# dylkot/cNMF

Measured on NVIDIA H100. Metric: NMF restarts/sec on NxG counts, K-sweep x100 seeds, 1/2/4/8 H100 vs sklearn CPU, higher is better.
Workload: dtype f32 (2-pass split-fp16 tensor-core products of group-normalised factors x exact integer counts, fp32 accumulate)

## Files before the change

### cnmf_b200/_lib.py

```python
import ctypes
import os

import numpy as np

_HERE = os.path.dirname(os.path.abspath(__file__))
LIB_PATH = os.path.join(_HERE, "libcnmf_b200.so")

SOLVER_MU, SOLVER_CD = 0, 1
PRECISION_FP32, PRECISION_TF32X3, PRECISION_TF32X3_GENERAL, PRECISION_F16X2, PRECISION_FP64 = 0, 1, 2, 3, 4
LOSS_FROBENIUS, LOSS_KULLBACK_LEIBLER, LOSS_ITAKURA_SAITO = 0, 1, 2
INIT_RANDOM, INIT_NNDSVD, INIT_NNDSVDA, INIT_NNDSVDAR = 0, 1, 2, 3
INIT_CODES = {"random": INIT_RANDOM, "nndsvd": INIT_NNDSVD, "nndsvda": INIT_NNDSVDA, "nndsvdar": INIT_NNDSVDAR}
MAX_COMPONENTS = 32


class CnmfError(RuntimeError):
    pass


class NmfParams(ctypes.Structure):
    _fields_ = [("solver", ctypes.c_int32), ("precision", ctypes.c_int32), ("max_iter", ctypes.c_int32),
                ("reserved", ctypes.c_int32), ("tol", ctypes.c_double),
                ("l1_reg_W", ctypes.c_double), ("l2_reg_W", ctypes.c_double),
                ("l1_reg_H", ctypes.c_double), ("l2_reg_H", ctypes.c_double),
                ("beta_loss", ctypes.c_int32), ("reserved2", ctypes.c_int32)]


UNIT_SOLVER_NONE = -1
UNIT_PIECES_NONE, UNIT_PIECES_TF32, UNIT_PIECES_F16 = 0, 1, 2
UNIT_GRAM_NONE, UNIT_GRAM_FUSED, UNIT_GRAM_STANDALONE = 0, 1, 2


class UpdateStepArgs(ctypes.Structure):
    _fields_ = [("n_slots", ctypes.c_int32), ("n_rids", ctypes.c_int32),
                ("ks", ctypes.c_void_p), ("rids", ctypes.c_void_p), ("done", ctypes.c_void_p),
                ("n", ctypes.c_int32), ("cpb_tiles", ctypes.c_int32), ("solver", ctypes.c_int32),
                ("pieces", ctypes.c_int32), ("gram", ctypes.c_int32), ("want_scalar", ctypes.c_int32),
                ("nsplit", ctypes.c_int32), ("l1", ctypes.c_float), ("l2", ctypes.c_float),
                ("F", ctypes.c_void_p), ("num", ctypes.c_void_p), ("gram_in", ctypes.c_void_p),
                ("piece_scale", ctypes.c_void_p), ("pieces_hi", ctypes.c_void_p), ("pieces_lo", ctypes.c_void_p),
                ("tile_scale", ctypes.c_void_p), ("gram_out", ctypes.c_void_p), ("scal_out", ctypes.c_void_p)]


UNIT_BETA_UPDATE, UNIT_BETA_DIVERGENCE = 0, 1
UNIT_SIDE_W, UNIT_SIDE_H = 0, 1


class BetaStepArgs(ctypes.Structure):
    _fields_ = [("n_slots", ctypes.c_int32), ("n_rids", ctypes.c_int32),
                ("ks", ctypes.c_void_p), ("rids", ctypes.c_void_p), ("done", ctypes.c_void_p),
                ("op", ctypes.c_int32), ("side", ctypes.c_int32), ("loss", ctypes.c_int32),
                ("n_items", ctypes.c_int32), ("n_contract", ctypes.c_int32), ("l1", ctypes.c_float), ("l2", ctypes.c_float),
                ("D", ctypes.c_void_p), ("F_own", ctypes.c_void_p), ("F_other", ctypes.c_void_p),
                ("oth_sum", ctypes.c_void_p), ("last", ctypes.c_void_p), ("totals", ctypes.c_void_p)]


UNIT_F64_UPDATE, UNIT_F64_GRAM, UNIT_F64_CROSS = 0, 1, 2


class UpdateStepF64Args(ctypes.Structure):
    _fields_ = [("n_slots", ctypes.c_int32), ("n_rids", ctypes.c_int32),
                ("ks", ctypes.c_void_p), ("rids", ctypes.c_void_p), ("done", ctypes.c_void_p),
                ("n", ctypes.c_int32), ("op", ctypes.c_int32), ("solver", ctypes.c_int32),
                ("want_scalar", ctypes.c_int32), ("l1", ctypes.c_double), ("l2", ctypes.c_double),
                ("F", ctypes.c_void_p), ("num", ctypes.c_void_p), ("gram_in", ctypes.c_void_p),
                ("gram_out", ctypes.c_void_p), ("scal_out", ctypes.c_void_p)]


FORM_FP32, FORM_TF32, FORM_TF32_EXACT, FORM_F16_EXACT, FORM_FP64 = 0, 1, 2, 3, 4
FORM_NAMES = {FORM_FP32: "fp32", FORM_TF32: "tf32", FORM_TF32_EXACT: "tf32_exact", FORM_F16_EXACT: "f16_exact",
              FORM_FP64: "fp64"}
OPERANDS = {"X": 0, "Xt": 1, "X_hi": 2, "X_lo": 3, "Xt_hi": 4, "Xt_lo": 5, "X_h16": 6, "Xt_h16": 7, "row_scale": 8,
            "col_scale": 9, "csc_col_ptr": 10, "csc_row_idx": 11, "csc_values": 12}


class ConvCheckArgs(ctypes.Structure):
    _fields_ = [("n_slots", ctypes.c_int32), ("n_rids", ctypes.c_int32),
                ("ks", ctypes.c_void_p), ("rids", ctypes.c_void_p),
                ("solver", ctypes.c_int32), ("it", ctypes.c_int32), ("max_iter", ctypes.c_int32),
                ("tol", ctypes.c_double), ("normX2", ctypes.c_double),
                ("cross", ctypes.c_void_p), ("gramA", ctypes.c_void_p), ("gramB", ctypes.c_void_p),
                ("violA", ctypes.c_void_p), ("violB", ctypes.c_void_p),
                ("done", ctypes.c_void_p), ("n_iter", ctypes.c_void_p),
                ("err0", ctypes.c_void_p), ("prev", ctypes.c_void_p), ("last", ctypes.c_void_p)]


_c = ctypes
_vp, _i, _ll, _d = _c.c_void_p, _c.c_int, _c.c_longlong, _c.c_double
_pp = _c.POINTER

SIGNATURES = {
    "cnmf_abi_version": (_i, []),
    "cnmf_last_error": (_c.c_char_p, []),
    "cnmf_create": (_i, [_pp(_vp), _i]),
    "cnmf_destroy": (_i, [_vp]),
    "cnmf_launch_count": (_ll, [_vp]),
    "cnmf_mem_info": (_i, [_vp, _pp(_ll), _pp(_ll), _pp(_ll)]),
    "cnmf_solve_bytes_per_row": (_ll, [_vp]),
    "cnmf_profile_enable": (_i, [_vp, _i]),
    "cnmf_profile_get": (_i, [_vp, _pp(_d), _pp(_ll), _pp(_d)]),
    "cnmf_profile_get_class": (_i, [_vp, _i, _pp(_d), _pp(_ll), _pp(_d)]),
    "cnmf_last_timing": (_i, [_vp, _pp(_d), _pp(_d), _pp(_d), _pp(_d)]),
    "cnmf_dataset_create": (_i, [_vp, _vp, _i, _i, _ll, _i, _i, _vp, _pp(_vp)]),
    "cnmf_dataset_create_csc": (_i, [_vp, _i, _i, _ll, _vp, _vp, _vp, _i, _vp, _pp(_vp)]),
    "cnmf_dataset_create_csr": (_i, [_vp, _i, _i, _ll, _vp, _vp, _vp, _i, _vp, _pp(_vp)]),
    "cnmf_dataset_create_from_csr": (_i, [_vp, _i, _i, _ll, _vp, _vp, _vp, _i, _vp, _pp(_vp)]),
    "cnmf_dataset_create_from_csr_f64": (_i, [_vp, _i, _i, _ll, _vp, _vp, _vp, _vp, _pp(_vp)]),
    "cnmf_dataset_dense_bytes": (_i, [_i, _i, _i, _pp(_ll)]),
    "cnmf_dataset_from_columns": (_i, [_vp, _vp, _vp, _i, _vp, _pp(_vp)]),
    "cnmf_dataset_destroy": (_i, [_vp]),
    "cnmf_dataset_shape": (_i, [_vp, _pp(_i), _pp(_i)]),
    "cnmf_dataset_ld": (_i, [_vp, _pp(_i), _pp(_i)]),
    "cnmf_dataset_is_exact": (_i, [_vp]),
    "cnmf_dataset_sums": (_i, [_vp, _pp(_d), _pp(_d)]),
    "cnmf_dataset_min": (_i, [_vp, _pp(_c.c_float), _vp]),
    "cnmf_dataset_col_stats": (_i, [_vp, _vp, _vp, _vp]),
    "cnmf_dataset_row_sums": (_i, [_vp, _vp, _vp]),
    "cnmf_dataset_scaled_col_stats": (_i, [_vp, _vp, _vp, _vp, _vp]),
    "cnmf_dataset_scale_rows": (_i, [_vp, _vp, _vp, _pp(_vp)]),
    "cnmf_dataset_tpm_stats": (_i, [_vp, _d, _vp, _vp, _vp, _vp]),
    "cnmf_random_init_host": (_i, [_c.c_uint32, _d, _i, _i, _i, _vp, _ll, _vp, _ll]),
    "cnmf_random_init_dev": (_i, [_vp, _i, _vp, _vp, _vp, _vp, _vp]),
    "cnmf_nndsvd_init_dev": (_i, [_vp, _i, _vp, _vp, _i, _vp, _vp, _vp]),
    "cnmf_nndsvd_chunk_limit": (_i, [_vp, _i]),
    "cnmf_nndsvd_gemm_host": (_i, [_vp, _i, _i, _vp, _vp, _vp]),
    "cnmf_dataset_create_f64": (_i, [_vp, _vp, _i, _i, _ll, _i, _vp, _pp(_vp)]),
    "cnmf_dataset_from_columns_f64": (_i, [_vp, _vp, _vp, _i, _vp, _pp(_vp)]),
    "cnmf_factorize_f64": (_i, [_vp, _i, _vp, _vp, _pp(NmfParams), _vp, _vp, _vp, _vp, _vp]),
    "cnmf_factorize_init_f64": (_i, [_vp, _i, _vp, _vp, _vp, _pp(NmfParams), _vp, _vp, _vp, _vp, _vp]),
    "cnmf_refit_f64": (_i, [_vp, _i, _i, _vp, _pp(NmfParams), _vp, _pp(_c.c_int32), _pp(_d), _vp]),
    "cnmf_project_rows_f64": (_i, [_vp, _i, _vp, _vp, _vp]),
    "cnmf_factorize": (_i, [_vp, _i, _vp, _vp, _pp(NmfParams), _vp, _vp, _vp, _vp, _vp]),
    "cnmf_factorize_seeds_dev": (_i, [_vp, _i, _vp, _vp, _pp(NmfParams), _vp, _ll, _vp, _vp, _vp]),
    "cnmf_allgather_spectra": (_i, [_vp, _vp, _ll, _ll, _vp, _vp]),
    "cnmf_comm_unique_id": (_i, [_vp]),
    "cnmf_comm_create": (_i, [_vp, _vp, _i, _i, _pp(_vp)]),
    "cnmf_comm_destroy": (_i, [_vp]),
    "cnmf_factorize_init": (_i, [_vp, _i, _vp, _vp, _vp, _pp(NmfParams), _vp, _vp, _vp, _vp, _vp]),
    "cnmf_factorize_dev": (_i, [_vp, _i, _vp, _vp, _vp, _pp(NmfParams), _vp, _vp, _vp, _vp]),
    "cnmf_refit": (_i, [_vp, _i, _i, _vp, _pp(NmfParams), _vp, _pp(_c.c_int32), _pp(_d), _vp]),
    "cnmf_project_rows": (_i, [_vp, _i, _vp, _vp, _vp]),
    "cnmf_gemm_abt_host": (_i, [_vp, _i, _vp, _vp, _i, _i, _i, _i, _i, _vp, _vp, _i, _vp, _i, _pp(_c.c_float), _vp]),
    "cnmf_update_step_host": (_i, [_vp, _pp(UpdateStepArgs), _vp]),
    "cnmf_beta_step_host": (_i, [_vp, _pp(BetaStepArgs), _vp]),
    "cnmf_update_step_f64_host": (_i, [_vp, _pp(UpdateStepF64Args), _vp]),
    "cnmf_conv_check_host": (_i, [_vp, _pp(ConvCheckArgs), _vp]),
    "cnmf_dataset_form": (_i, [_vp]),
    "cnmf_dataset_operand_host": (_i, [_vp, _i, _vp, _ll]),
    "cnmf_dataset_gemm_host": (_i, [_vp, _i, _i, _i, _vp, _vp, _pp(_i)]),
    "cnmf_l2_normalize_rows": (_i, [_vp, _vp, _i, _i, _i, _vp]),
    "cnmf_local_density": (_i, [_vp, _vp, _i, _i, _i, _i, _vp, _vp, _vp]),
    "cnmf_col_stats_dev": (_i, [_vp, _vp, _i, _i, _i, _vp, _vp, _vp]),
    "cnmf_gather_rows": (_i, [_vp, _vp, _i, _vp, _i, _i, _vp, _i, _vp]),
    "cnmf_sq_dists_to_rows": (_i, [_vp, _vp, _i, _i, _i, _vp, _i, _vp, _vp]),
    "cnmf_kmeans_step": (_i, [_vp, _vp, _i, _i, _i, _i, _vp, _vp, _vp, _vp, _vp, _vp, _vp, _vp, _pp(_c.c_int32), _pp(_c.c_int32), _pp(_d), _vp]),
    "cnmf_kmeans_fit": (_i, [_vp, _vp, _i, _i, _i, _i, _i, _i, _d, _vp, _vp, _i, _vp, _vp, _vp, _pp(_c.c_int32), _vp]),
    "cnmf_kmeans_assign": (_i, [_vp, _vp, _i, _i, _i, _vp, _i, _vp, _vp, _vp, _vp, _vp, _vp, _vp]),
    "cnmf_cluster_dist_sums": (_i, [_vp, _vp, _i, _i, _i, _vp, _i, _vp, _vp]),
    "cnmf_cluster_median": (_i, [_vp, _vp, _i, _i, _i, _vp, _i, _vp, _i, _vp]),
    "cnmf_l2_normalize_rows_f64": (_i, [_vp, _vp, _i, _i, _i, _vp]),
    "cnmf_local_density_f64": (_i, [_vp, _vp, _i, _i, _i, _i, _vp, _vp, _vp]),
    "cnmf_col_stats_dev_f64": (_i, [_vp, _vp, _i, _i, _i, _vp, _vp, _vp]),
    "cnmf_gather_rows_f64": (_i, [_vp, _vp, _i, _vp, _i, _i, _vp, _i, _vp]),
    "cnmf_sq_dists_to_rows_f64": (_i, [_vp, _vp, _i, _i, _i, _vp, _i, _vp, _vp]),
    "cnmf_kmeans_step_f64": (_i, [_vp, _vp, _i, _i, _i, _i, _vp, _vp, _vp, _vp, _vp, _vp, _pp(_c.c_int32), _pp(_c.c_int32), _pp(_d), _vp]),
    "cnmf_kmeans_fit_f64": (_i, [_vp, _vp, _i, _i, _i, _i, _i, _i, _d, _vp, _vp, _i, _vp, _vp, _vp, _pp(_c.c_int32), _vp]),
    "cnmf_kmeans_assign_f64": (_i, [_vp, _vp, _i, _i, _i, _vp, _i, _vp, _vp, _vp, _vp, _vp, _vp, _vp]),
    "cnmf_cluster_dist_sums_f64": (_i, [_vp, _vp, _i, _i, _i, _vp, _i, _vp, _vp]),
    "cnmf_cluster_median_f64": (_i, [_vp, _vp, _i, _i, _i, _vp, _i, _vp, _i, _vp]),
    "cnmf_moe_grams": (_i, [_vp, _vp, _vp, _vp, _i, _i, _i, _vp, _vp]),
    "cnmf_moe_correct": (_i, [_vp, _vp, _i, _i, _i, _ll, _i, _vp, _vp, _vp, _i, _i, _i, _vp, _ll, _i, _vp, _vp, _vp]),
    "cnmf_scale_quantile_ceiling": (_i, [_vp, _vp, _i, _i, _i, _ll, _i, _vp, _vp, _ll, _d, _i, _ll, _ll, _d, _vp, _ll,
                                         _i, _pp(_d), _vp]),
}

_lib = None


ABI_VERSION = 19


def load():
    global _lib
    if _lib is not None:
        return _lib
    if not os.path.exists(LIB_PATH):
        raise CnmfError(
            "libcnmf_b200.so not found at %s -- build it with `python -m cnmf_b200.build` "
            "(cnmf_b200 has no CPU / PyTorch fallback)" % LIB_PATH)
    lib = ctypes.CDLL(LIB_PATH)
    for name, (res, args) in SIGNATURES.items():
        fn = getattr(lib, name)
        fn.restype = res
        fn.argtypes = args
    if lib.cnmf_abi_version() != ABI_VERSION:
        raise CnmfError("libcnmf_b200.so ABI version mismatch")
    _lib = lib
    return lib


def check(rc):
    if rc != 0:
        msg = load().cnmf_last_error()
        raise CnmfError("cnmf_b200 error %d: %s" % (rc, msg.decode() if msg else "?"))


def ptr(a):
    if a is None:
        return None
    assert a.flags["C_CONTIGUOUS"]
    return a.ctypes.data_as(ctypes.c_void_p)


def f32c(a):
    return np.ascontiguousarray(a, dtype=np.float32)


def f64c(a):
    return np.ascontiguousarray(a, dtype=np.float64)
```

### cnmf_b200/csrc/capi_refit.cu

```cuda
#include <algorithm>
#include <chrono>
#include <cmath>
#include <cstring>
#include <vector>

#include "engine.h"
#include "gemm.h"
#include "nmf_kernels.cuh"

using namespace cnmf;

namespace {

__global__ void fill_kernel(float* p, float v, int rows, int n, int ld) {
  const long long total = (long long)rows * n;
  for (long long i = blockIdx.x * (long long)blockDim.x + threadIdx.x; i < total; i += (long long)gridDim.x * blockDim.x)
    p[(i / n) * ld + (i % n)] = v;
}

template <typename T>
__global__ void col_stats_kernel(const T* __restrict__ X, int rows, int cols, int ld,
                                 const double* __restrict__ row_scale, double* __restrict__ part) {
  const int c = blockIdx.x * blockDim.x + threadIdx.x;
  if (c >= cols) return;
// ... 342 lines not shown
  if (!A) return -2;
  CNMF_CUDA_CHECK(cudaMemsetAsync(A, 0, nr * 4, s));
  CNMF_CUDA_CHECK(cudaMemcpy2DAsync(A, (size_t)d->ld_r * 4, Ut_host, (size_t)d->n_rows * 4, (size_t)d->n_rows * 4, k,
                                    cudaMemcpyHostToDevice, s));
  if (v.form != Form::FP32) {
    A_hi = static_cast<float*>(h->dev_buf("proj.A_hi", nr * 4));
    A_lo = static_cast<float*>(h->dev_buf("proj.A_lo", nr * 4));
    if (!A_hi || !A_lo) return -2;
    if (v.form == Form::F16_EXACT) {
      A_rs = static_cast<float*>(h->dev_buf("proj.A_rs", sizeof(float) * (size_t)k * ((d->ld_r + 511) / 512)));
      if (!A_rs) return -2;
    }
    CNMF_TRY(make_pieces(v.form, A, k, d->n_rows, d->ld_r, v.scale_r, A_hi, A_lo, A_rs, s));
    h->launches += 1;
  }
  GemmArgs g{};
  g.M = k; g.N = d->n_cols; g.Kd = d->n_rows;
  g.lda = d->ld_r; g.ldb = d->ld_r; g.ldc = d->ld_c;
  int splits = 1;
  {
    const int tiles = ((k + 127) / 128) * ((d->n_cols + 255) / 256);
    if (tiles < 2 * h->sm_count) splits = (2 * h->sm_count + tiles - 1) / tiles;
    splits = std::min(splits, std::max(1, ((d->n_rows + 31) / 32) / 8));
    splits = std::min(splits, 32);
    splits = gemm_effective_splits(d->n_rows, splits, v.form == Form::F16_EXACT ? 1 : 0);
  }
  g.splits = g.splits_effective = splits;
  g.c_split_stride = (long long)k * d->ld_c;
  float* C = static_cast<float*>(h->dev_buf("proj.C", (size_t)splits * k * d->ld_c * 4));
  if (!C) return -2;
  g.C = C;
  CNMF_TRY(form_gemm(v.form, g, A, A_hi, A_lo, A_rs, v.B_cols, v.scale_c, s));
  h->launches += 1;
  std::vector<float> tmp((size_t)splits * k * d->ld_c);
  CNMF_CUDA_CHECK(cudaMemcpyAsync(tmp.data(), C, tmp.size() * 4, cudaMemcpyDeviceToHost, s));
  CNMF_CUDA_CHECK(cudaStreamSynchronize(s));
  for (int c = 0; c < k; ++c)
    for (int j = 0; j < d->n_cols; ++j) {
      double a = 0.0;
      for (int z = 0; z < splits; ++z) a += tmp[(size_t)z * k * d->ld_c + (size_t)c * d->ld_c + j];
      out_host[(size_t)c * d->n_cols + j] = (float)a;
    }
  return 0;
}

int cnmf_dataset_from_columns_f64(cnmf_dataset_t src, const int32_t* cols_host, const double* divisor_host, int n_cols,
                                  void* stream, cnmf_dataset_t* out) {
  CNMF_REQUIRE(src && cols_host && divisor_host && out && n_cols > 0, "dataset_from_columns_f64: bad arguments");
  CNMF_TRY(require_f64(src, "dataset_from_columns"));
  for (int c = 0; c < n_cols; ++c)
    CNMF_REQUIRE(cols_host[c] >= 0 && cols_host[c] < src->n_cols, "dataset_from_columns_f64: column index out of range");
  cnmf_handle_s* h = src->h;
  cudaStream_t s = as_stream(stream);
  CNMF_CUDA_CHECK(cudaSetDevice(h->device));
  int* d_cols = static_cast<int*>(h->dev_buf("fromcols.idx", sizeof(int) * n_cols));
  double* d_div = static_cast<double*>(h->dev_buf("fromcols.div64", sizeof(double) * n_cols));
  if (!d_cols || !d_div) return -2;
  CNMF_CUDA_CHECK(cudaMemcpyAsync(d_cols, cols_host, sizeof(int) * n_cols, cudaMemcpyHostToDevice, s));
  CNMF_CUDA_CHECK(cudaMemcpyAsync(d_div, divisor_host, sizeof(double) * n_cols, cudaMemcpyHostToDevice, s));
  auto* d = new cnmf_dataset_s(h, src->n_rows, n_cols, CNMF_PRECISION_FP64);
  d->form = Form::FP64;
  const size_t nx = (size_t)d->n_rows * d->ld_c;
  float* buf = nullptr;
  int rc = dataset_alloc(d, &buf, 2 * nx);
  if (rc == 0) {
    d->X64 = reinterpret_cast<double*>(buf);
    if (cudaMemsetAsync(d->X64, 0, nx * sizeof(double), s) != cudaSuccess) rc = -2;
  }
  if (rc == 0) {
    dim3 grid((n_cols + 127) / 128, std::min(d->n_rows, 16384));
    gather_cols_div_kernel<<<grid, 128, 0, s>>>(src->X64, d->n_rows, src->ld_c, d_cols, d_div, n_cols, d->X64, d->ld_c);
    h->launches += 1;
    if (cudaGetLastError() != cudaSuccess) rc = -2;
  }
  double sums[2] = {0.0, 0.0};
  if (rc == 0) rc = matrix_sums_f64(h, d->X64, d->n_rows, d->n_cols, d->ld_c, sums, s);
  if (rc != 0) {
    cnmf_dataset_destroy(d);
    return rc;
  }
  d->sum = sums[0];
  d->sum_sq = sums[1];
  *out = d;
  return 0;
}

int cnmf_refit_f64(cnmf_dataset_t d, int transposed, int k, const double* fixed_host, const cnmf_nmf_params* p,
                   double* out_host, int32_t* n_iter_host, double* err_host, void* stream) {
  CNMF_REQUIRE(d && fixed_host && p && out_host, "refit_f64: NULL argument");
  CNMF_TRY(require_f64(d, "refit"));
  CNMF_TRY(check_params_precision(d, p));
  CNMF_REQUIRE(k >= 1 && k <= KMAX, "refit_f64: n_components must be in [1, 32] on the CUDA path");
  if (p->beta_loss != CNMF_LOSS_FROBENIUS) {
    set_last_error("cnmf_refit_f64: float64 datasets support beta_loss = frobenius only");
    return -3;
  }
  cnmf_handle_s* h = d->h;
  cudaStream_t s = as_stream(stream);
  CNMF_CUDA_CHECK(cudaSetDevice(h->device));
  const DataView v = make_view(d, transposed != 0);
  const size_t nr = (size_t)k * v.ld_r, nc = (size_t)k * v.ld_c;
  double* Fr = static_cast<double*>(h->dev_buf("refit.Fr64", nr * 8));
  double* Fc = static_cast<double*>(h->dev_buf("refit.Fc64", nc * 8));
  double* T = static_cast<double*>(h->dev_buf("refit.T64", (size_t)v.n_r * k * 8));
  if (!Fr || !Fc || !T) return -2;
  CNMF_CUDA_CHECK(cudaMemsetAsync(Fr, 0, nr * 8, s));
  CNMF_CUDA_CHECK(cudaMemsetAsync(Fc, 0, nc * 8, s));
  CNMF_CUDA_CHECK(cudaMemcpy2DAsync(Fc, (size_t)v.ld_c * 8, fixed_host, (size_t)v.n_c * 8, (size_t)v.n_c * 8, k,
                                    cudaMemcpyHostToDevice, s));
  if (p->solver == CNMF_SOLVER_MU) {
    const double mean = v.sum / ((double)v.n_r * (double)v.n_c);
    CNMF_TRY(fill_f64(Fr, std::sqrt(mean / k), k, v.n_r, v.ld_r, s));
    h->launches += 1;
  }
  SolveIO io;
  io.R = 1;
  io.ks = {k};
  io.Fr64 = Fr;
  io.Fc64 = Fc;
  io.update_cols = false;
  CNMF_TRY(solve_batched(h, v, io, *p, s));
  transpose64_kernel<<<NUM_SMS * 4, 256, 0, s>>>(Fr, k, v.n_r, v.ld_r, T);
  CNMF_CUDA_CHECK(cudaGetLastError());
  h->launches += 1;
  CNMF_CUDA_CHECK(cudaMemcpyAsync(out_host, T, (size_t)v.n_r * k * 8, cudaMemcpyDeviceToHost, s));
  CNMF_CUDA_CHECK(cudaStreamSynchronize(s));
  if (n_iter_host) *n_iter_host = io.n_iter[0];
  if (err_host) *err_host = io.err[0];
  return 0;
}

int cnmf_project_rows_f64(cnmf_dataset_t d, int k, const double* Ut_host, double* out_host, void* stream) {
  CNMF_REQUIRE(d && Ut_host && out_host && k >= 1, "project_rows_f64: bad arguments");
  CNMF_TRY(require_f64(d, "project_rows"));
  cnmf_handle_s* h = d->h;
  cudaStream_t s = as_stream(stream);
  CNMF_CUDA_CHECK(cudaSetDevice(h->device));
  const size_t na = (size_t)k * d->ld_r, nc = (size_t)k * d->ld_c;
  double* A = static_cast<double*>(h->dev_buf("proj.A64", na * 8));
  double* C = static_cast<double*>(h->dev_buf("proj.C64", nc * 8));
  if (!A || !C) return -2;
  CNMF_CUDA_CHECK(cudaMemsetAsync(A, 0, na * 8, s));
  CNMF_CUDA_CHECK(cudaMemcpy2DAsync(A, (size_t)d->ld_r * 8, Ut_host, (size_t)d->n_rows * 8, (size_t)d->n_rows * 8, k,
                                    cudaMemcpyHostToDevice, s));
  h->launches += 1;
  CNMF_TRY(launch_gemm_f64(A, d->ld_r, k, d->X64, d->n_rows, d->n_cols, d->ld_c, true, C, d->ld_c, s));
  CNMF_CUDA_CHECK(cudaMemcpy2DAsync(out_host, (size_t)d->n_cols * 8, C, (size_t)d->ld_c * 8, (size_t)d->n_cols * 8, k,
                                    cudaMemcpyDeviceToHost, s));
  CNMF_CUDA_CHECK(cudaStreamSynchronize(s));
  return 0;
}

int cnmf_gemm_abt_host(cnmf_handle_t h, int precision, const float* A, const float* B, int M, int N, int Kd, int splits,
                       int b_exact, const float* k_scale, const float* out_col_scale, int tile_n, float* C, int reps,
                       float* ms_out, void* stream) {
  CNMF_REQUIRE(h && A && B && C && M > 0 && N > 0 && Kd > 0, "gemm_abt_host: bad arguments");
  const bool f16 = precision == CNMF_PRECISION_F16X2;
  CNMF_REQUIRE(!b_exact || f16 || precision == CNMF_PRECISION_TF32X3, "gemm_abt_host: b_exact needs tf32x3 or f16x2");
  const bool exact = f16 || b_exact;
  CNMF_REQUIRE(exact || (!k_scale && !out_col_scale), "gemm_abt_host: k_scale / out_col_scale need an exact form");
  const Form form = f16 ? Form::F16_EXACT
                  : precision != CNMF_PRECISION_TF32X3 ? Form::FP32
                  : b_exact ? Form::TF32_EXACT : Form::TF32;
  cudaStream_t s = as_stream(stream);
  CNMF_CUDA_CHECK(cudaSetDevice(h->device));
  const int lda = pad_ld(Kd), ldc = pad_ld(N);
  const size_t na = (size_t)M * lda, nb = (size_t)N * lda;
  float* dA = static_cast<float*>(h->dev_buf("gemmtest.A", na * 4));
  float* dB = static_cast<float*>(h->dev_buf("gemmtest.B", nb * 4));
  float* dAh = static_cast<float*>(h->dev_buf("gemmtest.Ah", na * 4));
  float* dAl = static_cast<float*>(h->dev_buf("gemmtest.Al", na * 4));
  float* dBh = static_cast<float*>(h->dev_buf("gemmtest.Bh", nb * 4));
  float* dBl = static_cast<float*>(h->dev_buf("gemmtest.Bl", nb * 4));
  const int se = gemm_effective_splits(Kd, splits, f16 ? 1 : 0);
  float* dC = static_cast<float*>(h->dev_buf("gemmtest.C", (size_t)se * M * ldc * 4));
  float* dRs = static_cast<float*>(h->dev_buf("gemmtest.rs", sizeof(float) * (size_t)M * ((lda + 511) / 512)));
  if (!dA || !dB || !dAh || !dAl || !dBh || !dBl || !dC || !dRs) return -2;
  CNMF_CUDA_CHECK(cudaMemsetAsync(dA, 0, na * 4, s));
  CNMF_CUDA_CHECK(cudaMemsetAsync(dB, 0, nb * 4, s));
  CNMF_CUDA_CHECK(cudaMemcpy2DAsync(dA, (size_t)lda * 4, A, (size_t)Kd * 4, (size_t)Kd * 4, M, cudaMemcpyHostToDevice, s));
  CNMF_CUDA_CHECK(cudaMemcpy2DAsync(dB, (size_t)lda * 4, B, (size_t)Kd * 4, (size_t)Kd * 4, N, cudaMemcpyHostToDevice, s));
  float* dKs = nullptr;
  float* dCs = nullptr;
  if (k_scale) {
    dKs = static_cast<float*>(h->dev_buf("gemmtest.kscale", (size_t)lda * 4));
    if (!dKs) return -2;
    CNMF_CUDA_CHECK(cudaMemsetAsync(dKs, 0, (size_t)lda * 4, s));
    CNMF_CUDA_CHECK(cudaMemcpyAsync(dKs, k_scale, (size_t)Kd * 4, cudaMemcpyHostToDevice, s));
  }
  if (out_col_scale) {
    dCs = static_cast<float*>(h->dev_buf("gemmtest.cscale", (size_t)ldc * 4));
    if (!dCs) return -2;
    CNMF_CUDA_CHECK(cudaMemsetAsync(dCs, 0, (size_t)ldc * 4, s));
    CNMF_CUDA_CHECK(cudaMemcpyAsync(dCs, out_col_scale, (size_t)N * 4, cudaMemcpyHostToDevice, s));
  }
  if (f16) CNMF_TRY(launch_to_half(dB, dBh, (long long)nb, s));
  else if (form != Form::FP32) CNMF_TRY(launch_split_tf32(dB, dBh, dBl, (long long)nb, s));
  CNMF_TRY(make_pieces(form, dA, M, Kd, lda, dKs, dAh, dAl, dRs, s));
  CNMF_CUDA_CHECK(cudaMemsetAsync(dC, 0xff, (size_t)se * M * ldc * 4, s));
  GemmArgs g{};
  g.M = M; g.N = N; g.Kd = Kd; g.lda = lda; g.ldb = lda; g.ldc = ldc;
  g.C = dC; g.c_split_stride = (long long)M * ldc; g.splits = splits; g.splits_effective = se;
  g.tile_n = tile_n;
  const Operand Bop{dB, dBh, dBl, N, Kd, lda};
  cudaEvent_t e0, e1;
  CNMF_CUDA_CHECK(cudaEventCreate(&e0));
  CNMF_CUDA_CHECK(cudaEventCreate(&e1));
  if (reps < 1) reps = 1;
  int rc = form_gemm(form, g, dA, dAh, dAl, dRs, Bop, dCs, s);
  if (rc == 0 && reps > 1) {
    cudaEventRecord(e0, s);
    for (int i = 0; i < reps && rc == 0; ++i) rc = form_gemm(form, g, dA, dAh, dAl, dRs, Bop, dCs, s);
    cudaEventRecord(e1, s);
  }
  h->launches += reps;
  if (rc != 0) return rc;
  std::vector<float> tmp((size_t)se * M * ldc);
  CNMF_CUDA_CHECK(cudaMemcpyAsync(tmp.data(), dC, tmp.size() * 4, cudaMemcpyDeviceToHost, s));
  CNMF_CUDA_CHECK(cudaStreamSynchronize(s));
  if (ms_out) {
    float ms = 0.f;
    if (reps > 1) cudaEventElapsedTime(&ms, e0, e1);
    *ms_out = reps > 1 ? ms / reps : 0.f;
  }
  cudaEventDestroy(e0);
  cudaEventDestroy(e1);
  for (int m = 0; m < M; ++m)
    for (int n = 0; n < N; ++n) {
      double a = 0.0;
      for (int z = 0; z < se; ++z) a += tmp[(size_t)z * M * ldc + (size_t)m * ldc + n];
      C[(size_t)m * N + n] = (float)a;
    }
  return 0;
}

}
```

### cnmf_b200/csrc/capi_units.cu

```cuda
#include <algorithm>
#include <vector>

#include "engine.h"
#include "nmf_beta.h"
#include "nmf_f64.h"
#include "nmf_kernels.cuh"

using namespace cnmf;

extern "C" int cnmf_update_step_host(cnmf_handle_t h, const cnmf_update_step_args* a, void* stream) {
  CNMF_REQUIRE(h && a && a->ks && a->rids && a->done && a->F && a->gram_in, "update_step: NULL argument");
  CNMF_REQUIRE(a->n_slots >= 1 && a->n_rids >= 1 && a->n >= 1 && a->nsplit >= 1, "update_step: bad sizes");
  CNMF_REQUIRE(a->cpb_tiles == 1 || a->cpb_tiles == 2 || a->cpb_tiles == 4, "update_step: cpb_tiles must be 1, 2 or 4");
  CNMF_REQUIRE(a->solver == CNMF_SOLVER_MU || a->solver == CNMF_SOLVER_CD || a->solver == CNMF_UNIT_SOLVER_NONE,
               "update_step: unknown solver");
  CNMF_REQUIRE(a->pieces >= CNMF_UNIT_PIECES_NONE && a->pieces <= CNMF_UNIT_PIECES_F16, "update_step: unknown pieces mode");
  CNMF_REQUIRE(a->gram >= CNMF_UNIT_GRAM_NONE && a->gram <= CNMF_UNIT_GRAM_STANDALONE, "update_step: unknown Gram mode");
  CNMF_REQUIRE(a->pieces == CNMF_UNIT_PIECES_NONE || (a->pieces_hi && a->pieces_lo), "update_step: pieces buffers missing");
  CNMF_REQUIRE(a->pieces != CNMF_UNIT_PIECES_F16 || a->tile_scale, "update_step: tile_scale missing");
  CNMF_REQUIRE(a->gram == CNMF_UNIT_GRAM_NONE || a->gram_out, "update_step: gram_out missing");
  CNMF_REQUIRE(!a->want_scalar || a->scal_out, "update_step: scal_out missing");
  const bool none = a->solver == CNMF_UNIT_SOLVER_NONE;
  CNMF_REQUIRE(!none || a->gram != CNMF_UNIT_GRAM_FUSED, "update_step: no update launch to fuse the Gram into");
  CNMF_REQUIRE(a->num || (none && !a->want_scalar), "update_step: num missing");
// ... 248 lines not shown
  CNMF_REQUIRE(a->op != CNMF_UNIT_F64_CROSS || (a->num && a->scal_out), "update_step_f64: num / scal_out missing");
  CNMF_REQUIRE(a->op != CNMF_UNIT_F64_GRAM || a->gram_out, "update_step_f64: gram_out missing");
  CNMF_REQUIRE(!(upd && a->want_scalar) || a->scal_out, "update_step_f64: scal_out missing");
  const int R = a->n_slots, NR = a->n_rids;
  std::vector<int> meta;
  int SK = 0, kmax = 0;
  CNMF_TRY(unit_slots(a->ks, a->rids, a->done, R, NR, "update_step_f64", meta, &SK, &kmax));
  const int kp = round_up(kmax, 4);

  cudaStream_t s = as_stream(stream);
  CNMF_CUDA_CHECK(cudaSetDevice(h->device));
  const int n = a->n, ld = pad_ld(n);
  const size_t nf = (size_t)SK * ld, gsz = (size_t)NR * KMAX * KMAX;
  const int chunks = f64_chunks(n), gchunks = f64_gram_chunks(n);
  int* d_meta = static_cast<int*>(h->dev_buf("unit.meta", sizeof(int) * meta.size()));
  double* d_F = static_cast<double*>(h->dev_buf("unit.F64", nf * 8));
  double* d_num = static_cast<double*>(h->dev_buf("unit.num64", nf * 8));
  double* d_gin = static_cast<double*>(h->dev_buf("unit.gram_in", sizeof(double) * gsz));
  double* d_gout = static_cast<double*>(h->dev_buf("unit.gram_out", sizeof(double) * gsz));
  double* d_scal = static_cast<double*>(h->dev_buf("unit.scal", sizeof(double) * NR));
  double* d_gpart = static_cast<double*>(h->dev_buf("unit.gram_part", sizeof(double) * (size_t)NR * gchunks * kp * kp));
  double* d_spart = static_cast<double*>(h->dev_buf("unit.scal_part", sizeof(double) * (size_t)NR * chunks));
  if (!d_meta || !d_F || !d_num || !d_gin || !d_gout || !d_scal || !d_gpart || !d_spart) return -2;
  CNMF_CUDA_CHECK(cudaMemcpyAsync(d_meta, meta.data(), sizeof(int) * meta.size(), cudaMemcpyHostToDevice, s));
  CNMF_CUDA_CHECK(cudaMemcpyAsync(d_F, a->F, nf * 8, cudaMemcpyHostToDevice, s));
  if (a->num) CNMF_CUDA_CHECK(cudaMemcpyAsync(d_num, a->num, nf * 8, cudaMemcpyHostToDevice, s));
  if (a->gram_in) CNMF_CUDA_CHECK(cudaMemcpyAsync(d_gin, a->gram_in, sizeof(double) * gsz, cudaMemcpyHostToDevice, s));
  if (a->gram_out) CNMF_CUDA_CHECK(cudaMemcpyAsync(d_gout, a->gram_out, sizeof(double) * gsz, cudaMemcpyHostToDevice, s));
  if (a->scal_out) CNMF_CUDA_CHECK(cudaMemcpyAsync(d_scal, a->scal_out, sizeof(double) * NR, cudaMemcpyHostToDevice, s));

  const BatchMeta b{d_meta, d_meta + R, d_meta + 2 * R, d_meta + 3 * R, R, kp};
  const F64Launch L{h, s, SK};
  const F64View f{d_F, n, ld};
  if (upd)
    CNMF_TRY(f64_update(L, a->solver == CNMF_SOLVER_CD, f, d_num, d_gin, b, a->l1, a->l2, d_spart,
                        a->want_scalar ? d_scal : nullptr));
  else if (a->op == CNMF_UNIT_F64_GRAM)
    CNMF_TRY(f64_gram(L, f, b, d_gpart, d_gout));
  else
    CNMF_TRY(f64_cross(L, f, d_num, b, d_spart, d_scal));

  CNMF_CUDA_CHECK(cudaMemcpyAsync(a->F, d_F, nf * 8, cudaMemcpyDeviceToHost, s));
  if (a->gram_out) CNMF_CUDA_CHECK(cudaMemcpyAsync(a->gram_out, d_gout, sizeof(double) * gsz, cudaMemcpyDeviceToHost, s));
  if (a->scal_out) CNMF_CUDA_CHECK(cudaMemcpyAsync(a->scal_out, d_scal, sizeof(double) * NR, cudaMemcpyDeviceToHost, s));
  CNMF_CUDA_CHECK(cudaStreamSynchronize(s));
  return 0;
}

extern "C" int cnmf_conv_check_host(cnmf_handle_t h, const cnmf_conv_check_args* a, void* stream) {
  CNMF_REQUIRE(h && a && a->ks && a->rids && a->done && a->n_iter && a->err0 && a->prev && a->last,
               "conv_check: NULL argument");
  CNMF_REQUIRE(a->n_slots >= 1 && a->n_rids >= 1, "conv_check: bad sizes");
  CNMF_REQUIRE(a->solver == CNMF_SOLVER_MU || a->solver == CNMF_SOLVER_CD, "conv_check: unknown solver");
  const bool mu = a->solver == CNMF_SOLVER_MU;
  CNMF_REQUIRE(!mu || (a->cross && a->gramA && a->gramB), "conv_check: cross / gramA / gramB missing");
  CNMF_REQUIRE(mu || a->violA, "conv_check: violA missing");
  const int R = a->n_slots, NR = a->n_rids;
  std::vector<int> meta;
  int SK = 0, kmax = 0;
  CNMF_TRY(unit_slots(a->ks, a->rids, nullptr, R, NR, "conv_check", meta, &SK, &kmax));
  meta.resize(3 * R + 2 * NR);
  for (int r = 0; r < NR; ++r) {
    meta[3 * R + r] = a->done[r];
    meta[3 * R + NR + r] = a->n_iter[r];
  }

  cudaStream_t s = as_stream(stream);
  CNMF_CUDA_CHECK(cudaSetDevice(h->device));
  const size_t gsz = (size_t)NR * KMAX * KMAX;
  int* d_meta = static_cast<int*>(h->dev_buf("unit.meta", sizeof(int) * meta.size()));
  double* d_state = static_cast<double*>(h->dev_buf("unit.conv_state", sizeof(double) * 6 * NR));
  double* d_gram = static_cast<double*>(h->dev_buf("unit.conv_gram", sizeof(double) * 2 * gsz));
  if (!d_meta || !d_state || !d_gram) return -2;
  double *d_err0 = d_state, *d_prev = d_state + NR, *d_last = d_state + 2 * NR;
  double *d_x = d_state + 3 * NR, *d_vb = d_state + 4 * NR;
  CNMF_CUDA_CHECK(cudaMemcpyAsync(d_meta, meta.data(), sizeof(int) * meta.size(), cudaMemcpyHostToDevice, s));
  CNMF_CUDA_CHECK(cudaMemcpyAsync(d_err0, a->err0, sizeof(double) * NR, cudaMemcpyHostToDevice, s));
  CNMF_CUDA_CHECK(cudaMemcpyAsync(d_prev, a->prev, sizeof(double) * NR, cudaMemcpyHostToDevice, s));
  CNMF_CUDA_CHECK(cudaMemcpyAsync(d_last, a->last, sizeof(double) * NR, cudaMemcpyHostToDevice, s));
  CNMF_CUDA_CHECK(cudaMemcpyAsync(d_x, mu ? a->cross : a->violA, sizeof(double) * NR, cudaMemcpyHostToDevice, s));
  if (mu) {
    CNMF_CUDA_CHECK(cudaMemcpyAsync(d_gram, a->gramA, sizeof(double) * gsz, cudaMemcpyHostToDevice, s));
    CNMF_CUDA_CHECK(cudaMemcpyAsync(d_gram + gsz, a->gramB, sizeof(double) * gsz, cudaMemcpyHostToDevice, s));
  } else if (a->violB) {
    CNMF_CUDA_CHECK(cudaMemcpyAsync(d_vb, a->violB, sizeof(double) * NR, cudaMemcpyHostToDevice, s));
  }

  int* d_done = d_meta + 3 * R;
  const BatchMeta b{d_meta, d_meta + R, d_meta + 2 * R, d_done, R, round_up(kmax, 4)};
  const ConvState st{d_err0, d_prev, d_last, d_done, d_done + NR};
  h->launches += 1;
  if (mu) CNMF_TRY(launch_mu_check(st, d_x, d_gram, d_gram + gsz, a->normX2, b, a->it, a->tol, a->max_iter, s));
  else CNMF_TRY(launch_cd_check(st, d_x, a->violB ? d_vb : nullptr, b, a->it, a->tol, a->max_iter, s));

  CNMF_CUDA_CHECK(cudaMemcpyAsync(meta.data(), d_meta, sizeof(int) * meta.size(), cudaMemcpyDeviceToHost, s));
  CNMF_CUDA_CHECK(cudaMemcpyAsync(a->err0, d_err0, sizeof(double) * NR, cudaMemcpyDeviceToHost, s));
  CNMF_CUDA_CHECK(cudaMemcpyAsync(a->prev, d_prev, sizeof(double) * NR, cudaMemcpyDeviceToHost, s));
  CNMF_CUDA_CHECK(cudaMemcpyAsync(a->last, d_last, sizeof(double) * NR, cudaMemcpyDeviceToHost, s));
  CNMF_CUDA_CHECK(cudaStreamSynchronize(s));
  for (int r = 0; r < NR; ++r) {
    a->done[r] = meta[3 * R + r];
    a->n_iter[r] = meta[3 * R + NR + r];
  }
  return 0;
}

static_assert((int)Form::FP32 == CNMF_FORM_FP32 && (int)Form::TF32 == CNMF_FORM_TF32 &&
                  (int)Form::TF32_EXACT == CNMF_FORM_TF32_EXACT && (int)Form::F16_EXACT == CNMF_FORM_F16_EXACT &&
                  (int)Form::FP64 == CNMF_FORM_FP64,
              "CNMF_FORM_* mirror cnmf::Form");

extern "C" int cnmf_dataset_form(cnmf_dataset_t d) {
  CNMF_REQUIRE(d, "dataset_form: NULL dataset");
  return (int)d->form;
}

extern "C" int cnmf_dataset_operand_host(cnmf_dataset_t d, int which, void* out_host, long long bytes) {
  CNMF_REQUIRE(d && out_host, "dataset_operand: NULL argument");
  const long long nx = (long long)d->n_rows * d->ld_c, nxt = (long long)d->n_cols * d->ld_r;
  const void* src = nullptr;
  long long size = 0;
  switch (which) {
    case CNMF_OPERAND_X: src = d->X; size = 4 * nx; break;
    case CNMF_OPERAND_XT: src = d->Xt; size = 4 * nxt; break;
    case CNMF_OPERAND_X_HI: src = d->X_hi; size = 4 * nx; break;
    case CNMF_OPERAND_X_LO: src = d->X_lo; size = 4 * nx; break;
    case CNMF_OPERAND_XT_HI: src = d->Xt_hi; size = 4 * nxt; break;
    case CNMF_OPERAND_XT_LO: src = d->Xt_lo; size = 4 * nxt; break;
    case CNMF_OPERAND_X_H16: src = d->X_h16; size = 2 * nx; break;
    case CNMF_OPERAND_XT_H16: src = d->Xt_h16; size = 2 * nxt; break;
    case CNMF_OPERAND_ROW_SCALE: src = d->row_scale; size = 4LL * d->ld_r; break;
    case CNMF_OPERAND_COL_SCALE: src = d->col_scale; size = 4LL * d->ld_c; break;
    case CNMF_OPERAND_CSC_COL_PTR: src = d->col_ptr; size = 8LL * (d->n_cols + 1); break;
    case CNMF_OPERAND_CSC_ROW_IDX: src = d->row_idx; size = 4LL * d->nnz; break;
    case CNMF_OPERAND_CSC_VALUES: src = d->vals; size = 4LL * d->nnz; break;
    default: CNMF_REQUIRE(false, "dataset_operand: unknown array");
  }
  if (!src) {
    set_last_error("dataset_operand: this dataset does not hold that array");
    return -3;
  }
  CNMF_REQUIRE(bytes == size, "dataset_operand: bytes must be the array's size");
  CNMF_CUDA_CHECK(cudaSetDevice(d->h->device));
  CNMF_CUDA_CHECK(cudaMemcpy(out_host, src, (size_t)size, cudaMemcpyDeviceToHost));
  return 0;
}

extern "C" int cnmf_dataset_gemm_host(cnmf_dataset_t d, int transposed, int side, int SK, const float* F_host,
                                      float* out_host, int* splits_out) {
  CNMF_REQUIRE(d && splits_out && (side == 0 || side == 1) && SK >= 1, "dataset_gemm: bad arguments");
  CNMF_TRY(require_dense(d, "dataset_gemm"));
  cnmf_handle_s* h = d->h;
  const DataView v = make_view(d, transposed != 0);
  const GemmPlan plan = view_gemm_plan(v, side, SK);
  *splits_out = plan.splits;
  if (!out_host) return 0;
  CNMF_REQUIRE(F_host, "dataset_gemm: NULL factor");
  const int n_in = side == 0 ? v.n_c : v.n_r, ld_in = side == 0 ? v.ld_c : v.ld_r;
  const int n_out = side == 0 ? v.n_r : v.n_c, ld_out = side == 0 ? v.ld_r : v.ld_c;
  const float* piece_scale = side == 0 ? v.scale_c : v.scale_r;
  cudaStream_t s = nullptr;
  CNMF_CUDA_CHECK(cudaSetDevice(h->device));
  const size_t nf = (size_t)SK * ld_in, nc = (size_t)plan.splits * SK * ld_out;
  const int ktiles = (ld_in + 511) / 512;
  float* F = static_cast<float*>(h->dev_buf("unit.gemm_F", nf * 4));
  float* F_hi = static_cast<float*>(h->dev_buf("unit.gemm_F_hi", nf * 4));
  float* F_lo = static_cast<float*>(h->dev_buf("unit.gemm_F_lo", nf * 4));
  float* ts = static_cast<float*>(h->dev_buf("unit.gemm_tile_scale", sizeof(float) * (size_t)SK * ktiles));
  float* C = static_cast<float*>(h->dev_buf("unit.gemm_C", nc * 4));
  if (!F || !F_hi || !F_lo || !ts || !C) return -2;
  CNMF_CUDA_CHECK(cudaMemsetAsync(F, 0, nf * 4, s));
  CNMF_CUDA_CHECK(cudaMemcpy2DAsync(F, (size_t)ld_in * 4, F_host, (size_t)n_in * 4, (size_t)n_in * 4, SK,
                                    cudaMemcpyHostToDevice, s));
  CNMF_TRY(make_pieces(v.form, F, SK, n_in, ld_in, piece_scale, F_hi, F_lo, ts, s));
  h->launches += v.form == Form::FP32 ? 0 : 1;
  CNMF_TRY(view_gemm(h, v, side, F, F_hi, F_lo, ts, SK, C, plan, s));
  CNMF_CUDA_CHECK(cudaMemcpy2DAsync(out_host, (size_t)n_out * 4, C, (size_t)ld_out * 4, (size_t)n_out * 4,
                                    (size_t)plan.splits * SK, cudaMemcpyDeviceToHost, s));
  CNMF_CUDA_CHECK(cudaStreamSynchronize(s));
  return 0;
}
```

### cnmf_b200/csrc/engine.h

```cpp
#pragma once
#include <cuda_runtime.h>

#include <map>
#include <string>
#include <vector>

#include "../../include/cnmf_b200.h"
#include "common.cuh"
#include "gemm.h"

namespace cnmf {

enum class Form { FP32, TF32, TF32_EXACT, F16_EXACT, FP64 };
inline bool form_exact(Form f) { return f == Form::TF32_EXACT || f == Form::F16_EXACT; }

}

struct cnmf_handle_s {
  int device = 0;
  int sm_count = cnmf::NUM_SMS;
  long long launches = 0;
  bool profile = false;
  std::vector<cudaEvent_t> ev_pool;
  struct Pending { int begin; int end; int cls; double work; };
  int prof_last_end = -1;
  long long prof_last_launches = -1;
  cudaStream_t prof_last_stream = nullptr;
  std::vector<Pending> ev_pending;
  size_t ev_used = 0;
  static constexpr int PROF_CLASSES = 6;
  double prof_ms[PROF_CLASSES] = {}, prof_work[PROF_CLASSES] = {};
  long long prof_launches[PROF_CLASSES] = {};
  int nndsvd_chunk_restarts = 0;
  double t_rng_ms = 0, t_h2d_ms = 0, t_solve_ms = 0, t_d2h_ms = 0;
  int prof_begin(cudaStream_t s, double work, int cls = 0);
  void prof_end(cudaStream_t s, int slot);
  void prof_collect();
  std::map<std::string, std::pair<void*, size_t>> ws;
  std::map<std::string, std::pair<void*, size_t>> pinned;

  std::multimap<size_t, void*> pool;
  size_t pool_bytes = 0;
  void* pool_take(size_t bytes);
  void pool_give(void* p, size_t bytes);
  void* dev_buf(const std::string& name, size_t bytes);
  void* host_buf(const std::string& name, size_t bytes);
  void release_all();
};

struct cnmf_dataset_s {
  cnmf_handle_s* h = nullptr;
  int n_rows = 0, n_cols = 0;
  int ld_c = 0;
  int ld_r = 0;
  int precision = 0;
  cnmf::Form form = cnmf::Form::FP32;
  float *X = nullptr, *Xt = nullptr;
  float *X_hi = nullptr, *X_lo = nullptr, *Xt_hi = nullptr, *Xt_lo = nullptr;
  void *X_h16 = nullptr, *Xt_h16 = nullptr;
  float *row_scale = nullptr, *col_scale = nullptr;
  double sum = 0.0, sum_sq = 0.0;
  bool sparse = false;
  long long nnz = 0;
  long long* col_ptr = nullptr;
  int* row_idx = nullptr;
  float* vals = nullptr;
  double* col_sums = nullptr;
  int* item_ptr = nullptr;
  int n_items = 0;
  double* X64 = nullptr;
  std::vector<std::pair<void*, size_t>> owned;

  cnmf_dataset_s(cnmf_handle_s* h_, int rows, int cols, int precision_)
      : h(h_), n_rows(rows), n_cols(cols), ld_c(cnmf::pad_ld(cols)), ld_r(cnmf::pad_ld(rows)), precision(precision_) {}
};

namespace cnmf {

inline cudaStream_t as_stream(void* s) { return reinterpret_cast<cudaStream_t>(s); }

struct Operand {
  const float* full;
  const float* hi;
  const float* lo;
  int rows, cols, ld;
};

struct DataView {
  Operand B_rows;
  Operand B_cols;
  int n_r, n_c, ld_r, ld_c;
  double sum, sum_sq;
  Form form;
  const float* scale_r;
  const float* scale_c;
  const double* X64;
  bool transposed;
};

DataView make_view(const cnmf_dataset_s* d, bool transposed);

int form_gemm(Form form, GemmArgs g, const float* A, const float* A_hi, const float* A_lo, const float* a_tile_scale,
              const Operand& B, const float* out_scale, cudaStream_t s);
struct GemmPlan {
  int splits;
  long long split_stride;
};
GemmPlan view_gemm_plan(const DataView& v, int side, int SK);
int view_gemm(cnmf_handle_s* h, const DataView& v, int side, const float* F, const float* F_hi, const float* F_lo,
              const float* tile_scale, int SK, float* C, const GemmPlan& plan, cudaStream_t s);
int make_pieces(Form form, const float* F, int rows, int n, int ld, const float* scale, float* hi, float* lo,
                float* tile_scale, cudaStream_t s);

int dataset_alloc(cnmf_dataset_s* d, float** p, size_t elems);
int dataset_finish(cnmf_dataset_s* d, cudaStream_t s, bool exact = false);
int dataset_resolve_form(cnmf_dataset_s* d, bool exact, cudaStream_t s);
int check_params_precision(const cnmf_dataset_s* d, const cnmf_nmf_params* p);
int require_f32(const cnmf_dataset_s* d, const char* what);
int require_f64(const cnmf_dataset_s* d, const char* what);

struct SolveIO {
  int R = 0;
  std::vector<int> ks;
  float *Fr = nullptr, *Fc = nullptr;
  bool update_cols = true;
  const float* num_rows = nullptr;
  double *Fr64 = nullptr, *Fc64 = nullptr;
  std::vector<int> n_iter;
  std::vector<double> last;
  std::vector<double> err;
};

int solve_batched(cnmf_handle_s* h, const DataView& v, SolveIO& io, const cnmf_nmf_params& p, cudaStream_t s);
int solve_batched_beta(cnmf_handle_s* h, const DataView& v, SolveIO& io, const cnmf_nmf_params& p, cudaStream_t s);
int solve_batched_f64(cnmf_handle_s* h, const DataView& v, SolveIO& io, const cnmf_nmf_params& p, cudaStream_t s);
int matrix_sums_f64(cnmf_handle_s* h, const double* X, int rows, int cols, int ld, double* out_host, cudaStream_t s);
int fill_f64(double* p, double v, int rows, int n, int ld, cudaStream_t s);
int matrix_min(cnmf_handle_s* h, const float* X, int rows, int cols, int ld, float* out_host, cudaStream_t s);
int dataset_ensure_full_transpose(cnmf_dataset_s* d, cudaStream_t s);

constexpr int CSC_CHUNK = 4096;
int require_dense(const cnmf_dataset_s* d, const char* what);
int csc_project(const cnmf_dataset_s* d, const float* U, int k, int kp, float* out, int ld, cudaStream_t s);
int stage_rows(cnmf_handle_s* h, const float* F, int k, int n, int ld, int kp, float* U, cudaStream_t s);
int csc_col_stats(cnmf_dataset_s* d, cudaStream_t s);
int csc_detect_exact(cnmf_dataset_s* d, cudaStream_t s, bool* exact);
int csc_gather_cols(const cnmf_dataset_s* d, const int* cols, const float* scale, int n_cols, float* dst, int ld_dst,
                    cudaStream_t s);
int csc_tpm_sums(const cnmf_dataset_s* d, double target_sum, double* totals, double* col_sums, cudaStream_t s);
struct DeviceTemp {
  void* p = nullptr;
  DeviceTemp() = default;
  DeviceTemp(const DeviceTemp&) = delete;
  DeviceTemp& operator=(const DeviceTemp&) = delete;
  ~DeviceTemp() {
    if (p) cudaFree(p);
  }
  int alloc(size_t bytes, const std::string& what) {
    const cudaError_t e = cudaMalloc(&p, bytes < 256 ? 256 : bytes);
    if (e != cudaSuccess) {
      p = nullptr;
      set_last_error(what + ": cudaMalloc(" + std::to_string(bytes) + " bytes) failed: " + cudaGetErrorString(e));
      return -2;
    }
    return 0;
  }
  template <class T>
  T* as() const { return static_cast<T*>(p); }
};
int check_csr(const char* what, int n_rows, int n_cols, long long nnz, const int64_t* row_ptr, const int32_t* col_idx);
constexpr int CSR_ROW_BLOCK = 256;
constexpr long long CSR_COUNT_BUDGET = 1LL << 25;
int csr_to_csc(cnmf_dataset_s* d, const long long* row_ptr, const int* col_idx, const float* vals, cudaStream_t s);
int csr_scatter_rows(const long long* row_ptr, long long base, const int* col_idx, const float* vals, int r0, int r1,
                     float* X, int ld, cudaStream_t s);
int csr_scatter_rows(const long long* row_ptr, long long base, const int* col_idx, const double* vals, int r0, int r1,
                     double* X, int ld, cudaStream_t s);

int launch_gemm_f64(const double* A, int lda, int M, const float* X, int n_rows, int n_cols, int ldx, bool to_genes,
                    double* C, int ldc, cudaStream_t s);
int launch_gemm_f64(const double* A, int lda, int M, const double* X, int n_rows, int n_cols, int ldx, bool to_genes,
                    double* C, int ldc, cudaStream_t s);
int launch_gemm_f64_split(const double* A, int lda, int M, const float* X, int n_rows, int n_cols, int ldx,
                          bool to_genes, int k_chunk, double* C, int ldc, long long c_split_stride, cudaStream_t s);
int launch_gemm_f64_split(const double* A, int lda, int M, const double* X, int n_rows, int n_cols, int ldx,
                          bool to_genes, int k_chunk, double* C, int ldc, long long c_split_stride, cudaStream_t s);
int nndsvd_starts_dev(cnmf_dataset_s* d, int R, const int* ks, const uint32_t* seeds, int init, float* Wt, float* H,
                      cudaStream_t s);
int nndsvd_starts_dev(cnmf_dataset_s* d, int R, const int* ks, const uint32_t* seeds, int init, double* Wt, double* H,
                      cudaStream_t s);

}
```

### cnmf_b200/csrc/gemm.h

```cpp
#pragma once
#include <cuda_runtime.h>

namespace cnmf {

struct GemmArgs {
  const float* A_hi;
  const float* A_lo;
  const float* B_hi;
  const float* B_lo;
  float* C;
  int M, N, Kd;
  int lda, ldb, ldc;
  long long c_split_stride;
  int splits;
  int splits_effective;
  int b_exact;
  const float* out_col_scale;
  int f16;
  const float* a_tile_scale;
  int a_tiles;
  int tile_n;
};

int gemm_effective_splits(int Kd, int splits, int f16 = 0);

int gemm_fixed_splits(int Kd, int f16 = 0);

int gemm_tf32x3(const GemmArgs& g, cudaStream_t stream);

int gemm_fp32_simt(const GemmArgs& g, cudaStream_t stream);

}
```

### cnmf_b200/csrc/gemm_simt.cu

```cuda
#include <cuda_runtime.h>

#include "common.cuh"
#include "gemm.h"

namespace cnmf {

namespace {

constexpr int TM = 128, TN = 128, TK = 16;

__global__ void __launch_bounds__(256)
gemm_fp32_simt_kernel(const float* __restrict__ A, const float* __restrict__ B, float* __restrict__ C, int M, int N,
                      int Kd, int lda, int ldb, int ldc, long long c_split_stride, int k_per_split) {
  __shared__ float As[TK][TM + 4];
  __shared__ float Bs[TK][TN + 4];

  const int m0 = blockIdx.y * TM;
  const int n0 = blockIdx.x * TN;
  const int z = blockIdx.z;
  const int k_begin = z * k_per_split;
  const int k_end = min(Kd, k_begin + k_per_split);

  const int tid = threadIdx.x;
  const int tx = tid & 15;
  const int ty = tid >> 4;
  const int lrow = tid >> 2;
  const int lk = (tid & 3) * 4;

  float acc[8][8];
#pragma unroll
  for (int i = 0; i < 8; ++i)
#pragma unroll
    for (int j = 0; j < 8; ++j) acc[i][j] = 0.f;

  for (int k0 = k_begin; k0 < k_end; k0 += TK) {
#pragma unroll
    for (int h = 0; h < 2; ++h) {
      const int r = lrow + h * 64;
      float4 va = make_float4(0.f, 0.f, 0.f, 0.f), vb = va;
      const int gk = k0 + lk;
      if (m0 + r < M) {
        const float* p = A + static_cast<long long>(m0 + r) * lda + gk;
        if (gk + 3 < k_end) va = *reinterpret_cast<const float4*>(p);
        else {
          if (gk < k_end) va.x = p[0];
          if (gk + 1 < k_end) va.y = p[1];
          if (gk + 2 < k_end) va.z = p[2];
        }
      }
      if (n0 + r < N) {
        const float* p = B + static_cast<long long>(n0 + r) * ldb + gk;
        if (gk + 3 < k_end) vb = *reinterpret_cast<const float4*>(p);
        else {
          if (gk < k_end) vb.x = p[0];
          if (gk + 1 < k_end) vb.y = p[1];
          if (gk + 2 < k_end) vb.z = p[2];
        }
      }
      As[lk + 0][r] = va.x; As[lk + 1][r] = va.y; As[lk + 2][r] = va.z; As[lk + 3][r] = va.w;
      Bs[lk + 0][r] = vb.x; Bs[lk + 1][r] = vb.y; Bs[lk + 2][r] = vb.z; Bs[lk + 3][r] = vb.w;
    }
    __syncthreads();
#pragma unroll
    for (int k = 0; k < TK; ++k) {
      float a[8], b[8];
      const float4 a0 = *reinterpret_cast<const float4*>(&As[k][ty * 4]);
      const float4 a1 = *reinterpret_cast<const float4*>(&As[k][ty * 4 + 64]);
      const float4 b0 = *reinterpret_cast<const float4*>(&Bs[k][tx * 4]);
      const float4 b1 = *reinterpret_cast<const float4*>(&Bs[k][tx * 4 + 64]);
      a[0] = a0.x; a[1] = a0.y; a[2] = a0.z; a[3] = a0.w; a[4] = a1.x; a[5] = a1.y; a[6] = a1.z; a[7] = a1.w;
      b[0] = b0.x; b[1] = b0.y; b[2] = b0.z; b[3] = b0.w; b[4] = b1.x; b[5] = b1.y; b[6] = b1.z; b[7] = b1.w;
#pragma unroll
      for (int i = 0; i < 8; ++i)
#pragma unroll
        for (int j = 0; j < 8; ++j) acc[i][j] = fmaf(a[i], b[j], acc[i][j]);
    }
    __syncthreads();
  }

  float* Cz = C + static_cast<long long>(z) * c_split_stride;
#pragma unroll
  for (int i = 0; i < 8; ++i) {
    const int m = m0 + ty * 4 + (i & 3) + (i >> 2) * 64;
    if (m >= M) continue;
#pragma unroll
    for (int jh = 0; jh < 2; ++jh) {
      const int n = n0 + tx * 4 + jh * 64;
      if (n + 3 < ldc && n < round_up(N, 4)) {
        *reinterpret_cast<float4*>(Cz + static_cast<long long>(m) * ldc + n) =
            make_float4(acc[i][jh * 4], acc[i][jh * 4 + 1], acc[i][jh * 4 + 2], acc[i][jh * 4 + 3]);
      }
    }
  }
}

}

int gemm_fp32_simt(const GemmArgs& g, cudaStream_t stream) {
  CNMF_REQUIRE(g.M > 0 && g.N > 0 && g.Kd > 0, "gemm: empty problem");
  CNMF_REQUIRE(g.lda % 4 == 0 && g.ldb % 4 == 0 && g.ldc % 4 == 0, "gemm: leading dimensions must be multiples of 4 floats");
  const int splits = gemm_effective_splits(g.Kd, g.splits);
  CNMF_REQUIRE(splits == g.splits_effective, "gemm: splits_effective mismatch");
  const int total_kb = (g.Kd + 31) / 32;
  const int kb_per_split = (total_kb + splits - 1) / splits;
  dim3 grid((g.N + TN - 1) / TN, (g.M + TM - 1) / TM, splits);
  gemm_fp32_simt_kernel<<<grid, 256, 0, stream>>>(g.A_hi, g.B_hi, g.C, g.M, g.N, g.Kd, g.lda, g.ldb, g.ldc,
                                                   g.c_split_stride, kb_per_split * 32);
  CNMF_CUDA_CHECK(cudaGetLastError());
  return 0;
}

}
```

### cnmf_b200/csrc/gemm_tf32x3.cu

```cuda
#include <cuda.h>
#include <cuda_runtime.h>
#include <cstdint>
#include <cstdio>
#include <algorithm>
#include <map>
#include <mutex>
#include <tuple>

#include "common.cuh"
#include "gemm.h"

namespace cnmf {

namespace {

constexpr int BM = 128;
constexpr int NUM_THREADS = 128 * (1 + BM / 64);
constexpr int BK = 32;
constexpr long long WAIT_TIMEOUT_CYCLES = 4000000000LL;

template <int BN, int STAGES, bool BEXACT>
struct SmemLayout {
  static constexpr int A_BYTES = BM * BK * 4;
  static constexpr int B_BYTES = BN * BK * 4;
  static constexpr int STAGE_BYTES = 2 * A_BYTES + (BEXACT ? 1 : 2) * B_BYTES;
  static constexpr int BAR_OFFSET = STAGES * STAGE_BYTES;
  static constexpr int TOTAL = BAR_OFFSET + 3 * STAGES * 8;
  static constexpr int DYN_BYTES = TOTAL + 1024;
  static_assert(DYN_BYTES <= 227 * 1024, "pipeline stages do not fit the shared memory of an SM");
};

__device__ __forceinline__ void mbar_init(uint32_t bar, uint32_t count) {
  asm volatile("mbarrier.init.shared::cta.b64 [%0], %1;" ::"r"(bar), "r"(count) : "memory");
}
__device__ __forceinline__ void mbar_arrive_expect_tx(uint32_t bar, uint32_t bytes) {
  asm volatile("mbarrier.arrive.expect_tx.shared::cta.b64 _, [%0], %1;" ::"r"(bar), "r"(bytes) : "memory");
}
__device__ __forceinline__ void mbar_arrive(uint32_t bar) {
  asm volatile("mbarrier.arrive.shared::cta.b64 _, [%0];" ::"r"(bar) : "memory");
}
__device__ __forceinline__ bool mbar_try_wait(uint32_t bar, uint32_t parity) {
  uint32_t ok;
  asm volatile(
      "{\n\t.reg .pred p;\n\t"
      "mbarrier.try_wait.parity.shared::cta.b64 p, [%1], %2;\n\t"
      "selp.u32 %0, 1, 0, p;\n\t}"
      : "=r"(ok)
      : "r"(bar), "r"(parity)
      : "memory");
  return ok != 0;
}
template <bool TRAP>
__device__ __forceinline__ void mbar_wait(uint32_t bar, uint32_t parity) {
  if (mbar_try_wait(bar, parity)) return;
  const long long t0 = clock64();
  while (!mbar_try_wait(bar, parity)) {
    if (TRAP && clock64() - t0 > WAIT_TIMEOUT_CYCLES) __trap();
  }
}
__device__ __forceinline__ void tma_load_2d(uint32_t dst, const CUtensorMap* map, uint32_t bar, int c0, int c1) {
  asm volatile(
      "cp.async.bulk.tensor.2d.shared::cluster.global.mbarrier::complete_tx::bytes [%0], [%1, {%3, %4}], [%2];"
      ::"r"(dst), "l"(reinterpret_cast<uint64_t>(map)), "r"(bar), "r"(c0), "r"(c1)
      : "memory");
}
__device__ __forceinline__ void tma_load_2d_multicast(uint32_t dst, const CUtensorMap* map, uint32_t bar, int c0, int c1,
                                                      uint16_t mask) {
  asm volatile(
      "cp.async.bulk.tensor.2d.shared::cluster.global.mbarrier::complete_tx::bytes.multicast::cluster"
      " [%0], [%1, {%3, %4}], [%2], %5;"
      ::"r"(dst), "l"(reinterpret_cast<uint64_t>(map)), "r"(bar), "r"(c0), "r"(c1), "h"(mask)
      : "memory");
}

__device__ __forceinline__ void mbar_arrive_remote(uint32_t bar, uint32_t rank) {
  asm volatile(
      "{\n\t.reg .b32 remote;\n\t"
      "mapa.shared::cluster.u32 remote, %0, %1;\n\t"
      "mbarrier.arrive.shared::cluster.b64 _, [remote];\n\t}"
      ::"r"(bar), "r"(rank)
      : "memory");
}
__device__ __forceinline__ void cluster_sync() {
  asm volatile("barrier.cluster.arrive.release;\n\tbarrier.cluster.wait.acquire;" ::: "memory");
}

__device__ __forceinline__ uint64_t make_smem_desc(uint32_t smem_addr) {
  uint64_t d = 0;
  d |= static_cast<uint64_t>((smem_addr & 0x3FFFFu) >> 4);
  d |= static_cast<uint64_t>(1) << 16;
  d |= static_cast<uint64_t>(1024 >> 4) << 32;
  d |= static_cast<uint64_t>(1) << 62;
  return d;
}

__device__ __forceinline__ void named_bar_sync(uint32_t id, uint32_t count) {
  asm volatile("bar.sync %0, %1;" ::"r"(id), "r"(count) : "memory");
}
__device__ __forceinline__ void named_bar_arrive(uint32_t id, uint32_t count) {
  asm volatile("bar.arrive %0, %1;" ::"r"(id), "r"(count) : "memory");
}

template <int N>
__device__ __forceinline__ void setmaxnreg_dec() { asm volatile("setmaxnreg.dec.sync.aligned.u32 %0;" ::"n"(N)); }
template <int N>
__device__ __forceinline__ void setmaxnreg_inc() { asm volatile("setmaxnreg.inc.sync.aligned.u32 %0;" ::"n"(N)); }

__device__ __forceinline__ void wgmma_fence() { asm volatile("wgmma.fence.sync.aligned;" ::: "memory"); }
__device__ __forceinline__ void wgmma_commit() { asm volatile("wgmma.commit_group.sync.aligned;" ::: "memory"); }
template <int N>
__device__ __forceinline__ void wgmma_wait() { asm volatile("wgmma.wait_group.sync.aligned %0;" ::"n"(N) : "memory"); }

#define CNMF_R64                                                                      \
  "%0, %1, %2, %3, %4, %5, %6, %7, %8, %9, %10, %11, %12, %13, %14, %15, "            \
  "%16, %17, %18, %19, %20, %21, %22, %23, %24, %25, %26, %27, %28, %29, %30, %31, "  \
  "%32, %33, %34, %35, %36, %37, %38, %39, %40, %41, %42, %43, %44, %45, %46, %47, "  \
  "%48, %49, %50, %51, %52, %53, %54, %55, %56, %57, %58, %59, %60, %61, %62, %63"
#define CNMF_R84 CNMF_R64 ", %64, %65, %66, %67, %68, %69, %70, %71, %72, %73, %74, %75, %76, %77, %78, %79, " \
  "%80, %81, %82, %83"
#define CNMF_R96 CNMF_R84 ", %84, %85, %86, %87, %88, %89, %90, %91, %92, %93, %94, %95"
#define CNMF_D4(i) "+f"(d[i]), "+f"(d[i + 1]), "+f"(d[i + 2]), "+f"(d[i + 3])
#define CNMF_D8(i) CNMF_D4(i), CNMF_D4(i + 4)
#define CNMF_D64 CNMF_D8(0), CNMF_D8(8), CNMF_D8(16), CNMF_D8(24), CNMF_D8(32), CNMF_D8(40), CNMF_D8(48), CNMF_D8(56)
#define CNMF_D84 CNMF_D64, CNMF_D8(64), CNMF_D8(72), CNMF_D4(80)
#define CNMF_D96 CNMF_D64, CNMF_D8(64), CNMF_D8(72), CNMF_D8(80), CNMF_D8(88)
#define CNMF_WGMMA(N, REGS, IA, IB, IACC, ...)                                                                        \
  template <bool F16>                                                                                                 \
  __device__ __forceinline__ void wgmma_m64n##N(float (&d)[N / 2], uint64_t adesc, uint64_t bdesc, uint32_t acc) {    \
    if constexpr (F16)                                                                                                \
      asm volatile("{\n\t.reg .pred p;\n\tsetp.ne.b32 p, %" IACC ", 0;\n\t"                                          \
                   "wgmma.mma_async.sync.aligned.m64n" #N "k16.f32.f16.f16 {" REGS "}, %" IA ", %" IB                 \
                   ", p, 1, 1, 0, 0;\n\t}"                                                                            \
                   : __VA_ARGS__ : "l"(adesc), "l"(bdesc), "r"(acc));                                                 \
    else                                                                                                              \
      asm volatile("{\n\t.reg .pred p;\n\tsetp.ne.b32 p, %" IACC ", 0;\n\t"                                          \
                   "wgmma.mma_async.sync.aligned.m64n" #N "k8.f32.tf32.tf32 {" REGS "}, %" IA ", %" IB ", p, 1, 1;\n\t}" \
                   : __VA_ARGS__ : "l"(adesc), "l"(bdesc), "r"(acc));                                                 \
  }
CNMF_WGMMA(128, CNMF_R64, "64", "65", "66", CNMF_D64)
CNMF_WGMMA(168, CNMF_R84, "84", "85", "86", CNMF_D84)
CNMF_WGMMA(192, CNMF_R96, "96", "97", "98", CNMF_D96)

template <int BN, bool F16>
__device__ __forceinline__ void wgmma_tile(float (&d)[BN / 2], uint64_t adesc, uint64_t bdesc, uint32_t acc) {
  if constexpr (BN == 128) wgmma_m64n128<F16>(d, adesc, bdesc, acc);
  else if constexpr (BN == 168) wgmma_m64n168<F16>(d, adesc, bdesc, acc);
  else wgmma_m64n192<F16>(d, adesc, bdesc, acc);
}

struct TileOrder {
  int m_tiles, n_pairs, group, group_n;
};

__host__ __device__ __forceinline__ void decode_item(int w, const TileOrder& o, int& mt, int& np, int& z) {
  const int per_slice = o.m_tiles * o.n_pairs;
  z = w / per_slice;
  int r = w - z * per_slice;
  const int q_tiles = o.group_n ? o.n_pairs : o.m_tiles;
  const int p_tiles = o.group_n ? o.m_tiles : o.n_pairs;
  const int g0 = r / (o.group * p_tiles) * o.group;
  r -= g0 * p_tiles;
  const int gq = q_tiles - g0 < o.group ? q_tiles - g0 : o.group;
  const int p = r / gq, q = g0 + r % gq;
  mt = o.group_n ? p : q;
  np = o.group_n ? q : p;
}

template <int BN, int STAGES, bool BEXACT, bool F16>
__device__ __forceinline__ void
gemm_body(const CUtensorMap& tmA_hi, const CUtensorMap& tmA_lo, const CUtensorMap& tmB_hi, const CUtensorMap& tmB_lo,
          float* __restrict__ C, int M, int ldc, long long c_split_stride,
          const TileOrder& ord, int n_tiles, int splits, int total_kb, int kb_per_split, int chain_kb,
          const float* __restrict__ out_scale, const float* __restrict__ a_tile_scale, int a_tiles, int a_gshift) {
  static_assert(!F16 || BEXACT, "the fp16 path exists for exact integer B operands only");
  static_assert(BN == 128 || (BEXACT && (BN == 168 || BN == 192)), "wide n-tiles in the exact-B forms only");
  constexpr int NC = BM / 64;
  constexpr int BKE = F16 ? 2 * BK : BK;
  constexpr int KSTEP_BYTES = 32;
  using L = SmemLayout<BN, STAGES, BEXACT>;
  extern __shared__ uint8_t smem_raw[];
  const uint32_t smem_base = (smem_u32(smem_raw) + 1023u) & ~1023u;

  const uint32_t bar_base = smem_base + L::BAR_OFFSET;
  auto full_bar = [&](int s) { return bar_base + 8u * s; };
  auto empty_bar = [&](int s) { return bar_base + 8u * (STAGES + s); };
  auto peer_free_bar = [&](int s) { return bar_base + 8u * (2 * STAGES + s); };

  const int wg = __shfl_sync(0xffffffffu, static_cast<int>(threadIdx.x >> 7), 0);
  const int warp = (threadIdx.x >> 5) & 3;
  const int lane = threadIdx.x & 31;
  const int rank = blockIdx.x & 1, cluster = blockIdx.x >> 1, clusters = gridDim.x >> 1;

  if (threadIdx.x == 0) {
    for (int s = 0; s < STAGES; ++s) {
      mbar_init(full_bar(s), 1);
      mbar_init(empty_bar(s), 4 * NC);
      mbar_init(peer_free_bar(s), 1);
    }
    asm volatile("fence.mbarrier_init.release.cluster;" ::: "memory");
  }
  cluster_sync();

  const int items = ord.m_tiles * ord.n_pairs * splits;

  constexpr bool REBALANCE = BN > 128;
  if (wg == 0) {
    if constexpr (REBALANCE) setmaxnreg_dec<40>();
    if (threadIdx.x == 0) {
      int stage = 0;
      uint32_t phase = 0;
      constexpr uint32_t stage_tx = static_cast<uint32_t>(L::STAGE_BYTES);
      constexpr uint32_t HALF_A = L::A_BYTES / 2;
      for (int w = cluster; w < items; w += clusters) {
        int mt, np, z;
        decode_item(w, ord, mt, np, z);
        const int nt = 2 * np + rank;
        const int kb0 = z * kb_per_split;
        const int kb1 = min(total_kb, kb0 + kb_per_split);
        for (int kb = kb0; kb < kb1; ++kb) {
          mbar_wait<true>(empty_bar(stage), phase ^ 1u);
          mbar_arrive_remote(peer_free_bar(stage), rank ^ 1);
          mbar_wait<true>(peer_free_bar(stage), phase);
          const uint32_t st = smem_base + stage * L::STAGE_BYTES;
          mbar_arrive_expect_tx(full_bar(stage), stage_tx);
          tma_load_2d_multicast(st + rank * HALF_A, &tmA_hi, full_bar(stage), kb * BKE, mt * BM + rank * (BM / 2), 0x3);
          tma_load_2d_multicast(st + L::A_BYTES + rank * HALF_A, &tmA_lo, full_bar(stage), kb * BKE,
                                mt * BM + rank * (BM / 2), 0x3);
          tma_load_2d(st + 2 * L::A_BYTES, &tmB_hi, full_bar(stage), kb * BKE, nt * BN);
          if constexpr (!BEXACT) tma_load_2d(st + 2 * L::A_BYTES + L::B_BYTES, &tmB_lo, full_bar(stage), kb * BKE, nt * BN);
          if (++stage == STAGES) { stage = 0; phase ^= 1u; }
        }
      }
      for (int s = 0; s < STAGES; ++s) {
        mbar_wait<true>(empty_bar(stage), phase ^ 1u);
        if (++stage == STAGES) { stage = 0; phase ^= 1u; }
      }
    }
  } else {
    if constexpr (REBALANCE) setmaxnreg_inc<232>();
    constexpr uint32_t TURN_BAR = 1, TURN_THREADS = 256;
    const int cw = wg - 1;
    const uint32_t a_off = static_cast<uint32_t>(cw * 64 * 128);
    const uint32_t next_bar = TURN_BAR + (cw + 1 == NC ? 0 : cw + 1);
    if (cw == NC - 1) named_bar_arrive(TURN_BAR, TURN_THREADS);
    int stage = 0;
    uint32_t phase = 0;
    for (int w = cluster; w < items; w += clusters) {
      int mt, np, z;
      decode_item(w, ord, mt, np, z);
      const int nt = 2 * np + rank;
      const int kb0 = z * kb_per_split;
      const int kb1 = min(total_kb, kb0 + kb_per_split);
      const int row0 = mt * BM + cw * 64 + warp * 16 + (lane >> 2);
      float acc[BN / 2];
#pragma unroll
      for (int i = 0; i < BN / 2; ++i) acc[i] = 0.f;
      const float* sc_row0 = (F16 && a_tile_scale && row0 < M) ? a_tile_scale + static_cast<long long>(row0) * a_tiles : nullptr;
      const float* sc_row1 = (F16 && a_tile_scale && row0 + 8 < M) ? a_tile_scale + static_cast<long long>(row0 + 8) * a_tiles : nullptr;
      for (int c0 = kb0; c0 < kb1; c0 += chain_kb) {
        const int c1 = min(kb1, c0 + chain_kb);
        float d[BN / 2];
        int prev = -1;
        for (int kb = c0; kb < c1; ++kb) {
          mbar_wait<false>(full_bar(stage), phase);
          named_bar_sync(TURN_BAR + cw, TURN_THREADS);
          const uint32_t st = smem_base + stage * L::STAGE_BYTES;
          const uint64_t a_hi = make_smem_desc(st + a_off);
          const uint64_t a_lo = make_smem_desc(st + L::A_BYTES + a_off);
          const uint64_t b_hi = make_smem_desc(st + 2 * L::A_BYTES);
          const uint64_t b_lo = make_smem_desc(st + 2 * L::A_BYTES + L::B_BYTES);
          wgmma_fence();
#pragma unroll
          for (int k = 0; k < BK * 4 / KSTEP_BYTES; ++k) {
            const uint64_t koff = static_cast<uint64_t>((k * KSTEP_BYTES) >> 4);
            const uint32_t acc0 = (kb > c0 || k > 0) ? 1u : 0u;
            wgmma_tile<BN, F16>(d, a_lo + koff, b_hi + koff, acc0);
            if constexpr (!BEXACT) wgmma_tile<BN, F16>(d, a_hi + koff, b_lo + koff, 1u);
            wgmma_tile<BN, F16>(d, a_hi + koff, b_hi + koff, 1u);
          }
          wgmma_commit();
          named_bar_arrive(next_bar, TURN_THREADS);
          if (prev >= 0) {
            wgmma_wait<1>();
            if (lane == 0) mbar_arrive(empty_bar(prev));
          }
          prev = stage;
          if (++stage == STAGES) { stage = 0; phase ^= 1u; }
        }
        wgmma_wait<0>();
        if (lane == 0) mbar_arrive(empty_bar(prev));
        if constexpr (F16) {
          const float s0 = sc_row0 ? sc_row0[c0 >> a_gshift] : 1.f;
          const float s1 = sc_row1 ? sc_row1[c0 >> a_gshift] : 1.f;
#pragma unroll
          for (int i = 0; i < BN / 2; i += 4) {
            acc[i] = fmaf(d[i], s0, acc[i]);
            acc[i + 1] = fmaf(d[i + 1], s0, acc[i + 1]);
            acc[i + 2] = fmaf(d[i + 2], s1, acc[i + 2]);
            acc[i + 3] = fmaf(d[i + 3], s1, acc[i + 3]);
          }
        } else {
#pragma unroll
          for (int i = 0; i < BN / 2; ++i) acc[i] += d[i];
        }
      }
      if (nt >= n_tiles) continue;
      constexpr int EPI_J = (BN / 8) % 8 == 0 ? 8 : 7;
      static_assert((BN / 8) % EPI_J == 0, "column groups in whole batches");
      float* cbase = C + static_cast<long long>(z) * c_split_stride;
      const int colq = nt * BN + 2 * (lane & 3);
#pragma unroll
      for (int j0 = 0; j0 < BN / 8; j0 += EPI_J) {
        float2 sc[EPI_J];
#pragma unroll
        for (int j = 0; j < EPI_J; ++j) {
          const int col = colq + 8 * (j0 + j);
          sc[j] = out_scale && col < ldc ? *reinterpret_cast<const float2*>(out_scale + col) : make_float2(1.f, 1.f);
        }
#pragma unroll
        for (int j = 0; j < EPI_J; ++j) {
          const int col = colq + 8 * (j0 + j);
          if (col >= ldc) continue;
          const float* a = acc + 4 * (j0 + j);
          if (row0 < M)
            *reinterpret_cast<float2*>(cbase + static_cast<long long>(row0) * ldc + col) =
                make_float2(a[0] * sc[j].x, a[1] * sc[j].y);
          if (row0 + 8 < M)
            *reinterpret_cast<float2*>(cbase + static_cast<long long>(row0 + 8) * ldc + col) =
                make_float2(a[2] * sc[j].x, a[3] * sc[j].y);
        }
      }
    }
    if (cw == 0) named_bar_sync(TURN_BAR, TURN_THREADS);
  }
  cluster_sync();
}

template <int BN, int STAGES, bool BEXACT, bool F16>
__global__ void __cluster_dims__(2, 1, 1) __launch_bounds__(NUM_THREADS, 1)
gemm_tf32x3_kernel(const __grid_constant__ CUtensorMap tmA_hi, const __grid_constant__ CUtensorMap tmA_lo,
                   const __grid_constant__ CUtensorMap tmB_hi, const __grid_constant__ CUtensorMap tmB_lo,
                   float* __restrict__ C, int M, int ldc, long long c_split_stride,
                   const TileOrder ord, int n_tiles, int splits, int total_kb, int kb_per_split, int chain_kb,
                   const float* __restrict__ out_scale, const float* __restrict__ a_tile_scale, int a_tiles, int a_gshift) {
  gemm_body<BN, STAGES, BEXACT, F16>(tmA_hi, tmA_lo, tmB_hi, tmB_lo, C, M, ldc, c_split_stride, ord, n_tiles, splits,
                                     total_kb, kb_per_split, chain_kb, out_scale, a_tile_scale, a_tiles, a_gshift);
}

typedef CUresult (*PFN_encodeTiled)(CUtensorMap*, CUtensorMapDataType, cuuint32_t, void*, const cuuint64_t*,
                                    const cuuint64_t*, const cuuint32_t*, const cuuint32_t*, CUtensorMapInterleave,
                                    CUtensorMapSwizzle, CUtensorMapL2promotion, CUtensorMapFloatOOBfill);

PFN_encodeTiled get_encode_fn() {
  static PFN_encodeTiled fn = nullptr;
  static std::once_flag once;
  std::call_once(once, [] {
    void* p = nullptr;
    cudaDriverEntryPointQueryResult qres;
    if (cudaGetDriverEntryPoint("cuTensorMapEncodeTiled", &p, cudaEnableDefault, &qres) == cudaSuccess &&
        qres == cudaDriverEntryPointSuccess)
      fn = reinterpret_cast<PFN_encodeTiled>(p);
  });
  return fn;
}

struct MapKey {
  const void* ptr; int rows, cols, ld, box_rows, f16;
  bool operator<(const MapKey& o) const {
    return std::tie(ptr, rows, cols, ld, box_rows, f16) < std::tie(o.ptr, o.rows, o.cols, o.ld, o.box_rows, o.f16);
  }
};

int make_map(CUtensorMap* map, const float* ptr, int rows, int cols, int ld, int box_rows, bool f16 = false) {
  static std::mutex mu;
  static std::map<MapKey, CUtensorMap> cache;
  const MapKey key{ptr, rows, cols, ld, box_rows, f16 ? 1 : 0};
  {
    std::lock_guard<std::mutex> lock(mu);
    auto it = cache.find(key);
    if (it != cache.end()) { *map = it->second; return 0; }
  }
  PFN_encodeTiled enc = get_encode_fn();
  if (!enc) { set_last_error("cuTensorMapEncodeTiled entry point not available"); return -2; }
  const int esize = f16 ? 2 : 4;
  cuuint64_t dims[2] = {static_cast<cuuint64_t>(cols), static_cast<cuuint64_t>(rows)};
  cuuint64_t strides[1] = {static_cast<cuuint64_t>(ld) * esize};
  cuuint32_t box[2] = {static_cast<cuuint32_t>(128 / esize), static_cast<cuuint32_t>(box_rows)};
  cuuint32_t estr[2] = {1, 1};
  CUresult r = enc(map, f16 ? CU_TENSOR_MAP_DATA_TYPE_FLOAT16 : CU_TENSOR_MAP_DATA_TYPE_FLOAT32, 2, const_cast<float*>(ptr), dims, strides, box, estr,
                   CU_TENSOR_MAP_INTERLEAVE_NONE, CU_TENSOR_MAP_SWIZZLE_128B, CU_TENSOR_MAP_L2_PROMOTION_L2_256B,
                   CU_TENSOR_MAP_FLOAT_OOB_FILL_NONE);
  if (r != CUDA_SUCCESS) {
    set_last_error("cuTensorMapEncodeTiled failed with CUresult " + std::to_string(static_cast<int>(r)));
    return -2;
  }
  std::lock_guard<std::mutex> lock(mu);
  if (cache.size() >= 512) cache.clear();
  cache.emplace(key, *map);
  return 0;
}

static double order_bytes(int q_tiles, int p_tiles, double q_panel, double p_panel, int group, int grid, double budget) {
  const long long waves = (static_cast<long long>(group) * p_tiles + grid - 1) / grid;
  const double q_reads = group * q_panel <= budget ? 1.0 : static_cast<double>(std::min<long long>(p_tiles, waves));
  return q_tiles * q_panel * q_reads + static_cast<double>((q_tiles + group - 1) / group) * p_tiles * p_panel;
}

static TileOrder pick_tile_order(int m_tiles, int n_pairs, double a_panel, double b_panel, int grid, long long l2_bytes) {
  const double budget = 0.5 * static_cast<double>(l2_bytes);
  TileOrder best{m_tiles, n_pairs, m_tiles, 0};
  double best_bytes = order_bytes(m_tiles, n_pairs, a_panel, b_panel, m_tiles, grid, budget);
  for (int gn = 0; gn < 2; ++gn) {
    const int q = gn ? n_pairs : m_tiles, p = gn ? m_tiles : n_pairs;
    const double qb = gn ? b_panel : a_panel, pb = gn ? a_panel : b_panel;
    int prev = 0;
    for (int ng = 1; ng <= q; ++ng) {
      const int g = (q + ng - 1) / ng;
      if (g == prev) continue;
      prev = g;
      const double b = order_bytes(q, p, qb, pb, g, grid, budget);
      if (b < best_bytes) { best_bytes = b; best = TileOrder{m_tiles, n_pairs, g, gn}; }
    }
  }
  return best;
}

template <int BN, int STAGES, bool BEXACT, bool F16>
int launch(const GemmArgs& g, cudaStream_t stream) {
  using L = SmemLayout<BN, STAGES, BEXACT>;
  constexpr int BKE = F16 ? 2 * BK : BK;
  CUtensorMap mAh, mAl, mBh, mBl;
  int rc;
  if ((rc = make_map(&mAh, g.A_hi, g.M, g.Kd, g.lda, BM / 2, F16))) return rc;
  if ((rc = make_map(&mAl, g.A_lo, g.M, g.Kd, g.lda, BM / 2, F16))) return rc;
  if ((rc = make_map(&mBh, g.B_hi, g.N, g.Kd, g.ldb, BN, F16))) return rc;
  if ((rc = make_map(&mBl, BEXACT ? g.B_hi : g.B_lo, g.N, g.Kd, g.ldb, BN, F16))) return rc;
  int dev = 0, l2 = 0;
  CNMF_CUDA_CHECK(cudaGetDevice(&dev));
  CNMF_CUDA_CHECK(cudaDeviceGetAttribute(&l2, cudaDevAttrL2CacheSize, dev));
  const int m_tiles = (g.M + BM - 1) / BM;
  const int n_tiles = (std::min(g.ldc, (g.N + 31) / 32 * 32) + BN - 1) / BN;
  const int n_pairs = (n_tiles + 1) / 2;
  const int total_kb = (g.Kd + BKE - 1) / BKE;
  int splits = g.splits < 1 ? 1 : g.splits;
  if (splits > total_kb) splits = total_kb;
  int kb_per_split = (total_kb + splits - 1) / splits;
  if (F16 && (kb_per_split & 1)) ++kb_per_split;
  splits = (total_kb + kb_per_split - 1) / kb_per_split;
  if (splits != g.splits_effective) { set_last_error("gemm: splits_effective mismatch (use gemm_effective_splits)"); return -1; }

  auto kern = gemm_tf32x3_kernel<BN, STAGES, BEXACT, F16>;
  static int max_clusters[64] = {};
  int clusters_cap = dev >= 0 && dev < 64 ? max_clusters[dev] : 0;
  if (clusters_cap == 0) {
    CNMF_CUDA_CHECK(cudaFuncSetAttribute(kern, cudaFuncAttributeMaxDynamicSharedMemorySize, L::DYN_BYTES));
    cudaLaunchConfig_t cfg = {};
    cfg.gridDim = dim3(2, 1, 1);
    cfg.blockDim = dim3(NUM_THREADS, 1, 1);
    cfg.dynamicSmemBytes = L::DYN_BYTES;
    CNMF_CUDA_CHECK(cudaOccupancyMaxActiveClusters(&clusters_cap, kern, &cfg));
    if (clusters_cap < 1) { set_last_error("gemm: no 2-CTA cluster of this kernel fits the device"); return -1; }
    if (dev >= 0 && dev < 64) max_clusters[dev] = clusters_cap;
  }
  const int items = m_tiles * n_pairs * splits;
  const int clusters = items < clusters_cap ? items : clusters_cap;
  const double kslice_row = static_cast<double>(kb_per_split) * BK * 4;
  const TileOrder ord = pick_tile_order(m_tiles, n_pairs, BM * kslice_row * 2, 2 * BN * kslice_row * (BEXACT ? 1 : 2),
                                        clusters, l2);
  kern<<<2 * clusters, NUM_THREADS, L::DYN_BYTES, stream>>>(mAh, mAl, mBh, mBl, g.C, g.M, g.ldc, g.c_split_stride,
                                                            ord, n_tiles, splits, total_kb, kb_per_split, BEXACT ? 2 : 1,
                                                    g.out_col_scale, g.a_tile_scale, g.a_tiles, 3);
  CNMF_CUDA_CHECK(cudaGetLastError());
  return 0;
}

}

int gemm_fixed_splits(int Kd, int f16) {
  const int bke = f16 ? 2 * BK : BK;
  const int total_kb = (Kd + bke - 1) / bke;
  const int s = std::max(1, std::min(16, (total_kb + 63) / 64));
  return gemm_effective_splits(Kd, s, f16);
}

int gemm_effective_splits(int Kd, int splits, int f16) {
  const int bke = f16 ? 2 * BK : BK;
  const int total_kb = (Kd + bke - 1) / bke;
  if (splits < 1) splits = 1;
  if (splits > total_kb) splits = total_kb;
  int kb_per_split = (total_kb + splits - 1) / splits;
  if (f16 && (kb_per_split & 1)) ++kb_per_split;
  return (total_kb + kb_per_split - 1) / kb_per_split;
}

static int pick_tile_n(const GemmArgs& g) {
  if (!g.b_exact) return 128;
  int dev = 0, sms = 0;
  CNMF_CUDA_CHECK(cudaGetDevice(&dev));
  CNMF_CUDA_CHECK(cudaDeviceGetAttribute(&sms, cudaDevAttrMultiProcessorCount, dev));
  const long long pairs = std::max(1, sms / 2);
  const long long m_items = static_cast<long long>((g.M + BM - 1) / BM) * g.splits_effective;
  const int cols = std::min(g.ldc, (g.N + 31) / 32 * 32);
  auto cost = [&](int bn, int per_item) {
    const long long items = m_items * (((cols + bn - 1) / bn + 1) / 2);
    return (items + pairs - 1) / pairs * per_item;
  };
  const long long narrow = cost(128, 100);
  int best = 128;
  long long best_cost = narrow * 98 / 100;
  for (const auto& [bn, per_item] : {std::pair<int, int>{168, 125}, std::pair<int, int>{192, 142}}) {
    const long long c = cost(bn, per_item);
    if (c <= best_cost) { best_cost = c; best = bn; }
  }
  return best;
}

int gemm_tf32x3(const GemmArgs& g, cudaStream_t stream) {
  CNMF_REQUIRE(g.M > 0 && g.N > 0 && g.Kd > 0, "gemm: empty problem");
  CNMF_REQUIRE(g.lda % 4 == 0 && g.ldb % 4 == 0 && g.ldc % 4 == 0, "gemm: leading dimensions must be multiples of 4 floats");
  CNMF_REQUIRE((reinterpret_cast<uintptr_t>(g.A_hi) | reinterpret_cast<uintptr_t>(g.A_lo) |
                reinterpret_cast<uintptr_t>(g.B_hi) | reinterpret_cast<uintptr_t>(g.B_lo) |
                reinterpret_cast<uintptr_t>(g.C) | reinterpret_cast<uintptr_t>(g.out_col_scale)) % 16 == 0,
               "gemm: pointers must be 16-byte aligned");
  CNMF_REQUIRE(g.tile_n == 0 || g.tile_n == 128 || (g.b_exact && (g.tile_n == 168 || g.tile_n == 192)),
               "gemm: tile_n must be 0 (the launcher's choice), 128, or 168 / 192 with an exact B");
  const int bn = g.tile_n ? g.tile_n : pick_tile_n(g);
  if (g.f16) {
    CNMF_REQUIRE(g.b_exact, "gemm: the fp16 path needs an exact B operand");
    CNMF_REQUIRE(g.lda % 8 == 0 && g.ldb % 8 == 0, "gemm: fp16 leading dimensions must be multiples of 8 halves");
    CNMF_REQUIRE(!g.a_tile_scale || g.a_tiles * 512 >= g.Kd, "gemm: a_tiles does not cover the reduction length");
    if (bn == 168) return launch<168, 4, true, true>(g, stream);
    if (bn == 192) return launch<192, 4, true, true>(g, stream);
    return launch<128, 4, true, true>(g, stream);
  }
  if (g.b_exact) {
    if (bn == 168) return launch<168, 4, true, false>(g, stream);
    if (bn == 192) return launch<192, 4, true, false>(g, stream);
    return launch<128, 4, true, false>(g, stream);
  }
  return launch<128, 3, false, false>(g, stream);
}

}
```

### cnmf_b200/csrc/nmf_engine.cu

```cuda
#include <algorithm>
#include <cmath>
#include <cstring>

#include "engine.h"
#include "gemm.h"
#include "nmf_kernels.cuh"

namespace cnmf {

DataView make_view(const cnmf_dataset_s* d, bool transposed) {
  const bool f16 = d->form == Form::F16_EXACT;
  Operand X{d->X, f16 ? static_cast<const float*>(d->X_h16) : d->X_hi, d->X_lo, d->n_rows, d->n_cols, d->ld_c};
  Operand Xt{d->Xt, f16 ? static_cast<const float*>(d->Xt_h16) : d->Xt_hi, d->Xt_lo, d->n_cols, d->n_rows, d->ld_r};
  DataView v;
  if (!transposed) {
    v.B_rows = X; v.B_cols = Xt;
    v.n_r = d->n_rows; v.n_c = d->n_cols; v.ld_r = d->ld_r; v.ld_c = d->ld_c;
  } else {
    v.B_rows = Xt; v.B_cols = X;
    v.n_r = d->n_cols; v.n_c = d->n_rows; v.ld_r = d->ld_c; v.ld_c = d->ld_r;
  }
  v.sum = d->sum;
  v.sum_sq = d->sum_sq;
  v.form = d->sparse ? Form::FP32 : d->form;
  v.scale_r = d->sparse ? nullptr : transposed ? d->col_scale : d->row_scale;
  v.scale_c = d->sparse ? nullptr : transposed ? d->row_scale : d->col_scale;
  v.X64 = d->X64;
  v.transposed = transposed;
  return v;
}

int form_gemm(Form form, GemmArgs g, const float* A, const float* A_hi, const float* A_lo, const float* a_tile_scale,
              const Operand& B, const float* out_scale, cudaStream_t s) {
  switch (form) {
    case Form::FP32:
      g.A_hi = A; g.B_hi = B.full;
      return gemm_fp32_simt(g, s);
    case Form::TF32:
      g.B_lo = B.lo;
      break;
    case Form::F16_EXACT:
      g.f16 = 1; g.a_tile_scale = a_tile_scale; g.a_tiles = (g.lda + 511) / 512;
      [[fallthrough]];
    case Form::TF32_EXACT:
      g.b_exact = 1; g.out_col_scale = out_scale;
      break;
    case Form::FP64:
      set_last_error("float64 datasets run their products through gemm_f64");
      return -3;
  }
  g.A_hi = A_hi; g.A_lo = A_lo; g.B_hi = B.hi;
  return gemm_tf32x3(g, s);
}

int make_pieces(Form form, const float* F, int rows, int n, int ld, const float* scale, float* hi, float* lo,
                float* tile_scale, cudaStream_t s) {
  switch (form) {
    case Form::FP32:
    case Form::FP64: return 0;
    case Form::F16_EXACT: return launch_emit_f16(F, rows, n, ld, scale, hi, lo, tile_scale, (ld + 511) / 512, s);
    default: return launch_split_scaled(F, hi, lo, rows, ld, scale, s);
  }
}

GemmPlan view_gemm_plan(const DataView& v, int side, int SK) {
  const int f16 = v.form == Form::F16_EXACT ? 1 : 0;
  return side == 0 ? GemmPlan{gemm_fixed_splits(v.n_c, f16), (long long)SK * v.ld_r}
                   : GemmPlan{gemm_fixed_splits(v.n_r, f16), (long long)SK * v.ld_c};
}

int view_gemm(cnmf_handle_s* h, const DataView& v, int side, const float* F, const float* F_hi, const float* F_lo,
              const float* tile_scale, int SK, float* C, const GemmPlan& plan, cudaStream_t s) {
  const Operand& B = side == 0 ? v.B_rows : v.B_cols;
  GemmArgs g{};
  g.M = SK; g.N = B.rows; g.Kd = B.cols;
  g.lda = side == 0 ? v.ld_c : v.ld_r;
  g.ldb = B.ld;
  g.ldc = side == 0 ? v.ld_r : v.ld_c;
  g.C = C;
  g.c_split_stride = plan.split_stride;
  g.splits = plan.splits;
  g.splits_effective = plan.splits;
  h->launches += 1;
  const int slot = h->prof_begin(s, 2.0 * (double)g.M * (double)g.N * (double)g.Kd);
  const int rc = form_gemm(v.form, g, F, F_hi, F_lo, tile_scale, B, side == 0 ? v.scale_r : v.scale_c, s);
  h->prof_end(s, slot);
  return rc;
}

int solve_batched(cnmf_handle_s* h, const DataView& v, SolveIO& io, const cnmf_nmf_params& p, cudaStream_t s) {
  const int R0 = io.R;
  if (v.form == Form::FP64) return solve_batched_f64(h, v, io, p, s);
  if (p.beta_loss != CNMF_LOSS_FROBENIUS) return solve_batched_beta(h, v, io, p, s);
  CNMF_REQUIRE(R0 > 0 && (int)io.ks.size() == R0, "solve: bad restart list");
  CNMF_REQUIRE(p.solver == CNMF_SOLVER_MU || p.solver == CNMF_SOLVER_CD, "solve: unknown solver");
  CNMF_REQUIRE(p.max_iter >= 1, "solve: max_iter must be >= 1");
  CNMF_REQUIRE(!io.num_rows || !io.update_cols, "solve: a caller-computed row product needs update_cols = false");
  const bool tf32 = v.form != Form::FP32;
  const bool f16 = v.form == Form::F16_EXACT;
  const bool mu = p.solver == CNMF_SOLVER_MU;

  std::vector<int> off0(R0), s_off(R0), s_k(io.ks), s_rid(R0);
  int SK0 = 0, kmax = 0;
  for (int r = 0; r < R0; ++r) {
    CNMF_REQUIRE(io.ks[r] >= 1 && io.ks[r] <= KMAX, "solve: n_components must be in [1, 32] on the CUDA path");
    off0[r] = s_off[r] = SK0;
    s_rid[r] = r;
    SK0 += io.ks[r];
    kmax = std::max(kmax, io.ks[r]);
  }
  int R = R0, SK = SK0;
  const int kp = kmax <= 16 ? 16 : 32;
  auto pack_offsets = [&](const std::vector<int>& kk, std::vector<int>& offs) -> int {
    int pos = 0;
    offs.clear();
    for (int k : kk) {
      offs.push_back(pos);
      pos += k;
    }
    return pos;
  };
  const int tile = upd_tile_cols(kp);
  int cpb_r = 0, cpb_c = 0, chunks_r = 0, chunks_c = 0;
  auto plan_blocks = [&](int r_live) {
    cpb_r = pick_cols_per_block(v.n_r, r_live, 4 * tile, tile, h->sm_count * 8);
    cpb_c = pick_cols_per_block(v.n_c, r_live, 4 * tile, tile, h->sm_count * 8);
    chunks_r = (v.n_r + cpb_r - 1) / cpb_r;
    chunks_c = (v.n_c + cpb_c - 1) / cpb_c;
  };
  const int gcpb_r = pick_cols_per_block(v.n_r, R0, 8192, 1024, h->sm_count * 2);
  const int gcpb_c = pick_cols_per_block(v.n_c, R0, 8192, 1024, h->sm_count * 2);
  const int chunks_cap = std::max((v.n_r + tile - 1) / tile, (v.n_c + tile - 1) / tile);
  const int gchunks_max = std::max((v.n_r + gcpb_r - 1) / gcpb_r, (v.n_c + gcpb_c - 1) / gcpb_c);
  size_t fused_part_slots = 0;
  for (int r = 1; r <= R0; ++r) {
    plan_blocks(r);
    fused_part_slots = std::max(fused_part_slots, (size_t)r * std::max(chunks_r, chunks_c));
  }
  plan_blocks(R0);
  const bool fuse = kp == 16;

  int* d_meta = static_cast<int*>(h->dev_buf("solve.meta", sizeof(int) * 8 * R0));
  double* d_state = static_cast<double*>(h->dev_buf("solve.state", sizeof(double) * 8 * R0));
  double* d_gram = static_cast<double*>(h->dev_buf("solve.gram", sizeof(double) * 2 * R0 * KMAX * KMAX));
  const size_t gpart_elems = std::max((size_t)R0 * std::max(gchunks_max, std::max((v.n_r + 1023) / 1024, (v.n_c + 1023) / 1024)),
                                     fused_part_slots) * kp * kp;
  double* d_gram_part = static_cast<double*>(h->dev_buf("solve.gram_part", sizeof(double) * 2 * gpart_elems));
  double* d_scal_part = static_cast<double*>(h->dev_buf("solve.scal_part", sizeof(double) * 2 * (size_t)R0 * chunks_cap));
  if (!d_meta || !d_state || !d_gram || !d_gram_part || !d_scal_part) return -2;

  GemmPlan plan_r, plan_c;
  float *NUMr = nullptr, *NUMc = nullptr;
  auto plan_gemms = [&]() -> int {
    plan_r = view_gemm_plan(v, 0, SK);
    if (io.num_rows) plan_r.splits = 1;
    plan_c = view_gemm_plan(v, 1, SK);
    return 0;
  };
  plan_gemms();
  {
    const size_t need_r = (size_t)plan_r.splits * (size_t)SK0 * v.ld_r;
    const size_t need_c = (size_t)plan_c.splits * (size_t)SK0 * v.ld_c;
    NUMr = io.num_rows ? const_cast<float*>(io.num_rows) : static_cast<float*>(h->dev_buf("solve.NUMr", sizeof(float) * need_r));
    NUMc = io.update_cols ? static_cast<float*>(h->dev_buf("solve.NUMc", sizeof(float) * need_c)) : nullptr;
    if (!NUMr || (io.update_cols && !NUMc)) return -2;
  }

  int* d_off = d_meta;
  int* d_k = d_meta + R0;
  int* d_rid = d_meta + 2 * R0;
  int* d_done = d_meta + 3 * R0;
  int* d_niter = d_meta + 4 * R0;
  int* d_ticket = d_meta + 5 * R0;
  auto upload_slots = [&]() -> int {
    std::vector<int> hm(3 * R0, 0);
    std::memcpy(hm.data(), s_off.data(), sizeof(int) * R);
    std::memcpy(hm.data() + R0, s_k.data(), sizeof(int) * R);
    std::memcpy(hm.data() + 2 * R0, s_rid.data(), sizeof(int) * R);
    CNMF_CUDA_CHECK(cudaMemcpyAsync(d_meta, hm.data(), sizeof(int) * 3 * R0, cudaMemcpyHostToDevice, s));
    CNMF_CUDA_CHECK(cudaStreamSynchronize(s));
    return 0;
  };
  CNMF_TRY(upload_slots());
  CNMF_CUDA_CHECK(cudaMemsetAsync(d_done, 0, sizeof(int) * 3 * R0, s));
  CNMF_CUDA_CHECK(cudaMemsetAsync(d_state, 0, sizeof(double) * 8 * R0, s));
  ConvState st{d_state, d_state + R0, d_state + 2 * R0, d_done, d_niter};
  double* d_crossA = d_state + 3 * R0;
  double* d_crossB = d_state + 4 * R0;
  double* d_gramR = d_gram;
  double* d_gramC = d_gram + (size_t)R0 * KMAX * KMAX;
  double* d_scalA = d_scal_part;
  double* d_scalB = d_scal_part + (size_t)R0 * chunks_cap;
  double* d_gpartR = d_gram_part;
  double* d_gpartC = d_gram_part + gpart_elems;

  float *wFr = io.Fr, *wFr_hi = nullptr, *wFr_lo = nullptr, *wFc = io.Fc, *wFc_hi = nullptr, *wFc_lo = nullptr;
  if (tf32) {
    const size_t nr = (size_t)SK0 * v.ld_r, nc = (size_t)SK0 * v.ld_c;
    wFr_hi = static_cast<float*>(h->dev_buf("solve.Fr_hi", nr * 4));
    wFr_lo = static_cast<float*>(h->dev_buf("solve.Fr_lo", nr * 4));
    wFc_hi = static_cast<float*>(h->dev_buf("solve.Fc_hi", nc * 4));
    wFc_lo = static_cast<float*>(h->dev_buf("solve.Fc_lo", nc * 4));
    if (!wFr_hi || !wFr_lo || !wFc_hi || !wFc_lo) return -2;
  }
  float *aFr = nullptr, *aFr_hi = nullptr, *aFr_lo = nullptr, *aFc = nullptr, *aFc_hi = nullptr, *aFc_lo = nullptr;
  float *resFr = nullptr, *resFc = nullptr;
  bool compacted = false;

  auto bm = [&]() { return BatchMeta{d_off, d_k, d_rid, d_done, R, kp}; };
  float* d_rs_r = nullptr;
  float* d_rs_c = nullptr;
  if (f16) {
    d_rs_r = static_cast<float*>(h->dev_buf("solve.rowscale_r", sizeof(float) * (size_t)SK0 * ((v.ld_r + 511) / 512)));
    d_rs_c = static_cast<float*>(h->dev_buf("solve.rowscale_c", sizeof(float) * (size_t)SK0 * ((v.ld_c + 511) / 512)));
    if (!d_rs_r || !d_rs_c) return -2;
  }
  const bool upd_pieces = tf32 && !f16;
  const int ktiles_r = (v.ld_r + 511) / 512, ktiles_c = (v.ld_c + 511) / 512;
  const bool emit_in_update = f16 && kp == 16 && io.update_cols;
  auto fr = [&]() {
    FactorView f{};
    f.F = wFr; f.F_hi = upd_pieces ? wFr_hi : nullptr; f.F_lo = upd_pieces ? wFr_lo : nullptr;
    f.n = v.n_r; f.ld = v.ld_r; f.piece_scale = v.scale_r;
    if (emit_in_update) { f.P_hi = wFr_hi; f.P_mid = wFr_lo; f.tile_scale = d_rs_r; f.n_ktiles = ktiles_r; }
    f.cpb = cpb_r; f.gcpb = gcpb_r;
    return f;
  };
  auto fc = [&]() {
    FactorView f{};
    f.F = wFc; f.F_hi = upd_pieces ? wFc_hi : nullptr; f.F_lo = upd_pieces ? wFc_lo : nullptr;
    f.n = v.n_c; f.ld = v.ld_c; f.piece_scale = v.scale_c;
    if (emit_in_update) { f.P_hi = wFc_hi; f.P_mid = wFc_lo; f.tile_scale = d_rs_c; f.n_ktiles = ktiles_c; }
    f.cpb = cpb_c; f.gcpb = gcpb_c;
    if (!io.update_cols) { f.F_hi = nullptr; f.F_lo = nullptr; }
    return f;
  };
  auto gram_full = [&](const FactorView& f, int side_is_c) -> int {
    h->launches += 2;
    double* part = side_is_c ? d_gpartC : d_gpartR;
    CNMF_TRY(launch_gram_partial(f, bm(), part, s));
    return launch_finalize(part, side_is_c ? d_gramC : d_gramR, nullptr, nullptr, gram_chunks(f), bm(), s);
  };
  auto gram_after = [&](const FactorView& f, int side_is_c) -> int {
    return fuse ? 0 : gram_full(f, side_is_c);
  };
  auto pieces = [&](int side_is_c) -> int {
    return side_is_c ? make_pieces(v.form, wFc, SK, v.n_c, v.ld_c, v.scale_c, wFc_hi, wFc_lo, d_rs_c, s)
                     : make_pieces(v.form, wFr, SK, v.n_r, v.ld_r, v.scale_r, wFr_hi, wFr_lo, d_rs_r, s);
  };
  auto emit_pieces = [&](int side_is_c) -> int {
    if (!f16) return 0;
    h->launches += 1;
    const int n = side_is_c ? v.n_c : v.n_r;
    const int slot = h->prof_begin(s, 8.0 * (double)SK * (double)n, 1);
    const int rc = pieces(side_is_c);
    h->prof_end(s, slot);
    return rc;
  };
  auto upd_bytes = [&](int n_items, int nsplit, int piece_floats) {
    return 4.0 * (double)SK * (double)n_items * (double)(2 + nsplit + piece_floats);
  };
  auto update = [&](bool cd, const FactorView& f, const float* NUM, const GemmPlan& pl, const double* gram_in, float l1,
                    float l2, const FusedOut& out) -> int {
    h->launches += 1;
    const int slot = h->prof_begin(s, upd_bytes(f.n, pl.splits, f.F_hi ? 2 : ((f.P_hi && out.gram_part) ? 1 : 0)), 1);
    const int rc = cd ? launch_cd_update(f, NUM, pl.splits, pl.split_stride, gram_in, bm(), l1, l2, out, s)
                      : launch_mu_update(f, NUM, pl.splits, pl.split_stride, gram_in, bm(), l1, l2, out, s);
    h->prof_end(s, slot);
    if (rc != 0 || !io.update_cols) return rc;
    if (f.P_hi && out.gram_part) return 0;
    return emit_pieces(f.F == wFc ? 1 : 0);
  };
  auto fused_out = [&](int side_is_c, bool want_gram, double* scal_part, double* scal) {
    FusedOut o{};
    if (want_gram && fuse) {
      o.gram_part = side_is_c ? d_gpartC : d_gpartR;
      o.gram = side_is_c ? d_gramC : d_gramR;
    }
    o.scal_part = scal_part;
    o.scal = scal;
    o.counter = d_ticket;
    return o;
  };
  auto finalize_scal = [&](const double* part, double* out, int chunks) -> int {
    h->launches += 1;
    return launch_finalize(nullptr, nullptr, part, out, chunks, bm(), s);
  };
  auto gemm_rows = [&]() -> int {
    if (io.num_rows) return 0;
    return view_gemm(h, v, 0, wFc, wFc_hi, wFc_lo, d_rs_c, SK, NUMr, plan_r, s);
  };
  auto gemm_cols = [&]() -> int {
    return view_gemm(h, v, 1, wFr, wFr_hi, wFr_lo, d_rs_r, SK, NUMc, plan_c, s);
  };

  constexpr int GATHER_SLOTS = 12;
  int* h_gidx = static_cast<int*>(h->host_buf("solve.gather_idx", sizeof(int) * 3 * (size_t)R0 * GATHER_SLOTS));
  int* d_gidx = static_cast<int*>(h->dev_buf("solve.gather_didx", sizeof(int) * 3 * (size_t)R0 * GATHER_SLOTS));
  if (!h_gidx || !d_gidx) return -2;
  int gslot = 0;
  auto gather = [&](const float* src, float* dst, const std::vector<int>& so, const std::vector<int>& dof,
                    const std::vector<int>& kk, int ld) -> int {
    const int cnt = (int)kk.size();
    if (cnt == 0 || !src || !dst) return 0;
    if (gslot == GATHER_SLOTS) {
      CNMF_CUDA_CHECK(cudaStreamSynchronize(s));
      gslot = 0;
    }
    int* hm = h_gidx + (size_t)gslot * 3 * R0;
    int* dm = d_gidx + (size_t)gslot * 3 * R0;
    ++gslot;
    std::memcpy(hm, so.data(), sizeof(int) * cnt);
    std::memcpy(hm + R0, dof.data(), sizeof(int) * cnt);
    std::memcpy(hm + 2 * R0, kk.data(), sizeof(int) * cnt);
    CNMF_CUDA_CHECK(cudaMemcpyAsync(dm, hm, sizeof(int) * 3 * R0, cudaMemcpyHostToDevice, s));
    h->launches += 1;
    return launch_gather_rows(src, dm, dst, dm + R0, dm + 2 * R0, cnt, ld, s);
  };

  const double normX2 = v.sum_sq;
  double* d_cd_err = d_state + 7 * R0;
  auto cd_final_error = [&]() -> int {
    int* d_zero = static_cast<int*>(h->dev_buf("solve.zero", sizeof(int) * 2 * R0));
    if (!d_zero) return -2;
    CNMF_CUDA_CHECK(cudaMemsetAsync(d_zero, 0, sizeof(int) * 2 * R0, s));
    BatchMeta bm0{d_off, d_k, d_rid, d_zero, R, kp};
    h->launches += 7;
    CNMF_TRY(launch_gram_partial(fr(), bm0, d_gpartR, s));
    CNMF_TRY(launch_gram_partial(fc(), bm0, d_gpartC, s));
    CNMF_TRY(launch_finalize(d_gpartR, d_gramR, nullptr, nullptr, gram_chunks(fr()), bm0, s));
    CNMF_TRY(launch_finalize(d_gpartC, d_gramC, nullptr, nullptr, gram_chunks(fc()), bm0, s));
    if (io.update_cols) {
      CNMF_TRY(launch_cross(fc(), NUMc, plan_c.splits, plan_c.split_stride, bm0, d_scalB, s));
      CNMF_TRY(launch_finalize(nullptr, nullptr, d_scalB, d_crossB, chunks_c, bm0, s));
    } else {
      CNMF_TRY(launch_cross(fr(), NUMr, plan_r.splits, plan_r.split_stride, bm0, d_scalA, s));
      CNMF_TRY(launch_finalize(nullptr, nullptr, d_scalA, d_crossB, chunks_r, bm0, s));
    }
    ConvState scratch{d_state + 5 * R0, d_state + 6 * R0, d_cd_err, d_zero, d_zero + R0};
    return launch_mu_check(scratch, d_crossB, d_gramR, d_gramC, normX2, bm0, 0, 0.0, p.max_iter, s);
  };

  std::vector<int> h_done(R0, 0);
  auto maybe_compact = [&]() -> int {
    if (!io.update_cols) return 0;
    int live_rows = 0;
    for (int sl = 0; sl < R; ++sl)
      if (!h_done[s_rid[sl]]) live_rows += s_k[sl];
    if (live_rows == SK || live_rows == 0) return 0;
    std::vector<int> lk, lo;
    for (int sl = 0; sl < R; ++sl)
      if (!h_done[s_rid[sl]]) lk.push_back(s_k[sl]);
    const int new_rows = pack_offsets(lk, lo);
    const bool saves_tile = (new_rows + 127) / 128 < (SK + 127) / 128;
    if (!saves_tile && new_rows > SK - SK / 8) return 0;
    if (!mu) CNMF_TRY(cd_final_error());
    if (!aFr) {
      const size_t nr = (size_t)SK0 * v.ld_r, nc = (size_t)SK0 * v.ld_c;
      aFr = static_cast<float*>(h->dev_buf("solve.alt.Fr", nr * 4));
      aFc = static_cast<float*>(h->dev_buf("solve.alt.Fc", nc * 4));
      resFr = static_cast<float*>(h->dev_buf("solve.res.Fr", nr * 4));
      resFc = static_cast<float*>(h->dev_buf("solve.res.Fc", nc * 4));
      if (!aFr || !aFc || !resFr || !resFc) return -2;
      if (tf32) {
        aFr_hi = static_cast<float*>(h->dev_buf("solve.alt.Fr_hi", nr * 4));
        aFr_lo = static_cast<float*>(h->dev_buf("solve.alt.Fr_lo", nr * 4));
        aFc_hi = static_cast<float*>(h->dev_buf("solve.alt.Fc_hi", nc * 4));
        aFc_lo = static_cast<float*>(h->dev_buf("solve.alt.Fc_lo", nc * 4));
        if (!aFr_hi || !aFr_lo || !aFc_hi || !aFc_lo) return -2;
      }
    }
    std::vector<int> f_src, f_dst, f_k, l_src, l_dst, l_k, n_off, n_k, n_rid;
    for (int sl = 0; sl < R; ++sl) {
      const int rid = s_rid[sl];
      if (h_done[rid]) {
        f_src.push_back(s_off[sl]); f_dst.push_back(off0[rid]); f_k.push_back(s_k[sl]);
      } else {
        l_src.push_back(s_off[sl]); l_k.push_back(s_k[sl]);
        n_k.push_back(s_k[sl]); n_rid.push_back(rid);
      }
    }
    const int pos = pack_offsets(l_k, l_dst);
    n_off = l_dst;
    CNMF_TRY(gather(wFr, resFr, f_src, f_dst, f_k, v.ld_r));
    CNMF_TRY(gather(wFc, resFc, f_src, f_dst, f_k, v.ld_c));
    CNMF_TRY(gather(wFr, aFr, l_src, l_dst, l_k, v.ld_r));
    CNMF_TRY(gather(wFc, aFc, l_src, l_dst, l_k, v.ld_c));
    if (upd_pieces) {
      CNMF_TRY(gather(wFr_hi, aFr_hi, l_src, l_dst, l_k, v.ld_r));
      CNMF_TRY(gather(wFr_lo, aFr_lo, l_src, l_dst, l_k, v.ld_r));
      CNMF_TRY(gather(wFc_hi, aFc_hi, l_src, l_dst, l_k, v.ld_c));
      CNMF_TRY(gather(wFc_lo, aFc_lo, l_src, l_dst, l_k, v.ld_c));
    }
    std::swap(wFr, aFr); std::swap(wFr_hi, aFr_hi); std::swap(wFr_lo, aFr_lo);
    std::swap(wFc, aFc); std::swap(wFc_hi, aFc_hi); std::swap(wFc_lo, aFc_lo);
    R = (int)n_k.size();
    SK = pos;
    std::copy(n_off.begin(), n_off.end(), s_off.begin());
    std::copy(n_k.begin(), n_k.end(), s_k.begin());
    std::copy(n_rid.begin(), n_rid.end(), s_rid.begin());
    CNMF_TRY(upload_slots());
    gslot = 0;
    plan_gemms();
    plan_blocks(R);
    CNMF_TRY(emit_pieces(0));
    CNMF_TRY(emit_pieces(1));
    compacted = true;
    return 0;
  };

  auto poll_all_done = [&]() -> int {
    CNMF_CUDA_CHECK(cudaMemcpyAsync(h_done.data(), d_done, sizeof(int) * R0, cudaMemcpyDeviceToHost, s));
    CNMF_CUDA_CHECK(cudaStreamSynchronize(s));
    for (int sl = 0; sl < R; ++sl)
      if (!h_done[s_rid[sl]]) return maybe_compact();
    return 1;
  };

  const float l1W = (float)p.l1_reg_W, l2W = (float)p.l2_reg_W, l1H = (float)p.l1_reg_H, l2H = (float)p.l2_reg_H;
  int it = 0;
  if (upd_pieces) {
    CNMF_TRY(pieces(0));
    CNMF_TRY(pieces(1));
    h->launches += 2;
  }
  CNMF_TRY(emit_pieces(0));
  CNMF_TRY(emit_pieces(1));

  if (mu) {
    CNMF_TRY(gram_full(fc(), 1));
    CNMF_TRY(gram_full(fr(), 0));
    if (io.update_cols) {
      CNMF_TRY(gemm_cols());
      h->launches += 1;
      CNMF_TRY(launch_cross(fc(), NUMc, plan_c.splits, plan_c.split_stride, bm(), d_scalB, s));
      CNMF_TRY(finalize_scal(d_scalB, d_crossB, chunks_c));
    } else {
      CNMF_TRY(gemm_rows());
      h->launches += 1;
      CNMF_TRY(launch_cross(fr(), NUMr, plan_r.splits, plan_r.split_stride, bm(), d_scalA, s));
      CNMF_TRY(finalize_scal(d_scalA, d_crossB, chunks_r));
    }
    h->launches += 1;
    CNMF_TRY(launch_mu_check(st, d_crossB, d_gramR, d_gramC, normX2, bm(), 0, p.tol, p.max_iter, s));

    for (it = 1; it <= p.max_iter; ++it) {
      const bool check = (p.tol > 0 && it % 10 == 0) || it == p.max_iter;
      if (io.update_cols) {
        CNMF_TRY(gemm_rows());
        CNMF_TRY(update(false, fr(), NUMr, plan_r, d_gramC, l1W, l2W, fused_out(0, true, nullptr, nullptr)));
        CNMF_TRY(gram_after(fr(), 0));
        CNMF_TRY(gemm_cols());
        CNMF_TRY(update(false, fc(), NUMc, plan_c, d_gramR, l1H, l2H, fused_out(1, true, check ? d_scalB : nullptr, d_crossB)));
        CNMF_TRY(gram_after(fc(), 1));
      } else {
        CNMF_TRY(update(false, fr(), NUMr, plan_r, d_gramC, l1W, l2W, fused_out(0, check, check ? d_scalA : nullptr, d_crossB)));
        if (check) CNMF_TRY(gram_after(fr(), 0));
      }
      if (check) {
        h->launches += 1;
        const double tol_eff = (p.tol > 0 && it % 10 == 0) ? p.tol : -1.0;
        CNMF_TRY(launch_mu_check(st, d_crossB, d_gramR, d_gramC, normX2, bm(), it, tol_eff, p.max_iter, s));
        const int all = poll_all_done();
        if (all < 0) return all;
        if (all) break;
      }
    }
  } else {
    const int poll_every = 4;
    for (it = 1; it <= p.max_iter; ++it) {
      if (it == 1) CNMF_TRY(gram_full(fc(), 1));
      if (io.update_cols || it == 1) CNMF_TRY(gemm_rows());
      CNMF_TRY(update(true, fr(), NUMr, plan_r, d_gramC, l1W, l2W, fused_out(0, io.update_cols, d_scalA, d_crossA)));
      if (io.update_cols) {
        CNMF_TRY(gram_after(fr(), 0));
        CNMF_TRY(gemm_cols());
        CNMF_TRY(update(true, fc(), NUMc, plan_c, d_gramR, l1H, l2H, fused_out(1, true, d_scalB, d_crossB)));
        CNMF_TRY(gram_after(fc(), 1));
      }
      h->launches += 1;
      CNMF_TRY(launch_cd_check(st, d_crossA, io.update_cols ? d_crossB : nullptr, bm(), it, p.tol, p.max_iter, s));
      if (it % poll_every == 0 || it == p.max_iter) {
        const int all = poll_all_done();
        if (all < 0) return all;
        if (all) break;
      }
    }
  }

  double* d_err = st.last;
  if (!mu) {
    CNMF_TRY(cd_final_error());
    d_err = d_cd_err;
  }

  if (compacted) {
    std::vector<int> so(s_off.begin(), s_off.begin() + R), ko(s_k.begin(), s_k.begin() + R), dof(R);
    for (int sl = 0; sl < R; ++sl) dof[sl] = off0[s_rid[sl]];
    CNMF_TRY(gather(wFr, resFr, so, dof, ko, v.ld_r));
    CNMF_TRY(gather(wFc, resFc, so, dof, ko, v.ld_c));
    CNMF_CUDA_CHECK(cudaMemcpyAsync(io.Fr, resFr, (size_t)SK0 * v.ld_r * 4, cudaMemcpyDeviceToDevice, s));
    CNMF_CUDA_CHECK(cudaMemcpyAsync(io.Fc, resFc, (size_t)SK0 * v.ld_c * 4, cudaMemcpyDeviceToDevice, s));
  }

  io.n_iter.assign(R0, 0);
  io.last.assign(R0, 0.0);
  io.err.assign(R0, 0.0);
  CNMF_CUDA_CHECK(cudaMemcpyAsync(io.n_iter.data(), d_niter, sizeof(int) * R0, cudaMemcpyDeviceToHost, s));
  CNMF_CUDA_CHECK(cudaMemcpyAsync(io.last.data(), st.last, sizeof(double) * R0, cudaMemcpyDeviceToHost, s));
  CNMF_CUDA_CHECK(cudaMemcpyAsync(io.err.data(), d_err, sizeof(double) * R0, cudaMemcpyDeviceToHost, s));
  CNMF_CUDA_CHECK(cudaStreamSynchronize(s));
  return 0;
}

}
```

### cnmf_b200/engine.py

```python
import ctypes

import numpy as np

from . import _lib
from ._lib import (LOSS_FROBENIUS, LOSS_ITAKURA_SAITO, LOSS_KULLBACK_LEIBLER, NmfParams, PRECISION_FP32,
                   PRECISION_F16X2, PRECISION_FP64, PRECISION_TF32X3, PRECISION_TF32X3_GENERAL, SOLVER_CD, SOLVER_MU,
                   check, f32c, f64c, ptr)

_DEFAULT_PRECISION = PRECISION_F16X2


def precision_code(p):
    if p in (PRECISION_FP32, PRECISION_TF32X3, PRECISION_TF32X3_GENERAL, PRECISION_F16X2, PRECISION_FP64):
        return p
    return {"fp32": PRECISION_FP32, "tf32x3": PRECISION_TF32X3, "tf32x3-general": PRECISION_TF32X3_GENERAL,
            "f16x2": PRECISION_F16X2, "fp64": PRECISION_FP64}[p]


def is_fp64(precision):
    return precision is not None and precision_code(precision) == PRECISION_FP64


def check_fp64_supported(precision, beta_loss="frobenius", rng="device"):
    if not is_fp64(precision):
# ... 5 lines not shown
        raise NotImplementedError("cnmf_b200: precision='fp64' draws its random starts on the device; rng='host' "
                                  "serves the float precisions only")


def _params_precision(p):
    return PRECISION_TF32X3 if p in (PRECISION_TF32X3_GENERAL, PRECISION_F16X2) else p


def check_supported(ks=None, init="random", beta_loss="frobenius"):
    from .nndsvd import INITS
    if ks is not None:
        bad = [int(k) for k in np.atleast_1d(ks) if int(k) < 1 or int(k) > _lib.MAX_COMPONENTS]
        if bad:
            raise ValueError("cnmf_b200: n_components must be in [1, %d] on the CUDA path (got %s); the batched "
                             "kernels keep a restart's K x K Gram matrix and its K factor values per item on chip"
                             % (_lib.MAX_COMPONENTS, bad))
    if init is not None and init not in INITS:
        raise ValueError("Invalid init parameter: got %r instead of one of %r" % (init, (None,) + INITS))
    loss_code(beta_loss)


def init_code(init, ks, n_samples, n_features):
    from .nndsvd import resolve_init
    which = {resolve_init(init, int(k), n_samples, n_features) for k in np.atleast_1d(ks)}
    if len(which) > 1:
        raise ValueError("init=%r resolves to %s for different n_components of one call; split the call by K"
                         % (init, sorted(which)))
    return _lib.INIT_CODES[which.pop()]


def nndsvd_starts(X, ks, seeds, init, dtype=np.float32):
    import concurrent.futures
    import os
    from .nndsvd import nndsvd_init, resolve_init
    ks = [int(k) for k in ks]
    n, g = X.shape
    offs = np.concatenate([[0], np.cumsum(ks)]).astype(np.int64)
    W0 = np.empty((int(offs[-1]), n), dtype)
    H0 = np.empty((int(offs[-1]), g), dtype)

    def one(r):
        which = resolve_init(init, ks[r], n, g)
        if which == "random":
            raise ValueError("init=None resolves to 'random' for n_components > min(shape): use the seeded device generator")
        W, H = nndsvd_init(X, ks[r], int(seeds[r]), which)
        W0[offs[r]:offs[r + 1]] = W.T
        H0[offs[r]:offs[r + 1]] = H

    workers = max(1, min(8, (os.cpu_count() or 1) // 4, len(ks)))
    if workers == 1:
        for r in range(len(ks)):
            one(r)
    else:
        with concurrent.futures.ThreadPoolExecutor(max_workers=workers) as ex:
            list(ex.map(one, range(len(ks))))
    return W0, H0


def make_params(nmf_kwargs, n_samples, n_features, precision, for_refit=False):
    solver = nmf_kwargs.get("solver", "mu")
    beta = nmf_kwargs.get("beta_loss", "frobenius")
    loss = loss_code(beta)
    if loss != LOSS_FROBENIUS and solver != "mu":
        raise ValueError("Invalid beta_loss parameter: solver %r does not handle beta_loss = %r" % (solver, beta))
    if not for_refit:
        check_supported(None, nmf_kwargs.get("init", "random"), beta)
    if solver not in ("mu", "cd"):
        raise ValueError("solver must be 'mu' or 'cd'")
    alpha_W = float(nmf_kwargs.get("alpha_W", 0.0))
    alpha_H = nmf_kwargs.get("alpha_H", 0.0)
    alpha_H = alpha_W if alpha_H == "same" else float(alpha_H)
    l1_ratio = float(nmf_kwargs.get("l1_ratio", 0.0))
    p = NmfParams()
    p.solver = SOLVER_MU if solver == "mu" else SOLVER_CD
    p.precision = _params_precision(precision_code(precision))
    rng = nmf_kwargs.get("rng", "device")
    if rng not in ("device", "host"):
        raise ValueError("rng must be 'device' or 'host'")
    check_fp64_supported(precision, beta, rng)
    p.reserved = 1 if rng == "host" else 0
    p.max_iter = int(nmf_kwargs.get("max_iter", 1000))
    p.tol = float(nmf_kwargs.get("tol", 1e-4))
    p.l1_reg_W = n_features * alpha_W * l1_ratio
    p.l1_reg_H = n_samples * alpha_H * l1_ratio
    p.l2_reg_W = n_features * alpha_W * (1.0 - l1_ratio)
    p.l2_reg_H = n_samples * alpha_H * (1.0 - l1_ratio)
    p.beta_loss = loss
    return p


def loss_code(beta):
    table = {"frobenius": LOSS_FROBENIUS, 2: LOSS_FROBENIUS, "kullback-leibler": LOSS_KULLBACK_LEIBLER,
             1: LOSS_KULLBACK_LEIBLER, "itakura-saito": LOSS_ITAKURA_SAITO, 0: LOSS_ITAKURA_SAITO}
    try:
        return table[beta]
    except (KeyError, TypeError):
        raise NotImplementedError("cnmf_b200: beta_loss must be 'frobenius' (2), 'kullback-leibler' (1) or "
                                  "'itakura-saito' (0) on the CUDA path (got %r)" % (beta,))


def _csr_arrays(C, dtype):
    if not C.has_canonical_format:
        C = C.copy()
        C.sum_duplicates()
    return (np.ascontiguousarray(C.indptr, dtype=np.int64), np.ascontiguousarray(C.indices, dtype=np.int32),
            np.ascontiguousarray(C.data, dtype=dtype))


class Engine:

    def __init__(self, device=0):
        self.lib = _lib.load()
        self._h = ctypes.c_void_p()
        check(self.lib.cnmf_create(ctypes.byref(self._h), int(device)))
        self.device = int(device)

    def close(self):
        if self._h:
            self.lib.cnmf_destroy(self._h)
            self._h = ctypes.c_void_p()

    def __del__(self):
        try:
            self.close()
        except Exception:
            pass

    @property
    def launch_count(self):
        return int(self.lib.cnmf_launch_count(self._h))

    def profile(self, on=True):
        check(self.lib.cnmf_profile_enable(self._h, 1 if on else 0))

    def profile_get(self, kernel_class=0):
        ms, n, fl = ctypes.c_double(), ctypes.c_longlong(), ctypes.c_double()
        check(self.lib.cnmf_profile_get_class(self._h, int(kernel_class), ctypes.byref(ms), ctypes.byref(n),
                                              ctypes.byref(fl)))
        return ms.value, int(n.value), fl.value

    def mem_info(self):
        v = [ctypes.c_longlong() for _ in range(3)]
        check(self.lib.cnmf_mem_info(self._h, *[ctypes.byref(x) for x in v]))
        return tuple(int(x.value) for x in v)

    def last_timing(self):
        v = [ctypes.c_double() for _ in range(4)]
        check(self.lib.cnmf_last_timing(self._h, *[ctypes.byref(x) for x in v]))
        return dict(zip(("rng_ms", "h2d_ms", "solve_ms", "d2h_ms"), [x.value for x in v]))

    def nndsvd_chunk_limit(self, max_restarts):
        check(self.lib.cnmf_nndsvd_chunk_limit(self._h, int(max_restarts)))

    def dataset(self, X, precision=_DEFAULT_PRECISION, stream=None):
        return Dataset(self, X, precision, stream)

    def sparse_dataset(self, X, precision=_DEFAULT_PRECISION, stream=None):
        if is_fp64(precision):
            raise NotImplementedError("cnmf_b200: precision='fp64' needs a dense dataset; sparse (CSC) datasets hold "
                                      "float32 values")
        import scipy.sparse as sp
        out = ctypes.c_void_p()
        if sp.issparse(X) and X.format == "csr":
            n, g = X.shape
            row_ptr, col_idx, vals = _csr_arrays(sp.csr_matrix(X, dtype=np.float32), np.float32)
            check(self.lib.cnmf_dataset_create_csr(self._h, n, g, int(row_ptr[-1]), ptr(row_ptr), ptr(col_idx),
                                                   ptr(vals), precision_code(precision), stream, ctypes.byref(out)))
            return Dataset(self, None, precision, _handle=out, sparse=True)
        C = sp.csc_matrix(X, dtype=np.float32)
        if not C.has_canonical_format:
            C = C.copy()
            C.sum_duplicates()
        n, g = C.shape
        col_ptr = np.ascontiguousarray(C.indptr, dtype=np.int64)
        row_idx = np.ascontiguousarray(C.indices, dtype=np.int32)
        vals = np.ascontiguousarray(C.data, dtype=np.float32)
        check(self.lib.cnmf_dataset_create_csc(self._h, n, g, int(col_ptr[-1]), ptr(col_ptr), ptr(row_idx), ptr(vals),
                                               precision_code(precision), stream, ctypes.byref(out)))
        return Dataset(self, None, precision, _handle=out, sparse=True)

    def dataset_from_device(self, X_ptr, n_rows, n_cols, ld, precision=_DEFAULT_PRECISION, stream=None):
        out = ctypes.c_void_p()
        check(self.lib.cnmf_dataset_create(self._h, ctypes.c_void_p(X_ptr), int(n_rows), int(n_cols), int(ld), 1,
                                           precision_code(precision), stream, ctypes.byref(out)))
        return Dataset(self, None, precision, _handle=out)

    def dense_dataset_bytes(self, n_rows, n_cols, precision=_DEFAULT_PRECISION):
        peak = ctypes.c_longlong()
        check(self.lib.cnmf_dataset_dense_bytes(int(n_rows), int(n_cols), precision_code(precision), ctypes.byref(peak)))
        return int(peak.value)

    def gemm_abt(self, A, B, precision=PRECISION_TF32X3, splits=1, reps=1, b_exact=False, k_scale=None,
                 out_col_scale=None, tile_n=0):
        A, B = f32c(A), f32c(B)
        M, Kd = A.shape
        N = B.shape[0]
        assert B.shape[1] == Kd
        ks = None if k_scale is None else f32c(k_scale)
        cs = None if out_col_scale is None else f32c(out_col_scale)
        assert ks is None or ks.shape == (Kd,)
        assert cs is None or cs.shape == (N,)
        C = np.empty((M, N), np.float32)
        ms = ctypes.c_float(0)
        pc = precision_code(precision)
        pc = PRECISION_TF32X3 if pc == PRECISION_TF32X3_GENERAL else pc
        check(self.lib.cnmf_gemm_abt_host(self._h, pc, ptr(A), ptr(B), M, N, Kd, splits, 1 if b_exact else 0,
                                          ptr(ks), ptr(cs), int(tile_n), ptr(C), reps, ctypes.byref(ms), None))
        return C, float(ms.value)

    def update_step(self, ks, rids, done, n, F, num, gram_in, solver="mu", pieces=None, gram=None, want_scalar=False,
                    cpb_tiles=1, l1=0.0, l2=0.0, piece_scale=None, pieces_hi=None, pieces_lo=None, tile_scale=None,
                    gram_out=None, scal_out=None):
        ks = np.ascontiguousarray(ks, np.int32)
        rids = np.ascontiguousarray(rids, np.int32)
        done = np.ascontiguousarray(done, np.int32)
        F = f32c(F).copy()
        SK, ld = F.shape
        assert SK == int(ks.sum()) and ld == -(-int(n) // 32) * 32
        num = f32c(num).reshape(-1, SK, ld) if num is not None else None
        gram_in = np.ascontiguousarray(gram_in, np.float64)
        n_rids = len(done)
        assert gram_in.shape == (n_rids, 32, 32)
        pmode = {None: _lib.UNIT_PIECES_NONE, "tf32": _lib.UNIT_PIECES_TF32, "f16": _lib.UNIT_PIECES_F16}[pieces]
        gmode = {None: _lib.UNIT_GRAM_NONE, "fused": _lib.UNIT_GRAM_FUSED, "standalone": _lib.UNIT_GRAM_STANDALONE}[gram]
        smode = {None: _lib.UNIT_SOLVER_NONE, "mu": SOLVER_MU, "cd": SOLVER_CD}[solver]
        pdt = np.float16 if pieces == "f16" else np.float32
        hi = lo = ts = None
        if pieces is not None:
            hi = np.zeros((SK, ld), pdt) if pieces_hi is None else np.ascontiguousarray(pieces_hi, pdt).copy()
            lo = np.zeros((SK, ld), pdt) if pieces_lo is None else np.ascontiguousarray(pieces_lo, pdt).copy()
        if pieces == "f16":
            nt = (ld + 511) // 512
            ts = np.zeros((SK, nt), np.float32) if tile_scale is None else f32c(tile_scale).copy()
        g_out = np.zeros((n_rids, 32, 32)) if gram_out is None else np.ascontiguousarray(gram_out, np.float64).copy()
        s_out = np.zeros(n_rids) if scal_out is None else np.ascontiguousarray(scal_out, np.float64).copy()
        ps = None if piece_scale is None else f32c(piece_scale)
        assert ps is None or ps.shape == (ld,)
        a = _lib.UpdateStepArgs()
        a.n_slots, a.n_rids, a.n, a.cpb_tiles = len(ks), n_rids, int(n), int(cpb_tiles)
        a.ks, a.rids, a.done = ptr(ks), ptr(rids), ptr(done)
        a.solver, a.pieces, a.gram, a.want_scalar = smode, pmode, gmode, 1 if want_scalar else 0
        a.nsplit = 1 if num is None else num.shape[0]
        a.l1, a.l2 = float(l1), float(l2)
        a.F, a.num, a.gram_in, a.piece_scale = ptr(F), ptr(num), ptr(gram_in), ptr(ps)
        a.pieces_hi, a.pieces_lo, a.tile_scale = ptr(hi), ptr(lo), ptr(ts)
        a.gram_out, a.scal_out = ptr(g_out), ptr(s_out)
        check(self.lib.cnmf_update_step_host(self._h, ctypes.byref(a), None))
        return dict(F=F, hi=hi, lo=lo, tile_scale=ts, gram=g_out, scal=s_out)

    def beta_step(self, ks, rids, done, side, loss, D, F_own, F_other, n_items, n_contract, op="update", l1=0.0, l2=0.0,
                  last=None, totals=None):
        ks = np.ascontiguousarray(ks, np.int32)
        rids = np.ascontiguousarray(rids, np.int32)
        done = np.ascontiguousarray(done, np.int32)
        SK, n_rids = int(ks.sum()), len(done)
        ld_i, ld_k = -(-int(n_items) // 32) * 32, -(-int(n_contract) // 32) * 32
        D = f32c(D)
        F = f32c(F_own).copy()
        Fo = f32c(F_other)
        assert D.shape == (n_contract, ld_i) and F.shape == (SK, ld_i) and Fo.shape == (SK, ld_k)
        lcode = {"kullback-leibler": LOSS_KULLBACK_LEIBLER, "itakura-saito": LOSS_ITAKURA_SAITO,
                 "frobenius": LOSS_FROBENIUS}[loss]
        oth = np.zeros(SK)
        lo = np.zeros(n_rids) if last is None else np.ascontiguousarray(last, np.float64).copy()
        tt = np.zeros((n_rids, 2)) if totals is None else np.ascontiguousarray(totals, np.float64).copy()
        assert lo.shape == (n_rids,) and tt.shape == (n_rids, 2)
        a = _lib.BetaStepArgs()
        a.n_slots, a.n_rids = len(ks), n_rids
        a.ks, a.rids, a.done = ptr(ks), ptr(rids), ptr(done)
        a.op = {"update": _lib.UNIT_BETA_UPDATE, "divergence": _lib.UNIT_BETA_DIVERGENCE}[op]
        a.side = {"W": _lib.UNIT_SIDE_W, "H": _lib.UNIT_SIDE_H}[side]
        a.loss, a.n_items, a.n_contract = lcode, int(n_items), int(n_contract)
        a.l1, a.l2 = float(l1), float(l2)
        a.D, a.F_own, a.F_other = ptr(D), ptr(F), ptr(Fo)
        a.oth_sum, a.last, a.totals = ptr(oth), ptr(lo), ptr(tt)
        check(self.lib.cnmf_beta_step_host(self._h, ctypes.byref(a), None))
        return dict(F=F, oth_sum=oth, last=lo, totals=tt)

    def update_step_f64(self, ks, rids, done, n, F, op="update", num=None, gram_in=None, solver="mu", want_scalar=False,
                        l1=0.0, l2=0.0, gram_out=None, scal_out=None):
        ks = np.ascontiguousarray(ks, np.int32)
        rids = np.ascontiguousarray(rids, np.int32)
        done = np.ascontiguousarray(done, np.int32)
        F = f64c(F).copy()
        SK, ld = F.shape
        assert SK == int(ks.sum()) and ld == -(-int(n) // 32) * 32
        num = None if num is None else f64c(num)
        assert num is None or num.shape == (SK, ld)
        n_rids = len(done)
        gin = None if gram_in is None else f64c(gram_in)
        assert gin is None or gin.shape == (n_rids, 32, 32)
        g_out = np.zeros((n_rids, 32, 32)) if gram_out is None else f64c(gram_out).copy()
        s_out = np.zeros(n_rids) if scal_out is None else f64c(scal_out).copy()
        a = _lib.UpdateStepF64Args()
        a.n_slots, a.n_rids, a.n = len(ks), n_rids, int(n)
        a.ks, a.rids, a.done = ptr(ks), ptr(rids), ptr(done)
        a.op = {"update": _lib.UNIT_F64_UPDATE, "gram": _lib.UNIT_F64_GRAM, "cross": _lib.UNIT_F64_CROSS}[op]
        a.solver = {"mu": SOLVER_MU, "cd": SOLVER_CD}[solver]
        a.want_scalar = 1 if want_scalar else 0
        a.l1, a.l2 = float(l1), float(l2)
        a.F, a.num, a.gram_in, a.gram_out, a.scal_out = ptr(F), ptr(num), ptr(gin), ptr(g_out), ptr(s_out)
        check(self.lib.cnmf_update_step_f64_host(self._h, ctypes.byref(a), None))
        return dict(F=F, gram=g_out, scal=s_out)

    def conv_check(self, ks, rids, solver, it, tol, max_iter, done, n_iter, err0, prev, last, normX2=0.0, cross=None,
                   gramA=None, gramB=None, violA=None, violB=None):
        ks = np.ascontiguousarray(ks, np.int32)
        rids = np.ascontiguousarray(rids, np.int32)
        st = dict(done=np.array(done, np.int32), n_iter=np.array(n_iter, np.int32), err0=np.array(err0, np.float64),
                  prev=np.array(prev, np.float64), last=np.array(last, np.float64))
        n_rids = len(st["done"])
        assert all(len(v) == n_rids for v in st.values())
        opt = {k: (None if v is None else f64c(v)) for k, v in
               dict(cross=cross, gramA=gramA, gramB=gramB, violA=violA, violB=violB).items()}
        a = _lib.ConvCheckArgs()
        a.n_slots, a.n_rids = len(ks), n_rids
        a.ks, a.rids = ptr(ks), ptr(rids)
        a.solver = {"mu": SOLVER_MU, "cd": SOLVER_CD}[solver]
        a.it, a.max_iter, a.tol, a.normX2 = int(it), int(max_iter), float(tol), float(normX2)
        for k, v in opt.items():
            setattr(a, k, ptr(v))
        for k, v in st.items():
            setattr(a, k, ptr(v))
        check(self.lib.cnmf_conv_check_host(self._h, ctypes.byref(a), None))
        return st


class Dataset:

    def __init__(self, engine, X, precision=_DEFAULT_PRECISION, stream=None, _handle=None, sparse=False):
        self.engine = engine
        self.lib = engine.lib
        self.precision = precision_code(precision)
        self.fp64 = self.precision == PRECISION_FP64
        self.sparse = sparse
        self._d = ctypes.c_void_p()
        if _handle is not None:
            self._d = _handle
        elif hasattr(X, "toarray"):
            import scipy.sparse as sp
            n, g = X.shape
            row_ptr, col_idx, vals = _csr_arrays(sp.csr_matrix(X), np.float64 if self.fp64 else np.float32)
            nnz = int(row_ptr[-1])
            if self.fp64:
                check(self.lib.cnmf_dataset_create_from_csr_f64(engine._h, n, g, nnz, ptr(row_ptr), ptr(col_idx),
                                                                ptr(vals), stream, ctypes.byref(self._d)))
            else:
                check(self.lib.cnmf_dataset_create_from_csr(engine._h, n, g, nnz, ptr(row_ptr), ptr(col_idx), ptr(vals),
                                                            self.precision, stream, ctypes.byref(self._d)))
        else:
            if self.fp64:
                X = f64c(X)
                n, g = X.shape
                check(self.lib.cnmf_dataset_create_f64(engine._h, ptr(X), n, g, g, 0, stream, ctypes.byref(self._d)))
            else:
                X = f32c(X)
                n, g = X.shape
                check(self.lib.cnmf_dataset_create(engine._h, ptr(X), n, g, g, 0, self.precision, stream,
                                                   ctypes.byref(self._d)))
        n, g = ctypes.c_int(), ctypes.c_int()
        check(self.lib.cnmf_dataset_shape(self._d, ctypes.byref(n), ctypes.byref(g)))
# ... 253 lines not shown
```

### include/cnmf_b200.h

```cpp
#ifndef CNMF_B200_H
#define CNMF_B200_H

#include <stdint.h>

#ifdef __cplusplus
extern "C" {
#endif

#define CNMF_B200_ABI_VERSION 19
#define CNMF_MAX_COMPONENTS 32

typedef struct cnmf_handle_s* cnmf_handle_t;
typedef struct cnmf_dataset_s* cnmf_dataset_t;

enum { CNMF_SOLVER_MU = 0, CNMF_SOLVER_CD = 1 };
enum { CNMF_PRECISION_FP32 = 0, CNMF_PRECISION_TF32X3 = 1, CNMF_PRECISION_TF32X3_GENERAL = 2,
       CNMF_PRECISION_F16X2 = 3,
       CNMF_PRECISION_FP64 = 4 };

enum { CNMF_LOSS_FROBENIUS = 0, CNMF_LOSS_KULLBACK_LEIBLER = 1, CNMF_LOSS_ITAKURA_SAITO = 2 };

enum { CNMF_INIT_RANDOM = 0, CNMF_INIT_NNDSVD = 1, CNMF_INIT_NNDSVDA = 2, CNMF_INIT_NNDSVDAR = 3 };

typedef struct cnmf_nmf_params {
  int32_t solver;
  int32_t precision;
  int32_t max_iter;
  int32_t reserved;
  double tol;
  double l1_reg_W, l2_reg_W, l1_reg_H, l2_reg_H;
  int32_t beta_loss;
  int32_t reserved2;
} cnmf_nmf_params;

int cnmf_abi_version(void);
const char* cnmf_last_error(void);
int cnmf_create(cnmf_handle_t* out, int device);
int cnmf_destroy(cnmf_handle_t h);
long long cnmf_launch_count(cnmf_handle_t h);
int cnmf_mem_info(cnmf_handle_t h, long long* free_bytes, long long* total_bytes, long long* cached_bytes);
long long cnmf_solve_bytes_per_row(cnmf_dataset_t d);

int cnmf_profile_enable(cnmf_handle_t h, int on);
int cnmf_profile_get(cnmf_handle_t h, double* gemm_ms, long long* gemm_launches, double* gemm_flops);
int cnmf_profile_get_class(cnmf_handle_t h, int kernel_class, double* ms, long long* launches, double* work);

int cnmf_last_timing(cnmf_handle_t h, double* rng_ms, double* h2d_ms, double* solve_ms, double* d2h_ms);

int cnmf_dataset_create(cnmf_handle_t h, const float* X, int n_rows, int n_cols, long long ld,
                        int src_is_device, int precision, void* stream, cnmf_dataset_t* out);
int cnmf_dataset_create_from_csr(cnmf_handle_t h, int n_rows, int n_cols, long long nnz, const int64_t* row_ptr,
                                 const int32_t* col_idx, const float* values, int precision, void* stream,
                                 cnmf_dataset_t* out);
int cnmf_dataset_create_csc(cnmf_handle_t h, int n_rows, int n_cols, long long nnz, const int64_t* col_ptr,
                            const int32_t* row_idx, const float* values, int precision, void* stream,
                            cnmf_dataset_t* out);
int cnmf_dataset_create_csr(cnmf_handle_t h, int n_rows, int n_cols, long long nnz, const int64_t* row_ptr,
                            const int32_t* col_idx, const float* values, int precision, void* stream,
                            cnmf_dataset_t* out);
int cnmf_dataset_dense_bytes(int n_rows, int n_cols, int precision, long long* peak);
int cnmf_dataset_from_columns(cnmf_dataset_t src, const int32_t* cols_host, const float* col_scale_host,
                              int n_cols, void* stream, cnmf_dataset_t* out);
int cnmf_dataset_destroy(cnmf_dataset_t d);
int cnmf_dataset_shape(cnmf_dataset_t d, int* n_rows, int* n_cols);
int cnmf_dataset_ld(cnmf_dataset_t d, int* ld_rows, int* ld_cols);
int cnmf_dataset_sums(cnmf_dataset_t d, double* sum, double* sum_sq);
int cnmf_dataset_min(cnmf_dataset_t d, float* min_host, void* stream);
int cnmf_dataset_is_exact(cnmf_dataset_t d);
int cnmf_dataset_col_stats(cnmf_dataset_t d, double* mean_host, double* var_host, void* stream);

int cnmf_dataset_row_sums(cnmf_dataset_t d, double* row_sums_host, void* stream);
int cnmf_dataset_scaled_col_stats(cnmf_dataset_t d, const double* row_scale_host, double* mean_host, double* var_host,
                                  void* stream);
int cnmf_dataset_tpm_stats(cnmf_dataset_t d, double target_sum, double* totals_host, double* mean_host,
                           double* var_host, void* stream);
int cnmf_dataset_scale_rows(cnmf_dataset_t src, const float* row_scale_host, void* stream, cnmf_dataset_t* out);

int cnmf_random_init_host(uint32_t seed, double avg, int n_samples, int n_features, int k,
                          float* Wt, long long ldW, float* H, long long ldH);

int cnmf_random_init_dev(cnmf_dataset_t d, int n_restarts, const int32_t* ks, const uint32_t* seeds, float* Wt_dev,
                         float* H_dev, void* stream);

int cnmf_nndsvd_init_dev(cnmf_dataset_t d, int n_restarts, const int32_t* ks, const uint32_t* seeds, int init,
                         float* Wt_dev, float* H_dev, void* stream);
int cnmf_nndsvd_chunk_limit(cnmf_handle_t h, int max_restarts);
int cnmf_nndsvd_gemm_host(cnmf_dataset_t d, int to_genes, int M, const double* A_host, double* C_host, void* stream);

int cnmf_dataset_create_f64(cnmf_handle_t h, const double* X, int n_rows, int n_cols, long long ld, int src_is_device,
                            void* stream, cnmf_dataset_t* out);
int cnmf_dataset_create_from_csr_f64(cnmf_handle_t h, int n_rows, int n_cols, long long nnz, const int64_t* row_ptr,
                                     const int32_t* col_idx, const double* values, void* stream, cnmf_dataset_t* out);
int cnmf_dataset_from_columns_f64(cnmf_dataset_t src, const int32_t* cols_host, const double* divisor_host, int n_cols,
                                  void* stream, cnmf_dataset_t* out);
int cnmf_factorize_f64(cnmf_dataset_t d, int n_restarts, const int32_t* ks, const uint32_t* seeds,
                       const cnmf_nmf_params* params, double* spectra_host, double* usages_host, int32_t* n_iter_host,
                       double* err_host, void* stream);
int cnmf_factorize_init_f64(cnmf_dataset_t d, int n_restarts, const int32_t* ks, const double* Wt0_host,
                            const double* H0_host, const cnmf_nmf_params* params, double* spectra_host,
                            double* usages_host, int32_t* n_iter_host, double* err_host, void* stream);
int cnmf_refit_f64(cnmf_dataset_t d, int transposed, int k, const double* fixed_host, const cnmf_nmf_params* params,
                   double* out_host, int32_t* n_iter_host, double* err_host, void* stream);
int cnmf_project_rows_f64(cnmf_dataset_t d, int k, const double* Ut_host, double* out_host, void* stream);

int cnmf_factorize(cnmf_dataset_t d, int n_restarts, const int32_t* ks, const uint32_t* seeds,
                   const cnmf_nmf_params* params, float* spectra_host, float* usages_host,
                   int32_t* n_iter_host, double* err_host, void* stream);

int cnmf_factorize_seeds_dev(cnmf_dataset_t d, int n_restarts, const int32_t* ks, const uint32_t* seeds,
                             const cnmf_nmf_params* params, float* spectra_dev, long long ld_out,
                             int32_t* n_iter_host, double* err_host, void* stream);

int cnmf_allgather_spectra(void* nccl_comm, const float* local_dev, long long rows_per_rank, long long ld,
                           float* merged_dev, void* stream);
int cnmf_comm_unique_id(char* id_out_128);
int cnmf_comm_create(cnmf_handle_t h, const char* id_128, int rank, int world, void** comm_out);
int cnmf_comm_destroy(void* nccl_comm);

int cnmf_factorize_init(cnmf_dataset_t d, int n_restarts, const int32_t* ks, const float* Wt0_host,
                        const float* H0_host, const cnmf_nmf_params* params, float* spectra_host,
                        float* usages_host, int32_t* n_iter_host, double* err_host, void* stream);

int cnmf_factorize_dev(cnmf_dataset_t d, int n_restarts, const int32_t* ks, const float* Wt0_dev,
                       const float* H0_dev, const cnmf_nmf_params* params, float* spectra_dev,
                       int32_t* n_iter_host, double* err_host, void* stream);

int cnmf_refit(cnmf_dataset_t d, int transposed, int k, const float* fixed_host, const cnmf_nmf_params* params,
               float* out_host, int32_t* n_iter_host, double* err_host, void* stream);

int cnmf_project_rows(cnmf_dataset_t d, int k, const float* Ut_host, float* out_host, void* stream);

int cnmf_gemm_abt_host(cnmf_handle_t h, int precision, const float* A, const float* B, int M, int N, int Kd,
                       int splits, int b_exact, const float* k_scale, const float* out_col_scale, int tile_n, float* C,
                       int reps, float* ms_out, void* stream);

enum { CNMF_UNIT_SOLVER_NONE = -1 };
enum { CNMF_UNIT_PIECES_NONE = 0, CNMF_UNIT_PIECES_TF32 = 1, CNMF_UNIT_PIECES_F16 = 2 };
enum { CNMF_UNIT_GRAM_NONE = 0, CNMF_UNIT_GRAM_FUSED = 1, CNMF_UNIT_GRAM_STANDALONE = 2 };
typedef struct cnmf_update_step_args {
  int32_t n_slots;
  int32_t n_rids;
  const int32_t* ks;
  const int32_t* rids;
  const int32_t* done;
  int32_t n;
  int32_t cpb_tiles;
  int32_t solver;
  int32_t pieces;
  int32_t gram;
  int32_t want_scalar;
  int32_t nsplit;
  float l1, l2;
  float* F;
  const float* num;
  const double* gram_in;
  const float* piece_scale;
  void* pieces_hi;
  void* pieces_lo;
  float* tile_scale;
  double* gram_out;
  double* scal_out;
} cnmf_update_step_args;
int cnmf_update_step_host(cnmf_handle_t h, const cnmf_update_step_args* args, void* stream);

enum { CNMF_UNIT_BETA_UPDATE = 0, CNMF_UNIT_BETA_DIVERGENCE = 1 };
enum { CNMF_UNIT_SIDE_W = 0, CNMF_UNIT_SIDE_H = 1 };
typedef struct cnmf_beta_step_args {
  int32_t n_slots;
  int32_t n_rids;
  const int32_t* ks;
  const int32_t* rids;
  const int32_t* done;
  int32_t op;
  int32_t side;
  int32_t loss;
  int32_t n_items, n_contract;
  float l1, l2;
  const float* D;
  float* F_own;
  const float* F_other;
  double* oth_sum;
  double* last;
  double* totals;
} cnmf_beta_step_args;
int cnmf_beta_step_host(cnmf_handle_t h, const cnmf_beta_step_args* args, void* stream);

enum { CNMF_UNIT_F64_UPDATE = 0, CNMF_UNIT_F64_GRAM = 1, CNMF_UNIT_F64_CROSS = 2 };
typedef struct cnmf_update_step_f64_args {
  int32_t n_slots;
  int32_t n_rids;
  const int32_t* ks;
  const int32_t* rids;
  const int32_t* done;
  int32_t n;
  int32_t op;
  int32_t solver;
  int32_t want_scalar;
  double l1, l2;
  double* F;
  const double* num;
  const double* gram_in;
  double* gram_out;
  double* scal_out;
} cnmf_update_step_f64_args;
int cnmf_update_step_f64_host(cnmf_handle_t h, const cnmf_update_step_f64_args* args, void* stream);

typedef struct cnmf_conv_check_args {
  int32_t n_slots;
  int32_t n_rids;
  const int32_t* ks;
  const int32_t* rids;
  int32_t solver;
  int32_t it, max_iter;
  double tol, normX2;
  const double* cross;
  const double* gramA;
  const double* gramB;
  const double* violA;
  const double* violB;
  int32_t* done;
  int32_t* n_iter;
  double* err0;
  double* prev;
  double* last;
} cnmf_conv_check_args;
int cnmf_conv_check_host(cnmf_handle_t h, const cnmf_conv_check_args* args, void* stream);

enum { CNMF_FORM_FP32 = 0, CNMF_FORM_TF32 = 1, CNMF_FORM_TF32_EXACT = 2, CNMF_FORM_F16_EXACT = 3, CNMF_FORM_FP64 = 4 };
int cnmf_dataset_form(cnmf_dataset_t d);
enum { CNMF_OPERAND_X = 0, CNMF_OPERAND_XT = 1, CNMF_OPERAND_X_HI = 2, CNMF_OPERAND_X_LO = 3, CNMF_OPERAND_XT_HI = 4,
       CNMF_OPERAND_XT_LO = 5, CNMF_OPERAND_X_H16 = 6, CNMF_OPERAND_XT_H16 = 7, CNMF_OPERAND_ROW_SCALE = 8,
       CNMF_OPERAND_COL_SCALE = 9, CNMF_OPERAND_CSC_COL_PTR = 10, CNMF_OPERAND_CSC_ROW_IDX = 11,
       CNMF_OPERAND_CSC_VALUES = 12 };
int cnmf_dataset_operand_host(cnmf_dataset_t d, int which, void* out_host, long long bytes);
int cnmf_dataset_gemm_host(cnmf_dataset_t d, int transposed, int side, int SK, const float* F_host, float* out_host,
                           int* splits_out);

int cnmf_l2_normalize_rows(cnmf_handle_t h, float* S_dev, int R, int G, int ld, void* stream);
int cnmf_local_density(cnmf_handle_t h, const float* S_dev, int R, int G, int ld, int n_neighbors,
                       float* density_dev, float* D_dev, void* stream);
int cnmf_col_stats_dev(cnmf_handle_t h, const float* S_dev, int R, int G, int ld, double* mean_host,
                       double* var_host, void* stream);
int cnmf_gather_rows(cnmf_handle_t h, const float* src_dev, int ld_src, const int32_t* idx_host, int n, int G,
                     float* dst_dev, int ld_dst, void* stream);
int cnmf_sq_dists_to_rows(cnmf_handle_t h, const float* S_dev, int R, int G, int ld, const int32_t* idx_host,
                          int n_c, float* out_host, void* stream);
int cnmf_kmeans_assign(cnmf_handle_t h, const float* S_dev, int R, int G, int ld, const float* centers_host, int K,
                       int32_t* labels_dev, double* sums_host, int32_t* counts_host, float* mind_dev,
                       int32_t* n_changed_host, double* inertia_host, void* stream);
int cnmf_kmeans_step(cnmf_handle_t h, const float* S_dev, int R, int G, int ld, int K, const float* C32_cur_dev,
                     const double* C64_cur_dev, double* C64_new_dev, float* C32_new_dev, int32_t* labels_dev,
                     float* mind_dev, double* sums_dev, int32_t* counts_dev, int32_t* n_changed_host,
                     int32_t* any_empty_host, double* shift_host, void* stream);
int cnmf_kmeans_fit(cnmf_handle_t h, const float* S_dev, int R, int G, int ld, int K, int n_init, int max_iter,
                    double tol_abs, const int32_t* first_idx_host, const double* uniforms_host, int n_trials,
                    int32_t* labels_host, double* inertia_host, int32_t* n_iter_host, int32_t* needs_host_path,
                    void* stream);
int cnmf_cluster_dist_sums(cnmf_handle_t h, const float* S_dev, int R, int G, int ld, const int32_t* labels_dev,
                           int K, double* sums_host, void* stream);
int cnmf_cluster_median(cnmf_handle_t h, const float* S_dev, int R, int G, int ld, const int32_t* labels_dev, int K,
                        float* M_dev, int ldm, void* stream);

int cnmf_l2_normalize_rows_f64(cnmf_handle_t h, double* S_dev, int R, int G, int ld, void* stream);
int cnmf_local_density_f64(cnmf_handle_t h, const double* S_dev, int R, int G, int ld, int n_neighbors,
                           double* density_dev, double* D_dev, void* stream);
int cnmf_col_stats_dev_f64(cnmf_handle_t h, const double* S_dev, int R, int G, int ld, double* mean_host,
                           double* var_host, void* stream);
int cnmf_gather_rows_f64(cnmf_handle_t h, const double* src_dev, int ld_src, const int32_t* idx_host, int n, int G,
                         double* dst_dev, int ld_dst, void* stream);
int cnmf_sq_dists_to_rows_f64(cnmf_handle_t h, const double* S_dev, int R, int G, int ld, const int32_t* idx_host,
                              int n_c, double* out_host, void* stream);
int cnmf_kmeans_assign_f64(cnmf_handle_t h, const double* S_dev, int R, int G, int ld, const double* centers_host,
                           int K, int32_t* labels_dev, double* sums_host, int32_t* counts_host, double* mind_dev,
                           int32_t* n_changed_host, double* inertia_host, void* stream);
int cnmf_kmeans_step_f64(cnmf_handle_t h, const double* S_dev, int R, int G, int ld, int K, const double* C64_cur_dev,
                         double* C64_new_dev, int32_t* labels_dev, double* mind_dev, double* sums_dev,
                         int32_t* counts_dev, int32_t* n_changed_host, int32_t* any_empty_host, double* shift_host,
                         void* stream);
int cnmf_kmeans_fit_f64(cnmf_handle_t h, const double* S_dev, int R, int G, int ld, int K, int n_init, int max_iter,
                        double tol_abs, const int32_t* first_idx_host, const double* uniforms_host, int n_trials,
                        int32_t* labels_host, double* inertia_host, int32_t* n_iter_host, int32_t* needs_host_path,
                        void* stream);
int cnmf_cluster_dist_sums_f64(cnmf_handle_t h, const double* S_dev, int R, int G, int ld, const int32_t* labels_dev,
                               int K, double* sums_host, void* stream);
int cnmf_cluster_median_f64(cnmf_handle_t h, const double* S_dev, int R, int G, int ld, const int32_t* labels_dev,
                            int K, double* M_dev, int ldm, void* stream);

// ... 17 lines not shown
```

Baseline: 575.0.

## Sum split-K GEMM slices in-kernel instead of writing separate slices

Adds a summed-slices mode to the exact-B tensor-core GEMM. Each cluster walks all K splits of an output tile in sequence and folds later splits into the first with vector red.add, falling back to an exact read-add-store when a value is denormal or out of range. The goal is to cut the size of the split-K output buffer and the slice reads in the downstream MU/CD update and cross kernels. A by-shape heuristic decides when to use it, and a handle knob can force it on or off. The cost is fewer independent work items, so less parallelism, plus atomic traffic and a possible change in summation order.

```diff
diff --git a/cnmf_b200/_lib.py b/cnmf_b200/_lib.py
--- a/cnmf_b200/_lib.py
+++ b/cnmf_b200/_lib.py
@@ -8,6 +8,7 @@
 
 SOLVER_MU, SOLVER_CD = 0, 1
 PRECISION_FP32, PRECISION_TF32X3, PRECISION_TF32X3_GENERAL, PRECISION_F16X2, PRECISION_FP64 = 0, 1, 2, 3, 4
+GEMM_SLICES = {"by_shape": 0, "separate": 1, "summed": 2}
 LOSS_FROBENIUS, LOSS_KULLBACK_LEIBLER, LOSS_ITAKURA_SAITO = 0, 1, 2
 INIT_RANDOM, INIT_NNDSVD, INIT_NNDSVDA, INIT_NNDSVDAR = 0, 1, 2, 3
 INIT_CODES = {"random": INIT_RANDOM, "nndsvd": INIT_NNDSVD, "nndsvda": INIT_NNDSVDA, "nndsvdar": INIT_NNDSVDAR}
@@ -140,7 +141,9 @@
     "cnmf_factorize_dev": (_i, [_vp, _i, _vp, _vp, _vp, _pp(NmfParams), _vp, _vp, _vp, _vp]),
     "cnmf_refit": (_i, [_vp, _i, _i, _vp, _pp(NmfParams), _vp, _pp(_c.c_int32), _pp(_d), _vp]),
     "cnmf_project_rows": (_i, [_vp, _i, _vp, _vp, _vp]),
-    "cnmf_gemm_abt_host": (_i, [_vp, _i, _vp, _vp, _i, _i, _i, _i, _i, _vp, _vp, _i, _vp, _i, _pp(_c.c_float), _vp]),
+    "cnmf_gemm_abt_host": (_i, [_vp, _i, _vp, _vp, _i, _i, _i, _i, _i, _vp, _vp, _i, _i, _vp, _vp, _i, _pp(_c.c_float), _vp]),
+    "cnmf_gemm_slice_sum": (_i, [_vp, _i]),
+    "cnmf_gemm_slice_plan_host": (_i, [_i, _i, _i, _i, _i, _pp(_c.c_int), _pp(_c.c_int), _pp(_c.c_int)]),
     "cnmf_update_step_host": (_i, [_vp, _pp(UpdateStepArgs), _vp]),
     "cnmf_beta_step_host": (_i, [_vp, _pp(BetaStepArgs), _vp]),
     "cnmf_update_step_f64_host": (_i, [_vp, _pp(UpdateStepF64Args), _vp]),
diff --git a/cnmf_b200/csrc/capi_refit.cu b/cnmf_b200/csrc/capi_refit.cu
--- a/cnmf_b200/csrc/capi_refit.cu
+++ b/cnmf_b200/csrc/capi_refit.cu
@@ -518,9 +518,10 @@
 }
 
 int cnmf_gemm_abt_host(cnmf_handle_t h, int precision, const float* A, const float* B, int M, int N, int Kd, int splits,
-                       int b_exact, const float* k_scale, const float* out_col_scale, int tile_n, float* C, int reps,
-                       float* ms_out, void* stream) {
+                       int b_exact, const float* k_scale, const float* out_col_scale, int tile_n, int slice_sum, float* C,
+                       float* C_slices, int reps, float* ms_out, void* stream) {
   CNMF_REQUIRE(h && A && B && C && M > 0 && N > 0 && Kd > 0, "gemm_abt_host: bad arguments");
+  CNMF_REQUIRE(slice_sum >= CNMF_GEMM_SLICES_BY_SHAPE && slice_sum <= CNMF_GEMM_SLICES_SUMMED, "gemm_abt_host: bad slice_sum");
   const bool f16 = precision == CNMF_PRECISION_F16X2;
   CNMF_REQUIRE(!b_exact || f16 || precision == CNMF_PRECISION_TF32X3, "gemm_abt_host: b_exact needs tf32x3 or f16x2");
   const bool exact = f16 || b_exact;
@@ -539,7 +540,13 @@
   float* dBh = static_cast<float*>(h->dev_buf("gemmtest.Bh", nb * 4));
   float* dBl = static_cast<float*>(h->dev_buf("gemmtest.Bl", nb * 4));
   const int se = gemm_effective_splits(Kd, splits, f16 ? 1 : 0);
-  float* dC = static_cast<float*>(h->dev_buf("gemmtest.C", (size_t)se * M * ldc * 4));
+  const int gform = form == Form::F16_EXACT ? 2 : form == Form::TF32_EXACT ? 1 : form == Form::TF32 ? 0 : -1;
+  CNMF_REQUIRE(gform >= 0 || slice_sum != CNMF_GEMM_SLICES_SUMMED, "gemm_abt_host: the fp32 path writes separate slices only");
+  const int sum = se > 1 && gform >= 0 &&
+                  (slice_sum == CNMF_GEMM_SLICES_SUMMED ||
+                   (slice_sum == CNMF_GEMM_SLICES_BY_SHAPE && gemm_pick_sum_slices(M, N, ldc, Kd, se, gform, gemm_device_pairs())));
+  const int outs = sum ? 1 : se;
+  float* dC = static_cast<float*>(h->dev_buf("gemmtest.C", (size_t)outs * M * ldc * 4));
   float* dRs = static_cast<float*>(h->dev_buf("gemmtest.rs", sizeof(float) * (size_t)M * ((lda + 511) / 512)));
   if (!dA || !dB || !dAh || !dAl || !dBh || !dBl || !dC || !dRs) return -2;
   CNMF_CUDA_CHECK(cudaMemsetAsync(dA, 0, na * 4, s));
@@ -563,11 +570,12 @@
   if (f16) CNMF_TRY(launch_to_half(dB, dBh, (long long)nb, s));
   else if (form != Form::FP32) CNMF_TRY(launch_split_tf32(dB, dBh, dBl, (long long)nb, s));
   CNMF_TRY(make_pieces(form, dA, M, Kd, lda, dKs, dAh, dAl, dRs, s));
-  CNMF_CUDA_CHECK(cudaMemsetAsync(dC, 0xff, (size_t)se * M * ldc * 4, s));
+  CNMF_CUDA_CHECK(cudaMemsetAsync(dC, 0xff, (size_t)outs * M * ldc * 4, s));
   GemmArgs g{};
   g.M = M; g.N = N; g.Kd = Kd; g.lda = lda; g.ldb = lda; g.ldc = ldc;
   g.C = dC; g.c_split_stride = (long long)M * ldc; g.splits = splits; g.splits_effective = se;
   g.tile_n = tile_n;
+  g.sum_slices = sum;
   const Operand Bop{dB, dBh, dBl, N, Kd, lda};
   cudaEvent_t e0, e1;
   CNMF_CUDA_CHECK(cudaEventCreate(&e0));
@@ -581,7 +589,7 @@
   }
   h->launches += reps;
   if (rc != 0) return rc;
-  std::vector<float> tmp((size_t)se * M * ldc);
+  std::vector<float> tmp((size_t)outs * M * ldc);
   CNMF_CUDA_CHECK(cudaMemcpyAsync(tmp.data(), dC, tmp.size() * 4, cudaMemcpyDeviceToHost, s));
   CNMF_CUDA_CHECK(cudaStreamSynchronize(s));
   if (ms_out) {
@@ -594,10 +602,30 @@
   for (int m = 0; m < M; ++m)
     for (int n = 0; n < N; ++n) {
       double a = 0.0;
-      for (int z = 0; z < se; ++z) a += tmp[(size_t)z * M * ldc + (size_t)m * ldc + n];
+      for (int z = 0; z < outs; ++z) {
+        const float t = tmp[(size_t)z * M * ldc + (size_t)m * ldc + n];
+        a += t;
+        if (C_slices) C_slices[((size_t)z * M + m) * N + n] = t;
+      }
       C[(size_t)m * N + n] = (float)a;
     }
   return 0;
 }
 
-}
+int cnmf_gemm_slice_sum(cnmf_handle_t h, int mode) {
+  CNMF_REQUIRE(h && mode >= CNMF_GEMM_SLICES_BY_SHAPE && mode <= CNMF_GEMM_SLICES_SUMMED, "gemm_slice_sum: bad arguments");
+  h->gemm_slice_sum = mode;
+  return 0;
+}
+
+int cnmf_gemm_slice_plan_host(int M, int N, int Kd, int form, int pairs, int* splits, int* sum_slices, int* tile_n) {
+  CNMF_REQUIRE(M > 0 && N > 0 && Kd > 0 && form >= 0 && form <= 2 && pairs >= 1 && splits && sum_slices && tile_n,
+               "gemm_slice_plan_host: bad arguments");
+  const int f16 = form == 2 ? 1 : 0, ldc = pad_ld(N);
+  *splits = gemm_fixed_splits(Kd, f16);
+  *sum_slices = gemm_pick_sum_slices(M, N, ldc, Kd, *splits, form, pairs);
+  *tile_n = *sum_slices ? 168 : gemm_pick_tile_n(M, N, ldc, form >= 1 ? 1 : 0, *splits, pairs);
+  return 0;
+}
+
+}
diff --git a/cnmf_b200/csrc/capi_units.cu b/cnmf_b200/csrc/capi_units.cu
--- a/cnmf_b200/csrc/capi_units.cu
+++ b/cnmf_b200/csrc/capi_units.cu
@@ -424,7 +424,7 @@
   CNMF_TRY(require_dense(d, "dataset_gemm"));
   cnmf_handle_s* h = d->h;
   const DataView v = make_view(d, transposed != 0);
-  const GemmPlan plan = view_gemm_plan(v, side, SK);
+  const GemmPlan plan = view_gemm_plan(v, side, SK, CNMF_GEMM_SLICES_SEPARATE);
   *splits_out = plan.splits;
   if (!out_host) return 0;
   CNMF_REQUIRE(F_host, "dataset_gemm: NULL factor");
diff --git a/cnmf_b200/csrc/engine.h b/cnmf_b200/csrc/engine.h
--- a/cnmf_b200/csrc/engine.h
+++ b/cnmf_b200/csrc/engine.h
@@ -32,6 +32,7 @@
   double prof_ms[PROF_CLASSES] = {}, prof_work[PROF_CLASSES] = {};
   long long prof_launches[PROF_CLASSES] = {};
   int nndsvd_chunk_restarts = 0;
+  int gemm_slice_sum = 0;
   double t_rng_ms = 0, t_h2d_ms = 0, t_solve_ms = 0, t_d2h_ms = 0;
   int prof_begin(cudaStream_t s, double work, int cls = 0);
   void prof_end(cudaStream_t s, int slot);
@@ -105,8 +106,10 @@
 struct GemmPlan {
   int splits;
   long long split_stride;
+  int sum_slices;
+  int out_slices() const { return sum_slices ? 1 : splits; }
 };
-GemmPlan view_gemm_plan(const DataView& v, int side, int SK);
+GemmPlan view_gemm_plan(const DataView& v, int side, int SK, int slice_sum);
 int view_gemm(cnmf_handle_s* h, const DataView& v, int side, const float* F, const float* F_hi, const float* F_lo,
               const float* tile_scale, int SK, float* C, const GemmPlan& plan, cudaStream_t s);
 int make_pieces(Form form, const float* F, int rows, int n, int ld, const float* scale, float* hi, float* lo,
diff --git a/cnmf_b200/csrc/gemm.h b/cnmf_b200/csrc/gemm.h
--- a/cnmf_b200/csrc/gemm.h
+++ b/cnmf_b200/csrc/gemm.h
@@ -20,7 +20,14 @@
   const float* a_tile_scale;
   int a_tiles;
   int tile_n;
+  int sum_slices;
 };
+
+int gemm_device_pairs();
+
+int gemm_pick_tile_n(int M, int N, int ldc, int b_exact, int items_per_m_tile, int pairs);
+
+int gemm_pick_sum_slices(int M, int N, int ldc, int Kd, int splits, int form, int pairs);
 
 int gemm_effective_splits(int Kd, int splits, int f16 = 0);
 
diff --git a/cnmf_b200/csrc/gemm_simt.cu b/cnmf_b200/csrc/gemm_simt.cu
--- a/cnmf_b200/csrc/gemm_simt.cu
+++ b/cnmf_b200/csrc/gemm_simt.cu
@@ -101,6 +101,7 @@
   CNMF_REQUIRE(g.lda % 4 == 0 && g.ldb % 4 == 0 && g.ldc % 4 == 0, "gemm: leading dimensions must be multiples of 4 floats");
   const int splits = gemm_effective_splits(g.Kd, g.splits);
   CNMF_REQUIRE(splits == g.splits_effective, "gemm: splits_effective mismatch");
+  CNMF_REQUIRE(!g.sum_slices, "gemm: the fp32 path writes separate split-K slices only");
   const int total_kb = (g.Kd + 31) / 32;
   const int kb_per_split = (total_kb + splits - 1) / splits;
   dim3 grid((g.N + TN - 1) / TN, (g.M + TM - 1) / TM, splits);
diff --git a/cnmf_b200/csrc/gemm_tf32x3.cu b/cnmf_b200/csrc/gemm_tf32x3.cu
--- a/cnmf_b200/csrc/gemm_tf32x3.cu
+++ b/cnmf_b200/csrc/gemm_tf32x3.cu
@@ -105,6 +105,24 @@
 __device__ __forceinline__ void setmaxnreg_dec() { asm volatile("setmaxnreg.dec.sync.aligned.u32 %0;" ::"n"(N)); }
 template <int N>
 __device__ __forceinline__ void setmaxnreg_inc() { asm volatile("setmaxnreg.inc.sync.aligned.u32 %0;" ::"n"(N)); }
+
+__device__ __forceinline__ void red_add_f32x2(float* p, float2 v) {
+  asm volatile("red.global.add.v2.f32 [%0], {%1, %2};" ::"l"(p), "f"(v.x), "f"(v.y) : "memory");
+}
+__device__ __forceinline__ bool flush_safe(float x) { return x == 0.f || (x >= 1.17549435e-38f && x <= 3.40282347e38f); }
+
+__device__ __forceinline__ void fold_or_store(float* p, float2 v, bool fold, bool& unsafe) {
+  const bool ok = flush_safe(v.x) && flush_safe(v.y);
+  if (!fold) {
+    *reinterpret_cast<float2*>(p) = v;
+  } else if (ok && !unsafe) {
+    red_add_f32x2(p, v);
+  } else {
+    const float2 c = __ldcg(reinterpret_cast<const float2*>(p));
+    *reinterpret_cast<float2*>(p) = make_float2(__fadd_rn(c.x, v.x), __fadd_rn(c.y, v.y));
+  }
+  unsafe |= !ok;
+}
 
 __device__ __forceinline__ void wgmma_fence() { asm volatile("wgmma.fence.sync.aligned;" ::: "memory"); }
 __device__ __forceinline__ void wgmma_commit() { asm volatile("wgmma.commit_group.sync.aligned;" ::: "memory"); }
@@ -166,7 +184,11 @@
   np = o.group_n ? q : p;
 }
 
-template <int BN, int STAGES, bool BEXACT, bool F16>
+__device__ __forceinline__ void next_item(int& w, int& zs, int per, int clusters) {
+  if (++zs == per) { zs = 0; w += clusters; }
+}
+
+template <int BN, int STAGES, bool BEXACT, bool F16, bool SUM>
 __device__ __forceinline__ void
 gemm_body(const CUtensorMap& tmA_hi, const CUtensorMap& tmA_lo, const CUtensorMap& tmB_hi, const CUtensorMap& tmB_lo,
           float* __restrict__ C, int M, int ldc, long long c_split_stride,
@@ -201,7 +223,8 @@
   }
   cluster_sync();
 
-  const int items = ord.m_tiles * ord.n_pairs * splits;
+  const int per = SUM ? splits : 1;
+  const int units = ord.m_tiles * ord.n_pairs * (splits / per);
 
   constexpr bool REBALANCE = BN > 128;
   if (wg == 0) {
@@ -211,9 +234,10 @@
       uint32_t phase = 0;
       constexpr uint32_t stage_tx = static_cast<uint32_t>(L::STAGE_BYTES);
       constexpr uint32_t HALF_A = L::A_BYTES / 2;
-      for (int w = cluster; w < items; w += clusters) {
+      for (int w = cluster, zs = 0; w < units; next_item(w, zs, per, clusters)) {
         int mt, np, z;
         decode_item(w, ord, mt, np, z);
+        z += zs;
         const int nt = 2 * np + rank;
         const int kb0 = z * kb_per_split;
         const int kb1 = min(total_kb, kb0 + kb_per_split);
@@ -245,9 +269,11 @@
     if (cw == NC - 1) named_bar_arrive(TURN_BAR, TURN_THREADS);
     int stage = 0;
     uint32_t phase = 0;
-    for (int w = cluster; w < items; w += clusters) {
+    bool unsafe = false;
+    for (int w = cluster, zs = 0; w < units; next_item(w, zs, per, clusters)) {
       int mt, np, z;
       decode_item(w, ord, mt, np, z);
+      z += zs;
       const int nt = 2 * np + rank;
       const int kb0 = z * kb_per_split;
       const int kb1 = min(total_kb, kb0 + kb_per_split);
@@ -307,7 +333,11 @@
       if (nt >= n_tiles) continue;
       constexpr int EPI_J = (BN / 8) % 8 == 0 ? 8 : 7;
       static_assert((BN / 8) % EPI_J == 0, "column groups in whole batches");
-      float* cbase = C + static_cast<long long>(z) * c_split_stride;
+      static_assert(!SUM || (BEXACT && BN == 168), "summed slices: exact-B forms at 168 columns");
+      const bool fold = SUM && z > 0;
+      if (z == 0) unsafe = false;
+      float* crow0 = C + (SUM ? 0LL : static_cast<long long>(z) * c_split_stride) + static_cast<long long>(row0) * ldc;
+      float* crow1 = crow0 + 8LL * ldc;
       const int colq = nt * BN + 2 * (lane & 3);
 #pragma unroll
       for (int j0 = 0; j0 < BN / 8; j0 += EPI_J) {
@@ -322,12 +352,15 @@
           const int col = colq + 8 * (j0 + j);
           if (col >= ldc) continue;
           const float* a = acc + 4 * (j0 + j);
-          if (row0 < M)
-            *reinterpret_cast<float2*>(cbase + static_cast<long long>(row0) * ldc + col) =
-                make_float2(a[0] * sc[j].x, a[1] * sc[j].y);
-          if (row0 + 8 < M)
-            *reinterpret_cast<float2*>(cbase + static_cast<long long>(row0 + 8) * ldc + col) =
-                make_float2(a[2] * sc[j].x, a[3] * sc[j].y);
+          const float2 v0 = make_float2(__fmul_rn(a[0], sc[j].x), __fmul_rn(a[1], sc[j].y));
+          const float2 v1 = make_float2(__fmul_rn(a[2], sc[j].x), __fmul_rn(a[3], sc[j].y));
+          if constexpr (SUM) {
+            if (row0 < M) fold_or_store(crow0 + col, v0, fold, unsafe);
+            if (row0 + 8 < M) fold_or_store(crow1 + col, v1, fold, unsafe);
+          } else {
+            if (row0 < M) *reinterpret_cast<float2*>(crow0 + col) = v0;
+            if (row0 + 8 < M) *reinterpret_cast<float2*>(crow1 + col) = v1;
+          }
         }
       }
     }
@@ -336,15 +369,16 @@
   cluster_sync();
 }
 
-template <int BN, int STAGES, bool BEXACT, bool F16>
+template <int BN, int STAGES, bool BEXACT, bool F16, bool SUM>
 __global__ void __cluster_dims__(2, 1, 1) __launch_bounds__(NUM_THREADS, 1)
 gemm_tf32x3_kernel(const __grid_constant__ CUtensorMap tmA_hi, const __grid_constant__ CUtensorMap tmA_lo,
                    const __grid_constant__ CUtensorMap tmB_hi, const __grid_constant__ CUtensorMap tmB_lo,
                    float* __restrict__ C, int M, int ldc, long long c_split_stride,
                    const TileOrder ord, int n_tiles, int splits, int total_kb, int kb_per_split, int chain_kb,
                    const float* __restrict__ out_scale, const float* __restrict__ a_tile_scale, int a_tiles, int a_gshift) {
-  gemm_body<BN, STAGES, BEXACT, F16>(tmA_hi, tmA_lo, tmB_hi, tmB_lo, C, M, ldc, c_split_stride, ord, n_tiles, splits,
-                                     total_kb, kb_per_split, chain_kb, out_scale, a_tile_scale, a_tiles, a_gshift);
+  gemm_body<BN, STAGES, BEXACT, F16, SUM>(tmA_hi, tmA_lo, tmB_hi, tmB_lo, C, M, ldc, c_split_stride, ord, n_tiles,
+                                          splits, total_kb, kb_per_split, chain_kb, out_scale, a_tile_scale, a_tiles,
+                                          a_gshift);
 }
 
 typedef CUresult (*PFN_encodeTiled)(CUtensorMap*, CUtensorMapDataType, cuuint32_t, void*, const cuuint64_t*,
@@ -425,7 +459,7 @@
   return best;
 }
 
-template <int BN, int STAGES, bool BEXACT, bool F16>
+template <int BN, int STAGES, bool BEXACT, bool F16, bool SUM = false>
 int launch(const GemmArgs& g, cudaStream_t stream) {
   using L = SmemLayout<BN, STAGES, BEXACT>;
   constexpr int BKE = F16 ? 2 * BK : BK;
@@ -449,7 +483,7 @@
   splits = (total_kb + kb_per_split - 1) / kb_per_split;
   if (splits != g.splits_effective) { set_last_error("gemm: splits_effective mismatch (use gemm_effective_splits)"); return -1; }
 
-  auto kern = gemm_tf32x3_kernel<BN, STAGES, BEXACT, F16>;
+  auto kern = gemm_tf32x3_kernel<BN, STAGES, BEXACT, F16, SUM>;
   static int max_clusters[64] = {};
   int clusters_cap = dev >= 0 && dev < 64 ? max_clusters[dev] : 0;
   if (clusters_cap == 0) {
@@ -462,14 +496,14 @@
     if (clusters_cap < 1) { set_last_error("gemm: no 2-CTA cluster of this kernel fits the device"); return -1; }
     if (dev >= 0 && dev < 64) max_clusters[dev] = clusters_cap;
   }
-  const int items = m_tiles * n_pairs * splits;
+  const int items = m_tiles * n_pairs * (SUM ? 1 : splits);
   const int clusters = items < clusters_cap ? items : clusters_cap;
-  const double kslice_row = static_cast<double>(kb_per_split) * BK * 4;
+  const double kslice_row = static_cast<double>(SUM ? total_kb : kb_per_split) * BK * 4;
   const TileOrder ord = pick_tile_order(m_tiles, n_pairs, BM * kslice_row * 2, 2 * BN * kslice_row * (BEXACT ? 1 : 2),
                                         clusters, l2);
   kern<<<2 * clusters, NUM_THREADS, L::DYN_BYTES, stream>>>(mAh, mAl, mBh, mBl, g.C, g.M, g.ldc, g.c_split_stride,
                                                             ord, n_tiles, splits, total_kb, kb_per_split, BEXACT ? 2 : 1,
-                                                    g.out_col_scale, g.a_tile_scale, g.a_tiles, 3);
+                                                            g.out_col_scale, g.a_tile_scale, g.a_tiles, 3);
   CNMF_CUDA_CHECK(cudaGetLastError());
   return 0;
 }
@@ -493,26 +527,58 @@
   return (total_kb + kb_per_split - 1) / kb_per_split;
 }
 
-static int pick_tile_n(const GemmArgs& g) {
-  if (!g.b_exact) return 128;
+int gemm_device_pairs() {
+  static int pairs[64] = {};
   int dev = 0, sms = 0;
-  CNMF_CUDA_CHECK(cudaGetDevice(&dev));
-  CNMF_CUDA_CHECK(cudaDeviceGetAttribute(&sms, cudaDevAttrMultiProcessorCount, dev));
-  const long long pairs = std::max(1, sms / 2);
-  const long long m_items = static_cast<long long>((g.M + BM - 1) / BM) * g.splits_effective;
-  const int cols = std::min(g.ldc, (g.N + 31) / 32 * 32);
+  if (cudaGetDevice(&dev) != cudaSuccess) return 1;
+  if (dev >= 0 && dev < 64 && pairs[dev] > 0) return pairs[dev];
+  if (cudaDeviceGetAttribute(&sms, cudaDevAttrMultiProcessorCount, dev) != cudaSuccess) return 1;
+  const int p = std::max(1, sms / 2);
+  if (dev >= 0 && dev < 64) pairs[dev] = p;
+  return p;
+}
+
+static int tile_n_and_cost(int M, int N, int ldc, int b_exact, int items_per_m_tile, int pairs, long long* cost_out) {
+  const long long m_items = static_cast<long long>((M + BM - 1) / BM) * items_per_m_tile;
+  const int cols = std::min(ldc, (N + 31) / 32 * 32);
   auto cost = [&](int bn, int per_item) {
     const long long items = m_items * (((cols + bn - 1) / bn + 1) / 2);
     return (items + pairs - 1) / pairs * per_item;
   };
   const long long narrow = cost(128, 100);
   int best = 128;
-  long long best_cost = narrow * 98 / 100;
-  for (const auto& [bn, per_item] : {std::pair<int, int>{168, 125}, std::pair<int, int>{192, 142}}) {
-    const long long c = cost(bn, per_item);
-    if (c <= best_cost) { best_cost = c; best = bn; }
-  }
+  long long best_cost = narrow;
+  if (b_exact) {
+    long long bar = narrow * 98 / 100;
+    for (const auto& [bn, per_item] : {std::pair<int, int>{168, 125}, std::pair<int, int>{192, 142}}) {
+      const long long c = cost(bn, per_item);
+      if (c <= bar) { bar = best_cost = c; best = bn; }
+    }
+  }
+  if (cost_out) *cost_out = best_cost;
   return best;
+}
+
+int gemm_pick_tile_n(int M, int N, int ldc, int b_exact, int items_per_m_tile, int pairs) {
+  return tile_n_and_cost(M, N, ldc, b_exact, items_per_m_tile, std::max(1, pairs), nullptr);
+}
+
+int gemm_pick_sum_slices(int M, int N, int ldc, int Kd, int splits, int form, int pairs) {
+  if (splits <= 1 || form < 1 || M <= 0 || N <= 0 || Kd <= 0) return 0;
+  pairs = std::max(1, pairs);
+  const int f16 = form == 2 ? 1 : 0, b_exact = form >= 1 ? 1 : 0;
+  const int total_kb = (Kd + (f16 ? 2 * BK : BK) - 1) / (f16 ? 2 * BK : BK);
+  int kb_per_split = (total_kb + splits - 1) / splits;
+  if (f16 && (kb_per_split & 1)) ++kb_per_split;
+  long long split_cost = 0;
+  tile_n_and_cost(M, N, ldc, b_exact, splits, pairs, &split_cost);
+  const long long tiles = static_cast<long long>((M + BM - 1) / BM) * (((std::min(ldc, (N + 31) / 32 * 32) + 167) / 168 + 1) / 2);
+  const long long sum_cost = (tiles + pairs - 1) / pairs * 125;
+  const double us_per_kb = 0.34 * 2;
+  const double t_split = 1e-2 * static_cast<double>(split_cost) * kb_per_split * us_per_kb +
+                         2.0 * (splits - 1) * static_cast<double>(M) * ldc * 4.0 / 3.0e6;
+  const double t_sum = 1e-2 * static_cast<double>(sum_cost) * total_kb * us_per_kb;
+  return t_sum < t_split ? 1 : 0;
 }
 
 int gemm_tf32x3(const GemmArgs& g, cudaStream_t stream) {
@@ -524,7 +590,17 @@
                "gemm: pointers must be 16-byte aligned");
   CNMF_REQUIRE(g.tile_n == 0 || g.tile_n == 128 || (g.b_exact && (g.tile_n == 168 || g.tile_n == 192)),
                "gemm: tile_n must be 0 (the launcher's choice), 128, or 168 / 192 with an exact B");
-  const int bn = g.tile_n ? g.tile_n : pick_tile_n(g);
+  if (g.sum_slices) {
+    CNMF_REQUIRE(g.b_exact && (g.tile_n == 0 || g.tile_n == 168),
+                 "gemm: summed slices need an exact B and run on 168-column tiles");
+    if (g.f16) {
+      CNMF_REQUIRE(g.lda % 8 == 0 && g.ldb % 8 == 0, "gemm: fp16 leading dimensions must be multiples of 8 halves");
+      CNMF_REQUIRE(!g.a_tile_scale || g.a_tiles * 512 >= g.Kd, "gemm: a_tiles does not cover the reduction length");
+      return launch<168, 4, true, true, true>(g, stream);
+    }
+    return launch<168, 4, true, false, true>(g, stream);
+  }
+  const int bn = g.tile_n ? g.tile_n : gemm_pick_tile_n(g.M, g.N, g.ldc, g.b_exact, g.splits_effective, gemm_device_pairs());
   if (g.f16) {
     CNMF_REQUIRE(g.b_exact, "gemm: the fp16 path needs an exact B operand");
     CNMF_REQUIRE(g.lda % 8 == 0 && g.ldb % 8 == 0, "gemm: fp16 leading dimensions must be multiples of 8 halves");
diff --git a/cnmf_b200/csrc/nmf_engine.cu b/cnmf_b200/csrc/nmf_engine.cu
--- a/cnmf_b200/csrc/nmf_engine.cu
+++ b/cnmf_b200/csrc/nmf_engine.cu
@@ -63,10 +63,17 @@
   }
 }
 
-GemmPlan view_gemm_plan(const DataView& v, int side, int SK) {
+GemmPlan view_gemm_plan(const DataView& v, int side, int SK, int slice_sum) {
   const int f16 = v.form == Form::F16_EXACT ? 1 : 0;
-  return side == 0 ? GemmPlan{gemm_fixed_splits(v.n_c, f16), (long long)SK * v.ld_r}
-                   : GemmPlan{gemm_fixed_splits(v.n_r, f16), (long long)SK * v.ld_c};
+  GemmPlan p = side == 0 ? GemmPlan{gemm_fixed_splits(v.n_c, f16), (long long)SK * v.ld_r, 0}
+                         : GemmPlan{gemm_fixed_splits(v.n_r, f16), (long long)SK * v.ld_c, 0};
+  const int form = v.form == Form::F16_EXACT ? 2 : v.form == Form::TF32_EXACT ? 1 : v.form == Form::TF32 ? 0 : -1;
+  if (p.splits > 1 && form >= 0 && slice_sum != CNMF_GEMM_SLICES_SEPARATE) {
+    const int n = side == 0 ? v.n_r : v.n_c, kd = side == 0 ? v.n_c : v.n_r, ld = side == 0 ? v.ld_r : v.ld_c;
+    p.sum_slices = slice_sum == CNMF_GEMM_SLICES_SUMMED ? 1
+                                                        : gemm_pick_sum_slices(SK, n, ld, kd, p.splits, form, gemm_device_pairs());
+  }
+  return p;
 }
 
 int view_gemm(cnmf_handle_s* h, const DataView& v, int side, const float* F, const float* F_hi, const float* F_lo,
@@ -81,6 +88,7 @@
   g.c_split_stride = plan.split_stride;
   g.splits = plan.splits;
   g.splits_effective = plan.splits;
+  g.sum_slices = plan.sum_slices;
   h->launches += 1;
   const int slot = h->prof_begin(s, 2.0 * (double)g.M * (double)g.N * (double)g.Kd);
   const int rc = form_gemm(v.form, g, F, F_hi, F_lo, tile_scale, B, side == 0 ? v.scale_r : v.scale_c, s);
@@ -152,15 +160,21 @@
   GemmPlan plan_r, plan_c;
   float *NUMr = nullptr, *NUMc = nullptr;
   auto plan_gemms = [&]() -> int {
-    plan_r = view_gemm_plan(v, 0, SK);
-    if (io.num_rows) plan_r.splits = 1;
-    plan_c = view_gemm_plan(v, 1, SK);
+    plan_r = view_gemm_plan(v, 0, SK, h->gemm_slice_sum);
+    if (io.num_rows) { plan_r.splits = 1; plan_r.sum_slices = 0; }
+    plan_c = view_gemm_plan(v, 1, SK, h->gemm_slice_sum);
     return 0;
   };
   plan_gemms();
+  auto product_rows = [&](int side) -> size_t {
+    size_t rows = 0;
+    for (int sk = 1; sk <= SK0; ++sk)
+      rows = std::max(rows, (size_t)view_gemm_plan(v, side, sk, h->gemm_slice_sum).out_slices() * (size_t)sk);
+    return rows;
+  };
   {
-    const size_t need_r = (size_t)plan_r.splits * (size_t)SK0 * v.ld_r;
-    const size_t need_c = (size_t)plan_c.splits * (size_t)SK0 * v.ld_c;
+    const size_t need_r = io.num_rows ? 0 : product_rows(0) * v.ld_r;
+    const size_t need_c = io.update_cols ? product_rows(1) * v.ld_c : 0;
     NUMr = io.num_rows ? const_cast<float*>(io.num_rows) : static_cast<float*>(h->dev_buf("solve.NUMr", sizeof(float) * need_r));
     NUMc = io.update_cols ? static_cast<float*>(h->dev_buf("solve.NUMc", sizeof(float) * need_c)) : nullptr;
     if (!NUMr || (io.update_cols && !NUMc)) return -2;
@@ -263,9 +277,9 @@
   auto update = [&](bool cd, const FactorView& f, const float* NUM, const GemmPlan& pl, const double* gram_in, float l1,
                     float l2, const FusedOut& out) -> int {
     h->launches += 1;
-    const int slot = h->prof_begin(s, upd_bytes(f.n, pl.splits, f.F_hi ? 2 : ((f.P_hi && out.gram_part) ? 1 : 0)), 1);
-    const int rc = cd ? launch_cd_update(f, NUM, pl.splits, pl.split_stride, gram_in, bm(), l1, l2, out, s)
-                      : launch_mu_update(f, NUM, pl.splits, pl.split_stride, gram_in, bm(), l1, l2, out, s);
+    const int slot = h->prof_begin(s, upd_bytes(f.n, pl.out_slices(), f.F_hi ? 2 : ((f.P_hi && out.gram_part) ? 1 : 0)), 1);
+    const int rc = cd ? launch_cd_update(f, NUM, pl.out_slices(), pl.split_stride, gram_in, bm(), l1, l2, out, s)
+                      : launch_mu_update(f, NUM, pl.out_slices(), pl.split_stride, gram_in, bm(), l1, l2, out, s);
     h->prof_end(s, slot);
     if (rc != 0 || !io.update_cols) return rc;
     if (f.P_hi && out.gram_part) return 0;
@@ -331,10 +345,10 @@
     CNMF_TRY(launch_finalize(d_gpartR, d_gramR, nullptr, nullptr, gram_chunks(fr()), bm0, s));
     CNMF_TRY(launch_finalize(d_gpartC, d_gramC, nullptr, nullptr, gram_chunks(fc()), bm0, s));
     if (io.update_cols) {
-      CNMF_TRY(launch_cross(fc(), NUMc, plan_c.splits, plan_c.split_stride, bm0, d_scalB, s));
+      CNMF_TRY(launch_cross(fc(), NUMc, plan_c.out_slices(), plan_c.split_stride, bm0, d_scalB, s));
       CNMF_TRY(launch_finalize(nullptr, nullptr, d_scalB, d_crossB, chunks_c, bm0, s));
     } else {
-      CNMF_TRY(launch_cross(fr(), NUMr, plan_r.splits, plan_r.split_stride, bm0, d_scalA, s));
+      CNMF_TRY(launch_cross(fr(), NUMr, plan_r.out_slices(), plan_r.split_stride, bm0, d_scalA, s));
       CNMF_TRY(launch_finalize(nullptr, nullptr, d_scalA, d_crossB, chunks_r, bm0, s));
     }
     ConvState scratch{d_state + 5 * R0, d_state + 6 * R0, d_cd_err, d_zero, d_zero + R0};
@@ -433,12 +447,12 @@
     if (io.update_cols) {
       CNMF_TRY(gemm_cols());
       h->launches += 1;
-      CNMF_TRY(launch_cross(fc(), NUMc, plan_c.splits, plan_c.split_stride, bm(), d_scalB, s));
+      CNMF_TRY(launch_cross(fc(), NUMc, plan_c.out_slices(), plan_c.split_stride, bm(), d_scalB, s));
       CNMF_TRY(finalize_scal(d_scalB, d_crossB, chunks_c));
     } else {
       CNMF_TRY(gemm_rows());
       h->launches += 1;
-      CNMF_TRY(launch_cross(fr(), NUMr, plan_r.splits, plan_r.split_stride, bm(), d_scalA, s));
+      CNMF_TRY(launch_cross(fr(), NUMr, plan_r.out_slices(), plan_r.split_stride, bm(), d_scalA, s));
       CNMF_TRY(finalize_scal(d_scalA, d_crossB, chunks_r));
     }
     h->launches += 1;
diff --git a/cnmf_b200/engine.py b/cnmf_b200/engine.py
--- a/cnmf_b200/engine.py
+++ b/cnmf_b200/engine.py
@@ -181,6 +181,9 @@
     def nndsvd_chunk_limit(self, max_restarts):
         check(self.lib.cnmf_nndsvd_chunk_limit(self._h, int(max_restarts)))
 
+    def gemm_slice_sum(self, mode):
+        check(self.lib.cnmf_gemm_slice_sum(self._h, _lib.GEMM_SLICES[mode]))
+
     def dataset(self, X, precision=_DEFAULT_PRECISION, stream=None):
         return Dataset(self, X, precision, stream)
 
@@ -220,7 +223,7 @@
         return int(peak.value)
 
     def gemm_abt(self, A, B, precision=PRECISION_TF32X3, splits=1, reps=1, b_exact=False, k_scale=None,
-                 out_col_scale=None, tile_n=0):
+                 out_col_scale=None, tile_n=0, slice_sum="separate", slices=False):
         A, B = f32c(A), f32c(B)
         M, Kd = A.shape
         N = B.shape[0]
@@ -233,9 +236,18 @@
         ms = ctypes.c_float(0)
         pc = precision_code(precision)
         pc = PRECISION_TF32X3 if pc == PRECISION_TF32X3_GENERAL else pc
+        S = None
+        if slices:
+            assert slice_sum in ("separate", "summed"), "slices=True needs a fixed slice_sum"
+            bke = 64 if pc == PRECISION_F16X2 else 32
+            total_kb = -(-Kd // bke)
+            kbps = -(-total_kb // max(1, min(int(splits), total_kb)))
+            kbps += kbps & 1 if pc == PRECISION_F16X2 else 0
+            S = np.empty((1 if slice_sum == "summed" else -(-total_kb // kbps), M, N), np.float32)
         check(self.lib.cnmf_gemm_abt_host(self._h, pc, ptr(A), ptr(B), M, N, Kd, splits, 1 if b_exact else 0,
-                                          ptr(ks), ptr(cs), int(tile_n), ptr(C), reps, ctypes.byref(ms), None))
-        return C, float(ms.value)
+                                          ptr(ks), ptr(cs), int(tile_n), _lib.GEMM_SLICES[slice_sum], ptr(C), ptr(S),
+                                          reps, ctypes.byref(ms), None))
+        return (C, float(ms.value), S) if slices else (C, float(ms.value))
 
     def update_step(self, ks, rids, done, n, F, num, gram_in, solver="mu", pieces=None, gram=None, want_scalar=False,
                     cpb_tiles=1, l1=0.0, l2=0.0, piece_scale=None, pieces_hi=None, pieces_lo=None, tile_scale=None,
diff --git a/include/cnmf_b200.h b/include/cnmf_b200.h
--- a/include/cnmf_b200.h
+++ b/include/cnmf_b200.h
@@ -131,8 +131,11 @@
 int cnmf_project_rows(cnmf_dataset_t d, int k, const float* Ut_host, float* out_host, void* stream);
 
 int cnmf_gemm_abt_host(cnmf_handle_t h, int precision, const float* A, const float* B, int M, int N, int Kd,
-                       int splits, int b_exact, const float* k_scale, const float* out_col_scale, int tile_n, float* C,
-                       int reps, float* ms_out, void* stream);
+                       int splits, int b_exact, const float* k_scale, const float* out_col_scale, int tile_n,
+                       int slice_sum, float* C, float* C_slices, int reps, float* ms_out, void* stream);
+enum { CNMF_GEMM_SLICES_BY_SHAPE = 0, CNMF_GEMM_SLICES_SEPARATE = 1, CNMF_GEMM_SLICES_SUMMED = 2 };
+int cnmf_gemm_slice_sum(cnmf_handle_t h, int mode);
+int cnmf_gemm_slice_plan_host(int M, int N, int Kd, int form, int pairs, int* splits, int* sum_slices, int* tile_n);
 
 enum { CNMF_UNIT_SOLVER_NONE = -1 };
 enum { CNMF_UNIT_PIECES_NONE = 0, CNMF_UNIT_PIECES_TF32 = 1, CNMF_UNIT_PIECES_F16 = 2 };
```

New measurement: 578.5, median of 6. Within noise of the previous version (+0.6%).
